# MrSwordFish/rvel-mcmc

Measured on AMD Instinct MI355X. Metric: walker-logL evals/sec (2-planet, 100 obs, 4096 walkers); ESS/sec, higher is better.
Workload: dtype f64

## Files before the change

include/rvmcmc.h:

```cpp
#ifndef RVMCMC_H
#define RVMCMC_H

#include <stddef.h>
#include <stdint.h>

#ifdef __cplusplus
extern "C" {
#endif

#define RVM_ABI_VERSION 12

#define RVM_STATUS_OK 0
#define RVM_STATUS_PRIOR 1
#define RVM_STATUS_ENCOUNTER 2
#define RVM_STATUS_NONFINITE 3
#define RVM_STATUS_UNRESOLVED 4
#define RVM_STATUS_SKIPPED 5

#define RVM_MAX_PLANETS 4
#define RVM_MAX_LEVELS 6
#define RVM_MAX_EPOCHS_PER_DIRECTION 1700
#define RVM_SMALA_MAX_PARAMS 20
#define RVM_RESOLVE_MAX_LIMIT 12

typedef struct {
    int32_t n_planets;
    double dt;
    int32_t n_levels;
    double npoints_norm;
    int32_t level_mult[RVM_MAX_LEVELS];
    double period_hint;
    int32_t inclined;
    double resolve_tol;
    int32_t resolve_max;
} rvm_config;

typedef struct rvm_plan rvm_plan;

int rvm_plan_create(const rvm_config* cfg, const double* t, const double* rv, const double* sigma, int32_t n_obs,
                    int32_t max_walkers, rvm_plan** out);
void rvm_plan_destroy(rvm_plan* plan);
int rvm_plan_info(const rvm_plan* plan, int32_t* steps_fwd, int32_t* steps_bwd, int32_t* epochs_fwd,
                  int32_t* epochs_bwd);
#define RVM_EXT_MAX_BYTES (4ull << 30)
int rvm_plan_extension(const rvm_plan* plan, int32_t* ext_mult);
int rvm_plan_set_verify_eccentricity(rvm_plan* plan, double e);

int rvm_plan_set_certain_reject(rvm_plan* plan, int32_t on);

int rvm_plan_faults(rvm_plan* plan, int32_t reset, int64_t* handoff_timeouts, int64_t* nonfinite,
                    int64_t* unresolved, int64_t* refined, int64_t* truncated, void* stream);
#define RVM_N_COUNTERS 7
int rvm_plan_counters(rvm_plan* plan, int32_t reset, int64_t* out, int32_t n, void* stream);
int rvm_plan_hedge_stats(rvm_plan* plan, int32_t reset, int64_t* hedged, int64_t* replayed, int64_t* missed,
                         void* stream);
int rvm_plan_hedge_marks(rvm_plan* plan, int32_t reset, int64_t* marked, int64_t* gave_up, void* stream);
int rvm_plan_time_kernels(rvm_plan* plan, int32_t max_launches);
int rvm_plan_kernel_times(rvm_plan* plan, float* logl_ms, float* refine_ms, int32_t max, int32_t* n_out);
int rvm_plan_set_handoff_timeout(rvm_plan* plan, double seconds);

int rvm_logl_batch(const rvm_plan* plan, int32_t n_walkers, const double* params, double hill_factor,
                   double* logl_out, int32_t* status_out, double* rv_out, void* stream);


int rvm_stretch_propose(int32_t n_params, int32_t n_s0, int64_t s0_begin, const double* x, int32_t n_s1,
                        const double* c, double a, uint64_t seed, uint64_t iteration, uint32_t half,
                        const double* draws, double* q_out, double* z_out, void* stream);
int rvm_stretch_accept(int32_t n_params, int32_t n_s0, int64_t s0_begin, double* x, double* lnp, const double* q,
                       const double* lnp_new, const double* z, uint64_t seed, uint64_t iteration, uint32_t half,
                       const double* draws, int32_t* accepted, void* stream);

#define RVM_MAX_PARAM_ROWS (7 * RVM_MAX_PLANETS)
typedef struct rvm_param_map {
    int32_t n_rows;
    int32_t src[RVM_MAX_PARAM_ROWS];
    double base[RVM_MAX_PARAM_ROWS];
} rvm_param_map;

int rvm_stretch_half_step(const rvm_plan* plan, const rvm_param_map* map, int32_t n_params, int32_t n_s0,
                          int64_t s0_begin, double* x, double* x_aos, double* lnp, int32_t n_s1, const double* c_aos,
                          double a, uint64_t seed, uint64_t iteration, uint32_t half, double hill_factor,
                          double* lnp_new_out, int32_t* status_out, int32_t* accepted, void* stream);

int rvm_stretch_iteration_begin(const rvm_plan* plan, const rvm_param_map* map, int32_t n_params, int32_t n_loc,
                                int64_t s0_begin, int64_t s1_begin, double* x0, double* lnp0, const double* x1,
                                const double* lnp1, int32_t n_half, const double* c0, const double* c1, double a,
                                uint64_t seed, uint64_t iteration, double hill_factor, double* lnp_spec,
                                int32_t* status_spec, int32_t* dec, int32_t* accepted0, void* stream);
int rvm_stretch_iteration_end(int32_t n_params, int32_t n_loc, int64_t s0_begin, int64_t s1_begin, const double* x0,
                              double* x0_aos, const int32_t* dec, const int32_t* dec_all, double* x1, double* x1_aos,
                              double* lnp1, int32_t n_half, const double* c0, const double* c1,
                              const double* lnp_spec, const int32_t* status_spec, double a, uint64_t seed,
                              uint64_t iteration, int32_t* accepted1, double* lnp_new_out, int32_t* status_new_out,
                              void* stream);

int rvm_pt_stretch_propose(int32_t n_params, int32_t n_temps, int32_t n_half, const double* x, const double* c,
                           double a, uint64_t seed, uint64_t iteration, uint32_t half, const double* draws,
                           double* q_out, double* z_out, void* stream);
int rvm_pt_stretch_accept(int32_t n_params, int32_t n_temps, int32_t n_half, const double* betas, double* x,
                          double* lnp, const double* q, const double* lnp_new, const double* z, uint64_t seed,
                          uint64_t iteration, uint32_t half, const double* draws, int32_t* accepted, void* stream);
int rvm_pt_swap(int32_t n_params, int32_t n_temps, int32_t n_half, const double* betas, double* x0, double* x1,
                double* lnp0, double* lnp1, uint64_t seed, uint64_t iteration, const double* draws,
                int32_t* swapped, void* stream);

int rvm_pt_ladder_update(int32_t n_temps, int32_t n_half, const int32_t* swapped, const double* lnp0,
                         const double* lnp1, double kappa, double* betas, int64_t* swap_totals_prev,
                         double* ratios_out, int64_t* n_refused, double* lnp_moments, void* workspace,
                         void* stream);

int rvm_mh_propose(int32_t n_params, int32_t n_chains, int64_t chain_begin, const double* x, const double* scales,
                   double step_size, uint64_t seed, uint64_t iteration, const double* draws, double* q_out,
                   void* stream);
int rvm_mh_accept(int32_t n_params, int32_t n_chains, int64_t chain_begin, double* x, double* lnp, const double* q,
                  const double* lnp_new, uint64_t seed, uint64_t iteration, const double* draws, int32_t* accepted,
                  void* stream);
int rvm_mh_step(const rvm_plan* plan, const rvm_param_map* map, int32_t n_params, int32_t n_chains,
                int64_t chain_begin, double* x, double* lnp, const double* scales, double step_size, uint64_t seed,
                uint64_t iteration, double hill_factor, double* lnp_new_out, int32_t* status_out, int32_t* accepted,
                void* stream);

int rvm_fd_params(int32_t n_params, int32_t n_chains, const double* x, double rel_step, const double* floor_,
                  double* out, void* stream);

typedef struct {
    double* lp;
    double* grad;
    double* mu;
    double* L;
    double* G;
    double* logdet;
    int32_t* ok;
} rvm_smala_cache;

int rvm_smala_derive(int32_t n_params, int32_t n_chains, int32_t n_obs, const double* x, double rel_step,
                     const double* floor_, const double* lp_stencil, const int32_t* status_stencil,
                     const double* rv_stencil, const double* inv_sigma2, double npoints_norm, double alpha,
                     double eps, const rvm_smala_cache* out, void* stream);
int rvm_smala_metric(int32_t n_params, int32_t n_chains, const double* x, const double* lp, const int32_t* status,
                     const double* grad, const double* hess, double alpha, double eps, const rvm_smala_cache* out,
                     void* stream);
int rvm_smala_propose(int32_t n_params, int32_t n_chains, int64_t chain_begin, const double* x,
                      const rvm_smala_cache* cur, double eps, uint64_t seed, uint64_t iteration,
                      const double* draws, double* x_prop, void* stream);
int rvm_smala_accept(int32_t n_params, int32_t n_chains, int64_t chain_begin, double* x, const rvm_smala_cache* cur,
                     const double* x_prop, const rvm_smala_cache* prop, double eps, uint64_t seed,
                     uint64_t iteration, const double* draws, int32_t* accepted, int32_t* failures, void* stream);

int rvm_smala_stencil_logl(const rvm_plan* plan, const rvm_param_map* map, int32_t n_params, int32_t n_chains,
                           const double* x, double rel_step, const double* floor_, double hill_factor,
                           double* logl_out, int32_t* status_out, double* rv_out, void* stream);
int rvm_smala_derive_accept(int32_t n_params, int32_t n_chains, int64_t chain_begin, int32_t n_obs, double* x,
                            const double* x_prop, double rel_step, const double* floor_, const double* lp_stencil,
                            const int32_t* status_stencil, const double* rv_stencil, const double* inv_sigma2,
                            double npoints_norm, double alpha, double eps, const rvm_smala_cache* cur,
                            const rvm_smala_cache* prop, uint64_t seed, uint64_t iteration, const double* draws,
                            int32_t* accepted, int32_t* failures, void* stream);
int rvm_smala_derive_sides(int32_t n_params, int32_t n_chains, int32_t n_obs, const double* x, double rel_step,
                           const double* floor_, const double* lp_stencil, const int32_t* status_stencil,
                           const double* rv_stencil, const double* inv_sigma2, double npoints_norm, double alpha,
                           double eps, const rvm_smala_cache* out, void* stream);
int rvm_smala_center_accept(int32_t n_params, int32_t n_chains, int64_t chain_begin, double* x, const double* x_prop,
                            const double* lp_center, const int32_t* status_center, const rvm_smala_cache* cur,
                            const rvm_smala_cache* prop, double eps, uint64_t seed, uint64_t iteration,
                            const double* draws, int32_t* accepted, int32_t* failures, void* stream);
int rvm_smala_metric_accept(int32_t n_params, int32_t n_chains, int64_t chain_begin, double* x, const double* x_prop,
                            const double* lp, const int32_t* status, const double* grad, const double* hess,
                            double alpha, double eps, const rvm_smala_cache* cur, const rvm_smala_cache* prop,
                            uint64_t seed, uint64_t iteration, const double* draws, int32_t* accepted,
                            int32_t* failures, void* stream);

size_t rvm_logl_derivs_workspace_bytes(int32_t n_chains, int32_t n_dirs);
int rvm_logl_derivs(const rvm_plan* plan, int32_t n_chains, const double* params, int32_t n_dirs,
                    const int32_t* dir_rows, double hill_factor, double* logl_out, double* grad_out, double* hess_out,
                    int32_t* status_out, void* workspace, void* stream);

int rvm_chain_record(int32_t n_params, int32_t n_cols, const double* src, int64_t src_ld, int64_t src_col0,
                     int64_t col_stride, double* dst, int64_t dst_ld, int64_t dst_col0, const double* lnp_src,
                     double* lnp_dst, void* stream);
int rvm_chain_moments(const double* chain, int32_t n_params, int32_t n_cols, int64_t t0, int64_t t1, double* mean_out,
                      double* m2_out, void* stream);
size_t rvm_chain_autocov_workspace_bytes(int32_t n_params, int32_t n_cols, int32_t n_lags);
int rvm_chain_autocov(const double* chain, const double* mean, int32_t n_params, int32_t n_cols, int64_t t0, int64_t t1,
                      int32_t lag0, int32_t n_lags, double* acov_out, void* workspace, void* stream);

const char* rvm_last_error(void);
int rvm_abi_version(void);

#ifdef __cplusplus
}
#endif

#endif
```

rvel-mcmc_amd/csrc/host_sanitize.cpp:

```cpp
#include <algorithm>
#include <cmath>
#include <cstdio>
#include <cstdlib>
#include <cstring>
#include <vector>

#include "rvm_plan_host.h"

static int fails = 0;
static void expect(bool ok, const char* what) {
    if (!ok) {
        std::fprintf(stderr, "FAIL %s\n", what);
        fails++;
    }
}

static double exact_weight(const int* m, int k0, int n, int k) {
    long long num = 1, den = 1;
    for (int j = k0; j < n; j++) {
        if (j == k) continue;
        num *= (long long)m[k] * m[k];
        den *= (long long)m[k] * m[k] - (long long)m[j] * m[j];
    }
    return (double)num / (double)den;
}

static bool close_rel(double a, double b, double rel) { return std::fabs(a - b) <= rel * std::fabs(b); }

static double ulp_of(double x) { return std::nextafter(std::fabs(x), INFINITY) - std::fabs(x); }

struct Range {
    size_t off, bytes;
    bool wide;
};
static void check_block(const std::vector<Range>& r, size_t block_bytes, const char* what) {
    size_t end = 0;
    for (const Range& x : r) {
        expect(x.off >= end, what);
        expect(!x.wide || x.off % 8 == 0, what);
        end = x.off + x.bytes;
    }
    expect(end <= block_bytes, what);
}

static const char* const kKnobNames[] = {
    "RVM_SKIP_VARIANTS", "RVM_LATE_SPO",   "RVM_NO_LEVEL_SPLIT", "RVM_REFINE_TEAMS", "RVM_EAGER_SPLIT",
    "RVM_NO_EXTENSION",  "RVM_REFINE_SPLIT", "RVM_TEAMS_HINT",   "RVM_EAGER",        "RVM_EAGER_PASSES",
    "RVM_HEDGE",         "RVM_HEDGE_GROUPS", "RVM_HEDGE_MARK",   "RVM_LS_F0"};

static rvm::PlanKnobs knobs_with(const char* name, const char* value) {
    setenv(name, value, 1);
    const rvm::PlanKnobs K = rvm::read_plan_knobs();
    unsetenv(name);
    return K;
}

static void check_plan_host(const rvm_config& cfg, const std::vector<double>& t, const std::vector<double>& rv,
                            const std::vector<double>& sg) {
    using namespace rvm;
    const int n_obs = (int)t.size();
    for (const char* name : kKnobNames) unsetenv(name);
    const PlanKnobs K = read_plan_knobs();
    expect(K.skip_variants == 1 && K.late_spo == 96.0 && !K.no_level_split && K.n_teams == RVM_TEAMS_DEFAULT &&
               K.eager_split == 1 && !K.no_extension && K.refine_split && K.teams_hint && K.eager &&
               K.eager_passes == 1 && K.hedge_groups == RVM_HEDGE_GROUPS_MAX && K.hedge_mark == 1,
           "knob defaults");
    expect(knobs_with("RVM_REFINE_TEAMS", "9").n_teams == RVM_TEAMS_MAX, "RVM_REFINE_TEAMS=9 clamps");
    expect(knobs_with("RVM_HEDGE", "0").hedge_groups == 0, "RVM_HEDGE=0");
    expect(knobs_with("RVM_HEDGE_GROUPS", "3").hedge_groups == 3, "RVM_HEDGE_GROUPS=3");
    expect(knobs_with("RVM_EAGER_PASSES", "2").eager_passes == 2, "RVM_EAGER_PASSES=2");
    expect(knobs_with("RVM_SKIP_VARIANTS", "0").skip_variants == 0, "RVM_SKIP_VARIANTS=0");

    int mult[RVM_MAX_LEVELS] = {}, max_mult = 0;
    expect(check_plan_config(&cfg, t.data(), rv.data(), sg.data(), n_obs, 4096, mult, &max_mult) == nullptr,
           "config ok");
    expect(mult[0] == 4 && mult[1] == 5 && mult[2] == 6 && mult[3] == 7 && max_mult == 7, "explicit ladder");
    {
        rvm_config h = cfg;
        h.n_levels = 3;
        std::memset(h.level_mult, 0, sizeof(h.level_mult));
        int hm[RVM_MAX_LEVELS] = {}, hmax = 0;
        expect(check_plan_config(&h, t.data(), rv.data(), sg.data(), n_obs, 64, hm, &hmax) == nullptr && hm[0] == 1 &&
                   hm[1] == 2 && hm[2] == 3 && hmax == 3,
               "harmonic ladder");
    }

    HostDir dir[2];
    expect(build_schedule(&cfg, mult, max_mult, t.data(), rv.data(), sg.data(), n_obs, dir) == nullptr, "schedule ok");
    std::vector<int> seen(n_obs, 0);
    int n_dup = 0;
    for (int d = 0; d < 2; d++) {
        const HostDir& D = dir[d];
        const size_t n = D.idx.size();
        expect(D.seg_n.size() == n && D.seg_len.size() == n && D.orv.size() == n && D.os2.size() == n,
               "schedule sizes");
        long long sum = 0, pre0 = 0, pre1 = 0;
        double tprev = 0.0;
        for (size_t i = 0; i < n; i++) {
            const int o = D.idx[i];
            expect(o >= 0 && o < n_obs && (d == 0) == (t[o] >= 0.0), "obs_idx direction");
            if (o >= 0 && o < n_obs) seen[o]++;
            const double at = std::fabs(t[o]), len = (d == 0 ? 1.0 : -1.0) * (at - tprev);
            expect(at >= tprev, "|t| non-decreasing");
            if (at == tprev) {
                n_dup += i > 0;
                expect(D.seg_n[i] == 0 && D.seg_len[i] == 0.0, "duplicate epoch: empty segment");
            } else {
                expect(D.seg_n[i] >= 1 && std::fabs(D.seg_len[i]) <= cfg.dt * (1.0 + 1e-9), "segment step <= dt");
                expect(std::fabs(D.seg_n[i] * D.seg_len[i] - len) <= 4.0 * ulp_of(len), "segment steps x step = length");
            }
            tprev = at;
            if ((int)i < D.split0) pre0 += D.seg_n[i];
            if ((int)i < D.split1) pre1 += D.seg_n[i];
            sum += D.seg_n[i];
        }
        expect(sum == D.total_steps, "sum(seg_n) = n_steps");
        expect(D.split0 >= 0 && D.split0 <= (int)n && D.split1 >= 0 && D.split1 <= (int)n, "split range");
        expect(pre0 == D.pre0 && pre1 == D.pre1, "pre = steps before the split");
    }
    expect(std::all_of(seen.begin(), seen.end(), [](int c) { return c == 1; }), "obs_idx is a permutation");
    expect(n_dup == 1, "one duplicate epoch");

    const size_t nf = dir[0].idx.size(), nb = dir[1].idx.size();
    rvm_config ad = cfg;
    ad.resolve_tol = 5e-7;
    ad.resolve_max = 6;
    DevPlan P{};
    fill_plan_scalars(&ad, mult, n_obs, nf, nb, 256, K, &P);
    expect(P.ext_mult == 0 && plan_wants_extension(P, K), "extension wanted, not yet applied");
    fill_plan_extension(&P);
    const int m5[5] = {4, 5, 6, 7, 8};
    for (int k = 0; k < 4; k++) expect(close_rel(P.lw[k], exact_weight(m5, 0, 4, k), 1e-14), "lw");
    for (int k = 1; k < 4; k++) expect(close_rel(P.lw3[k], exact_weight(m5, 1, 4, k), 1e-14), "lw3");
    for (int k = 0; k < 5; k++) expect(close_rel(P.lw5[k], exact_weight(m5, 0, 5, k), 1e-14), "lw5");
    expect(P.lw3[0] == 0.0 && P.lw[4] == 0.0 && P.lw[5] == 0.0 && P.lw5[5] == 0.0, "unused weights are zero");

    expect(P.fin_level == 3, "fin_level");
    expect(P.ext_mult == 8 && P.mult[4] == 8 && P.inv_ext == 0.125 && P.inv_mult[4] == 0.125, "ext_mult");
    expect(P.rmax == 6 && P.rtol_dir == 2.5e-7 && P.cut == 1 && P.n_teams == RVM_TEAMS_DEFAULT, "adaptive scalars");
    for (int k = 0; k < 4; k++) {
        const double nh = 2.0 * M_PI * cfg.dt / (mult[k] * cfg.period_hint), zn = 2.0 * nh * nh;
        expect(P.nt[k] == (zn <= 0.1 ? 6 : (zn <= 0.3 ? 7 : 8)) && P.spec[k] == (zn <= 0.04 ? 1 : 0), "nt / spec");
        expect(P.inv_mult[k] == 1.0 / mult[k], "inv_mult");
    }
    expect(P.ext_nt == P.nt[3] && P.ext_spec == P.spec[3] && P.nt[4] == P.nt[3] && P.spec[4] == P.spec[3],
           "ext nt / spec");
    expect(P.late_mult == (int)std::ceil(96 * 0.65 / 5.2 - 1e-9) && P.late_mult == 12, "late_mult");
    expect(P.lc_ring >= 2 && P.lc_ring <= RVM_LC_RING, "lc_ring range");
    expect((size_t)(cfg.n_levels + 1) * 32 * 8 * P.lc_ring <= RVM_LC_RING_BYTES, "lc_ring bytes");
    {
        DevPlan Q{};
        fill_plan_scalars(&cfg, mult, n_obs, nf, nb, 256, K, &Q);
        expect(Q.rmax == 0 && !plan_wants_extension(Q, K) && Q.ext_mult == 0, "no extension without resolve_tol");
        ad.resolve_max = 0;
        fill_plan_scalars(&ad, mult, n_obs, nf, nb, 256, K, &Q);
        expect(!plan_wants_extension(Q, K) && Q.ext_mult == 0, "no extension with resolve_max 0");
        expect(!plan_wants_extension(P, knobs_with("RVM_NO_EXTENSION", "1")), "RVM_NO_EXTENSION=1");
        fill_plan_scalars(&cfg, mult, n_obs, nf, nb, 256, knobs_with("RVM_LATE_SPO", "0"), &Q);
        expect(Q.late_mult == 0, "RVM_LATE_SPO=0");
    }

    for (int32_t mw : {1, 64, 6144}) {
        const size_t w = (size_t)mw, em = std::max(nf, nb);
        const DmemLayout D = dmem_layout(nf, nb, mw);
        check_block({{D.seg_h1[0], 8 * nf, true}, {D.obs_rv[0], 8 * nf, true}, {D.obs_s2[0], 8 * nf, true},
                     {D.seg_h1[1], 8 * nb, true}, {D.obs_rv[1], 8 * nb, true}, {D.obs_s2[1], 8 * nb, true},
                     {D.slots, 8 * w, true}, {D.counters, 8 * RVM_N_COUNTERS, true}, {D.seg_n[0], 4 * nf, false},
                     {D.obs_idx[0], 4 * nf, false}, {D.seg_n[1], 4 * nb, false}, {D.obs_idx[1], 4 * nb, false}},
                    D.bytes, "dmem layout");
        const LvLayout V = lv_layout(nf, nb, mw);
        expect(V.emax == (int32_t)em, "lv emax");
        check_block({{V.rv, 8 * 2 * em * w, true}, {V.enc, 4 * 2 * w, false}}, V.bytes, "lvmem layout");
        for (int teams : {1, 2, 4}) {
            const size_t nt = (size_t)std::max(teams, 2), xg = (w + 15) / 16 + 1;
            const XLayout X = x_layout(nf, nb, mw, teams);
            check_block({{X.lvx, 16 * em * w, true}, {X.rvp, 16 * em * w, true},
                         {X.rvp2, 16 * em * w * (teams - 1), true}},
                        X.bytes, "xmem layout");
            const RqLayout R = rq_layout(mw, teams);
            expect(R.xgroups == (int32_t)xg, "rq xgroups");
            check_block({{R.x, xg * nt * 256 * 8, true}, {R.xf, xg * nt * 2 * 8, true},
                         {R.t, xg * (nt - 1) * 1024 * 8, true}, {R.tf, xg * nt * 8, true}, {R.c, 16 * w, true},
                         {R.w, 12 * w, false}, {R.n, 16, false}, {R.gen, 8, true}, {R.mark, 4 * w, false},
                         {R.depth, 8 * (RVM_DEPTH_WINDOW + 1), true}},
                        R.bytes, "rqmem layout");
            expect(R.gen == R.n + 32 && R.mark == R.n + 64 && R.mark % 64 == R.n % 64, "rq_n | gen_dev | rq_mark");
        }
        const HLayout H = h_layout((int32_t)em, mw);
        const size_t hs = RVM_HEDGE_STRIDE;
        check_block({{H.hrv, 16 * em * hs, true}, {H.hsum, 48 * hs, true}, {H.hslot, 16 * hs, true},
                     {H.htab, 8 * w, true}, {H.hw, 8 * RVM_HW_WORDS, true}},
                    H.bytes, "hmem layout");
        const ELayout E = e_layout((int32_t)em, mw);
        check_block({{E.rve, 32 * em * w, true}, {E.esum, 96 * w, true},
                     {E.eflag, 8 * (RVM_EFLAG_WORDS * (size_t)((RVM_EAGER_MAX + 15) / 16) + 8), true}},
                    E.bytes, "emem layout");
    }
}

int main() {
    expect(rvm_abi_version() == RVM_ABI_VERSION, "abi version");
    rvm_config cfg{};
    cfg.n_planets = 2;
    cfg.dt = 0.65;
    cfg.n_levels = 4;
    cfg.npoints_norm = 100.0;
    const int mult[4] = {4, 5, 6, 7};
    std::memcpy(cfg.level_mult, mult, sizeof(mult));
    cfg.period_hint = 5.2;
    std::vector<double> t, rv, sg;
    for (int i = 0; i < 101; i++) {
        t.push_back(i % 2 ? -0.6 * i : 0.55 * (100 - i));
        rv.push_back(1e-4 * std::sin(i));
        sg.push_back(1.5e-4);
    }
    t[7] = t[9];
    rvm_plan* plan = nullptr;
    const int rc = rvm_plan_create(&cfg, t.data(), rv.data(), sg.data(), (int)t.size(), 4096, &plan);
    expect(rc == 0 || (rc < 0 && plan == nullptr), "plan_create valid input");
    if (rc == 0) rvm_plan_destroy(plan);
    check_plan_host(cfg, t, rv, sg);
    rvm_config bad = cfg;
    bad.n_levels = 0;
    expect(rvm_plan_create(&bad, t.data(), rv.data(), sg.data(), (int)t.size(), 64, &plan) < 0, "n_levels 0");
    bad = cfg;
    bad.level_mult[1] = 4;
    expect(rvm_plan_create(&bad, t.data(), rv.data(), sg.data(), (int)t.size(), 64, &plan) < 0, "dup multipliers");
    bad = cfg;
    bad.dt = -1.0;
    expect(rvm_plan_create(&bad, t.data(), rv.data(), sg.data(), (int)t.size(), 64, &plan) < 0, "negative dt");
    std::vector<double> tn = t;
    tn[3] = NAN;
    expect(rvm_plan_create(&cfg, tn.data(), rv.data(), sg.data(), (int)t.size(), 64, &plan) < 0, "nan epoch");
    expect(std::strlen(rvm_last_error()) > 0, "last_error");
    expect(rvm_logl_batch(nullptr, 1, nullptr, 1.0, nullptr, nullptr, nullptr, nullptr) < 0, "logl null plan");
    int64_t mk = -1, gu = -1;
    expect(rvm_plan_hedge_marks(nullptr, 0, &mk, &gu, nullptr) < 0 && mk == -1 && gu == -1, "hedge_marks null plan");
    rvm_param_map pm{};
    expect(rvm_stretch_half_step(nullptr, &pm, 10, 1, 0, nullptr, nullptr, nullptr, 1, nullptr, 2.0, 0, 0, 0, 1.0,
                                 nullptr, nullptr, nullptr, nullptr) < 0,
           "half_step null plan");
    expect(rvm_stretch_propose(0, 1, 0, nullptr, 1, nullptr, 2.0, 0, 0, 0, nullptr, nullptr, nullptr, nullptr) < 0,
           "propose bad");
    double d1 = 0.5;
    int32_t i1 = 0;
    expect(rvm_pt_stretch_propose(10, 0, 1, &d1, &d1, 2.0, 0, 0, 0, nullptr, &d1, &d1, nullptr) < 0, "pt n_temps 0");
    expect(rvm_pt_stretch_propose(10, 2, 1, &d1, &d1, 1.0, 0, 0, 0, nullptr, &d1, &d1, nullptr) < 0, "pt a = 1");
    expect(rvm_pt_stretch_propose(10, 1 << 16, 1 << 16, &d1, &d1, 2.0, 0, 0, 0, nullptr, &d1, &d1, nullptr) < 0,
           "pt int32 overflow");
    expect(rvm_pt_stretch_accept(10, 2, 1, nullptr, &d1, &d1, &d1, &d1, &d1, 0, 0, 0, nullptr, &i1, nullptr) < 0,
           "pt null betas");
    expect(rvm_pt_stretch_accept(10, 2, 1, &d1, &d1, &d1, &d1, &d1, &d1, 0, 0, 2, nullptr, &i1, nullptr) < 0,
           "pt half 2");
    expect(rvm_pt_swap(10, 2, 0, &d1, &d1, &d1, &d1, &d1, 0, 0, nullptr, &i1, nullptr) < 0, "pt n_half 0");
    expect(rvm_pt_swap(10, 1 << 15, 1 << 15, &d1, &d1, &d1, &d1, &d1, 0, 0, nullptr, &i1, nullptr) < 0,
           "pt swap int32 overflow");
    expect(rvm_pt_swap(10, 1, 4, nullptr, nullptr, nullptr, nullptr, nullptr, 0, 0, nullptr, nullptr, nullptr) == 0,
           "pt swap of one temperature");
    int64_t l1 = 0;
    expect(rvm_pt_ladder_update(3, 1, &i1, &d1, &d1, -1.0, &d1, &l1, &d1, &l1, nullptr, &d1, nullptr) < 0,
           "pt ladder kappa < 0");
    expect(rvm_pt_ladder_update(3, 1, &i1, &d1, &d1, 0.5, &d1, &l1, &d1, &l1, nullptr, nullptr, nullptr) < 0,
           "pt ladder null workspace");
    expect(rvm_pt_ladder_update(1 << 16, 1 << 15, &i1, &d1, &d1, 0.5, &d1, &l1, &d1, &l1, nullptr, &d1, nullptr) < 0,
           "pt ladder int32 overflow");
    expect(rvm_pt_ladder_update(1, 4, nullptr, nullptr, nullptr, 0.5, nullptr, nullptr, nullptr, nullptr, nullptr,
                                nullptr, nullptr) == 0,
           "pt ladder of one temperature");
    expect(rvm_chain_record(2, 4, &d1, 16, 0, INT64_MAX, &d1, 8, 0, nullptr, nullptr, nullptr) < 0,
           "chain record stride overflow");
    expect(rvm_chain_record(2, 4, &d1, 16, 0, 1, &d1, INT64_MAX, INT64_MAX - 1, nullptr, nullptr, nullptr) < 0,
           "chain record dst_col0 overflow");
    expect(rvm_chain_record(2, 4, &d1, 16, 0, 1, &d1, 8, 0, &d1, nullptr, nullptr) < 0, "chain record lone lnp_src");
    expect(rvm_chain_moments(&d1, 2, 4, 5, 5, &d1, &d1, nullptr) < 0, "chain moments empty range");
    expect(rvm_chain_autocov(&d1, &d1, 2, 4, 0, 10, INT32_MAX, 1 << 30, &d1, &d1, nullptr) < 0,
           "chain autocov lag overflow");
    expect(rvm_chain_autocov(&d1, &d1, 65534, 4, 0, INT64_MAX, 0, 1 << 30, &d1, &d1, nullptr) < 0,
           "chain autocov n_params * n_lags");
    expect(rvm_chain_autocov_workspace_bytes(10, 200, 17) == (size_t)8 * 10 * 32, "chain autocov workspace");
    expect(rvm_chain_autocov_workspace_bytes(1, 65535 * 256, 1 << 30) == (size_t)8 * ((size_t)1 << 30) * 65535,
           "chain autocov workspace, largest");
    expect(rvm_chain_autocov_workspace_bytes(65534, 4, 1 << 30) == 0, "chain autocov workspace, refused");
    expect(rvm_mh_accept(0, 1, 0, nullptr, nullptr, nullptr, nullptr, 0, 0, nullptr, nullptr, nullptr) < 0, "mh bad");
    expect(rvm_fd_params(10, 1, nullptr, 1e-6, nullptr, nullptr, nullptr) < 0, "fd bad");
    const int32_t rows[2] = {0, 0};
    expect(rvm_logl_derivs(nullptr, 1, nullptr, 2, rows, 1.0, nullptr, nullptr, nullptr, nullptr, nullptr, nullptr) < 0,
           "derivs null plan");
    expect(rvm_logl_derivs_workspace_bytes(256, 10) == (size_t)256 * 55 * 2 * 36, "derivs workspace");
    rvm_smala_cache c{};
    expect(rvm_smala_metric(10, 1, nullptr, nullptr, nullptr, nullptr, nullptr, 1.0, 0.5, &c, nullptr) < 0, "metric bad");
    std::printf("host sanitize driver: %d failures\n", fails);
    return fails;
}
```

rvel-mcmc_amd/csrc/rvm_internal.h:

```cpp
#pragma once
#include <stdint.h>

#include "../../include/rvmcmc.h"

namespace rvm {

constexpr int RVM_LS_RING = 64;
constexpr int RVM_LC_RING = 16;
constexpr int RVM_LC_RING_BYTES = 24 * 1024;
constexpr int RVM_LDS_PER_CU = 160 * 1024;
constexpr int RVM_INIT_DOUBLES = 8 * 64;
constexpr double RVM_EXT_ACCEPT = 1.0;
constexpr double RVM_CUT_EST_FACTOR = 100.0;
constexpr double RVM_FLOOR_BOUND = 4.0;
constexpr double RVM_CUT_ECC_FACTOR = 0.6712;
constexpr double RVM_CUT_GUARD_K = 10.0;
constexpr int RVM_CX_MIN_WALKERS = 32;
constexpr int RVM_EAGER_MAX = 512;
constexpr int RVM_EAGER_MIN = 32;
constexpr int RVM_EFLAG_WORDS = 8;
constexpr int RVM_TEAMS_MAX = 4;
constexpr int RVM_TEAMS_DEFAULT = 4;
constexpr int RVM_DEPTH_WINDOW = 8;
constexpr int RVM_HEDGE_GROUPS_MAX = 8;
constexpr int RVM_HEDGE_STRIDE = 512;
constexpr int RVM_HEDGE_CAND = RVM_HEDGE_STRIDE + 64;
constexpr int RVM_HEDGE_MAX_W = 12288;
constexpr int RVM_HW_STATS = 2 + 2 * RVM_HEDGE_GROUPS_MAX;
constexpr int RVM_HW_MARK = RVM_HW_STATS + 3 + 3;
constexpr int RVM_HW_WORDS = RVM_HW_MARK + 2 * RVM_HEDGE_GROUPS_MAX;

struct DirSched {
    int32_t n_epochs;
    int32_t n_steps;
    int32_t split0, pre0, split1, pre1;
    const int32_t* seg_n;
    const double* seg_h1;
    const double* obs_rv;
    const double* obs_s2;
    const int32_t* obs_idx;
};

struct DevPlan {
    int32_t n_planets;
    int32_t n_levels;
    int32_t mult[RVM_MAX_LEVELS];
    int32_t nt[RVM_MAX_LEVELS];
    int32_t spec[RVM_MAX_LEVELS];
    int32_t late_mult;
    int32_t lc_ring;
    double inv_mult[RVM_MAX_LEVELS];
    double lw[RVM_MAX_LEVELS];
    double lw3[RVM_MAX_LEVELS];
    double rtol_dir;
    int32_t rmax;
    int32_t fin_level;
    int32_t cut;
    int32_t ext_mult, ext_nt, ext_spec;
    double inv_ext;
    double lw5[RVM_MAX_LEVELS + 1];
    double* lvx;
    double* rvp;
    double e2_guard;
    double e2_cut;
    double cut_guard_k;
    int32_t lvx_emax, lvx_stride;
    int32_t* rq_n;
    int32_t* rq_w;
    double* rq_c;
    int32_t rq_cap;
    int32_t* rq_mark;
    int32_t skip_variants;
    unsigned long long* rq_x;
    unsigned long long* rq_xf;
    int32_t rq_xgroups;
    unsigned long long* rq_t;
    unsigned long long* rq_tf;
    double* rvp2;
    int32_t n_teams;
    unsigned long long* depth_w;
    double* rve;
    double* esum;
    unsigned long long* eflag;
    int32_t eager_max;
    int32_t eager_passes;
    int32_t eager_split;
    int32_t hedge_groups;
    int32_t hedge_mark;
    double* hrv;
    double* hsum;
    unsigned long long* hslot;
    unsigned long long* htab;
    unsigned long long* hw;
    unsigned long long* gen_dev;
    unsigned long long* counters;
    unsigned long long spin_ticks;
    double npoints;
    int32_t n_obs;
    int32_t inclined;
    int32_t n_cu;
    double* lv_rv;
    int32_t* lv_enc;
    int32_t lv_emax, lv_stride;
    DirSched fwd, bwd;
};

struct StretchArgs {
    const double* c;
    double* x;
    double* x_aos;
    double* lnp;
    int32_t* accepted;
    int64_t s0_begin;
    uint64_t seed, iteration;
    double a;
    int32_t n1, dim;
    uint32_t half;
    int32_t xstride;
    int32_t n_spec;
    const double* c0;
    const double* x1;
    int64_t s1_begin;
    int32_t* dec;
    const double* lnp1;
    const double* mh_scale;
    double mh_step;
    const double* fd_x;
    const double* fd_floor;
    double fd_rel;
    int32_t fd_n;
    int32_t src[RVM_MAX_PARAM_ROWS];
    double base[RVM_MAX_PARAM_ROWS];
};

struct IterEndArgs {
    int32_t dim, n, n_half;
    int64_t s0_begin, s1_begin;
    const double* x0;
    double* x0_aos;
    const int32_t* dec_local;
    const int32_t* dec_all;
    double* x1;
    double* x1_aos;
    double* lnp1;
    const double* c0;
    const double* c1;
    const double* lnp_spec;
    const int32_t* st_spec;
    double a;
    uint64_t seed, iteration;
    int32_t* accepted1;
    double* lnp_new_out;
    int32_t* status_new_out;
};

struct PtLadderArgs {
    int32_t T, Wh;
    const int32_t* swapped;
    const double* lnp0;
    const double* lnp1;
    double kappa;
    double* betas;
    int64_t* totals_prev;
    double* ratios;
    int64_t* n_refused;
    double* moments;
    int64_t* ws_totals;
    double* ws_moments;
};

struct SmalaCache {
    double* lp;
    double* grad;
    double* mu;
    double* L;
    double* G;
    double* logdet;
    int32_t* ok;
};

}
```

rvel-mcmc_amd/csrc/rvm_plan.hip:

```cpp
#include <algorithm>
#include <cmath>
#include <cstdlib>
#include <cstring>

#include "rvm_launch.h"
#include "rvm_plan.h"
#include "rvm_plan_host.h"

using rvm::fail;
using rvm::hip_fail;

namespace {

template <class T>
T* at(void* block, size_t offset) {
    return reinterpret_cast<T*>(reinterpret_cast<unsigned char*>(block) + offset);
}

template <class T>
const T* put(std::vector<unsigned char>& host, void* block, size_t offset, const std::vector<T>& v) {
    if (!v.empty()) std::memcpy(host.data() + offset, v.data(), v.size() * sizeof(T));
    return at<T>(block, offset);
}

bool alloc_filled(void** mem, size_t bytes, int fill) {
    if (hipMalloc(mem, bytes) == hipSuccess && hipMemset(*mem, fill, bytes) == hipSuccess &&
        hipDeviceSynchronize() == hipSuccess)
        return true;
    (void)hipGetLastError();
    if (*mem) (void)hipFree(*mem);
    *mem = nullptr;
    return false;
}

int upload_schedule(rvm_plan* plan, const rvm::HostDir dir[2], int32_t max_walkers) {
    const rvm::DmemLayout L = rvm::dmem_layout(dir[0].idx.size(), dir[1].idx.size(), max_walkers);
    hipError_t e = hipMalloc(&plan->dmem, L.bytes);
    if (e != hipSuccess) return hip_fail(e, "rvm_plan_create: hipMalloc");
    std::vector<unsigned char> host(L.bytes, 0);
    rvm::DirSched* S[2] = {&plan->dev.fwd, &plan->dev.bwd};
    for (int dd = 0; dd < 2; dd++) {
        const rvm::HostDir& D = dir[dd];
        S[dd]->n_epochs = (int32_t)D.idx.size();
        S[dd]->n_steps = plan->steps[dd] = (int32_t)D.total_steps;
        S[dd]->split0 = D.split0;
        S[dd]->pre0 = D.pre0;
        S[dd]->split1 = D.split1;
        S[dd]->pre1 = D.pre1;
        S[dd]->seg_h1 = put(host, plan->dmem, L.seg_h1[dd], D.seg_len);
        S[dd]->obs_rv = put(host, plan->dmem, L.obs_rv[dd], D.orv);
        S[dd]->obs_s2 = put(host, plan->dmem, L.obs_s2[dd], D.os2);
        S[dd]->seg_n = put(host, plan->dmem, L.seg_n[dd], D.seg_n);
        S[dd]->obs_idx = put(host, plan->dmem, L.obs_idx[dd], D.idx);
    }
    plan->slots = at<unsigned long long>(plan->dmem, L.slots);
    for (int32_t i = 0; i < max_walkers; i++)
        at<unsigned long long>(host.data(), L.slots)[i] = 0x7FF4DEADBEEF0001ULL;
    plan->dev.counters = at<unsigned long long>(plan->dmem, L.counters);
    plan->max_walkers = max_walkers;
    e = hipMemcpy(plan->dmem, host.data(), L.bytes, hipMemcpyHostToDevice);
    return e == hipSuccess ? 0 : hip_fail(e, "rvm_plan_create: hipMemcpy");
}

int device_cus() {
    int dev = 0, ncu = 0;
    if (hipGetDevice(&dev) != hipSuccess ||
        hipDeviceGetAttribute(&ncu, hipDeviceAttributeMultiprocessorCount, dev) != hipSuccess)
        ncu = 0;
    return ncu;
}

void alloc_level_split(rvm_plan* plan, size_t nf, size_t nb, const rvm::PlanKnobs& K) {
    rvm::DevPlan& P = plan->dev;
    if (!rvm::plan_wants_level_split(P, plan->max_walkers, K)) return;
    const rvm::LvLayout L = rvm::lv_layout(nf, nb, plan->max_walkers);
    if (!alloc_filled(&plan->lvmem, L.bytes, 0xFF)) return;
    P.lv_rv = at<double>(plan->lvmem, L.rv);
    P.lv_enc = at<int32_t>(plan->lvmem, L.enc);
    P.lv_emax = L.emax;
    P.lv_stride = plan->max_walkers;
    plan->lv_bytes = L.bytes;
}

void alloc_extension(rvm_plan* plan, size_t nf, size_t nb, const rvm::PlanKnobs& K) {
    rvm::DevPlan& P = plan->dev;
    if (!rvm::plan_wants_extension(P, K)) return;
    const rvm::XLayout L = rvm::x_layout(nf, nb, plan->max_walkers, K.n_teams);
    if (L.bytes > RVM_EXT_MAX_BYTES) return;
    if (hipMalloc(&plan->xmem, L.bytes) != hipSuccess) {
        plan->xmem = nullptr;
        (void)hipGetLastError();
        return;
    }
    rvm::fill_plan_extension(&P);
    P.lvx = at<double>(plan->xmem, L.lvx);
    P.rvp = at<double>(plan->xmem, L.rvp);
    P.rvp2 = K.n_teams >= 2 ? at<double>(plan->xmem, L.rvp2) : nullptr;
    P.lvx_emax = L.emax;
    P.lvx_stride = plan->max_walkers;
}

int alloc_work_lists(rvm_plan* plan, const rvm::PlanKnobs& K) {
    rvm::DevPlan& P = plan->dev;
    if (P.rmax <= 0) return 0;
    const rvm::RqLayout L = rvm::rq_layout(plan->max_walkers, K.n_teams);
    if (hipMalloc(&plan->rqmem, L.bytes) != hipSuccess || hipMemset(plan->rqmem, 0, L.bytes) != hipSuccess ||
        hipDeviceSynchronize() != hipSuccess) {
        (void)hipGetLastError();
        return fail(-3, "rvm_plan_create: hipMalloc of the refinement work lists failed");
    }
    P.rq_x = K.refine_split ? at<unsigned long long>(plan->rqmem, L.x) : nullptr;
    P.rq_xf = at<unsigned long long>(plan->rqmem, L.xf);
    P.rq_t = K.n_teams >= 2 ? at<unsigned long long>(plan->rqmem, L.t) : nullptr;
    P.rq_tf = at<unsigned long long>(plan->rqmem, L.tf);
    P.rq_c = at<double>(plan->rqmem, L.c);
    P.rq_w = at<int32_t>(plan->rqmem, L.w);
    P.rq_n = at<int32_t>(plan->rqmem, L.n);
    P.gen_dev = at<unsigned long long>(plan->rqmem, L.gen);
    P.rq_mark = at<int32_t>(plan->rqmem, L.mark);
    P.depth_w = K.teams_hint ? at<unsigned long long>(plan->rqmem, L.depth) : nullptr;
    P.rq_cap = plan->max_walkers;
    P.rq_xgroups = L.xgroups;
    const unsigned long long gen1 = 1;
    if (hipMemcpy(P.gen_dev, &gen1, sizeof(gen1), hipMemcpyHostToDevice) != hipSuccess) {
        (void)hipGetLastError();
        return fail(-3, "rvm_plan_create: initialising the launch generation failed");
    }
    return 0;
}

void side_drop(rvm_plan* plan) {
    (void)hipGetLastError();
    if (plan->ev_fork) (void)hipEventDestroy(plan->ev_fork);
    if (plan->ev_join) (void)hipEventDestroy(plan->ev_join);
    if (plan->side) (void)hipStreamDestroy(plan->side);
    plan->side = nullptr;
    plan->ev_fork = plan->ev_join = nullptr;
    plan->dev.hedge_groups = 0;
}

bool side_create(rvm_plan* plan) {
    if (hipStreamCreateWithFlags(&plan->side, hipStreamNonBlocking) == hipSuccess &&
        hipEventCreateWithFlags(&plan->ev_fork, hipEventDisableTiming) == hipSuccess &&
        hipEventCreateWithFlags(&plan->ev_join, hipEventDisableTiming) == hipSuccess)
        return true;
    side_drop(plan);
    return false;
}

void setup_side_features(rvm_plan* plan, const rvm::PlanKnobs& K) {
    rvm::DevPlan& P = plan->dev;
    const int32_t mw = plan->max_walkers;
    const bool refines = P.rmax >= 2 && P.rvp != nullptr && P.gen_dev != nullptr && P.n_levels <= 4 &&
                         mw >= rvm::RVM_EAGER_MIN;
    if (K.hedge_groups > 0 && refines && P.n_cu >= 4) {
        const rvm::HLayout L = rvm::h_layout(P.lvx_emax, mw);
        if (alloc_filled(&plan->hmem, L.bytes, 0)) {
            P.hrv = at<double>(plan->hmem, L.hrv);
            P.hsum = at<double>(plan->hmem, L.hsum);
            P.hslot = at<unsigned long long>(plan->hmem, L.hslot);
            P.htab = at<unsigned long long>(plan->hmem, L.htab);
            P.hw = at<unsigned long long>(plan->hmem, L.hw);
            P.hedge_groups = K.hedge_groups;
            P.hedge_mark = K.hedge_mark;
        }
    }
    if (!(refines && K.eager)) {
        if (P.hedge_groups > 0) (void)side_create(plan);
        return;
    }
    const rvm::ELayout L = rvm::e_layout(P.lvx_emax, P.lvx_stride);
    if (alloc_filled(&plan->emem, L.bytes, 0) && side_create(plan)) {
        P.rve = at<double>(plan->emem, L.rve);
        P.esum = at<double>(plan->emem, L.esum);
        P.eflag = at<unsigned long long>(plan->emem, L.eflag);
        P.eager_max = std::min<int>(mw, rvm::RVM_EAGER_MAX);
        P.eager_passes = K.eager_passes;
    } else {
        side_drop(plan);
        if (plan->emem) (void)hipFree(plan->emem);
        plan->emem = nullptr;
    }
}

int prepare_kernels(const rvm::DevPlan& P) {
    const hipError_t pe = rvm::prepare_logl(P);
    if (pe != hipSuccess)
        return fail(-1, pe == hipErrorInvalidConfiguration
                            ? "rvm_plan_create: the epoch schedule does not fit the likelihood kernel's LDS "
                              "(too many epochs in one direction)"
                            : "rvm_plan_create: n_planets has no kernel instantiation");
    if (rvm::prepare_refine(P) != hipSuccess)
        return fail(-1, "rvm_plan_create: the epoch schedule does not fit the refinement kernel's LDS "
                        "(too many epochs in one direction for the adaptive resolution)");
    return 0;
}

int read_hw_words(rvm_plan* plan, const char* who, int first, int n, int32_t reset, void* stream,
                  unsigned long long* h) {
    if (!plan) return fail(-1, std::string(who) + ": null plan");
    std::memset(h, 0, n * sizeof(*h));
    if (plan->dev.hw == nullptr) return 0;
    hipStream_t st = (hipStream_t)stream;
    unsigned long long* d = plan->dev.hw + first;
    hipError_t e = hipMemcpyAsync(h, d, n * sizeof(*h), hipMemcpyDeviceToHost, st);
    if (e == hipSuccess && reset) e = hipMemsetAsync(d, 0, n * sizeof(*h), st);
    if (e == hipSuccess) e = hipStreamSynchronize(st);
    return e == hipSuccess ? 0 : hip_fail(e, who);
}

}

extern "C" {

int rvm_plan_create(const rvm_config* cfg, const double* t, const double* rv, const double* sigma, int32_t n_obs,
                    int32_t max_walkers, rvm_plan** out) {
    if (!cfg || !t || !rv || !sigma || !out) return fail(-1, "rvm_plan_create: null argument");
    int mult[RVM_MAX_LEVELS], max_mult = 1;
    if (const char* m = rvm::check_plan_config(cfg, t, rv, sigma, n_obs, max_walkers, mult, &max_mult))
        return fail(-1, m);
    rvm::HostDir dir[2];
    if (const char* m = rvm::build_schedule(cfg, mult, max_mult, t, rv, sigma, n_obs, dir)) return fail(-1, m);
    const size_t nf = dir[0].idx.size(), nb = dir[1].idx.size();
    const rvm::PlanKnobs K = rvm::read_plan_knobs();
    rvm_plan* plan = new rvm_plan();
    int rc = upload_schedule(plan, dir, max_walkers);
    if (rc == 0) {
        rvm::fill_plan_scalars(cfg, mult, n_obs, nf, nb, device_cus(), K, &plan->dev);
        alloc_level_split(plan, nf, nb, K);
        alloc_extension(plan, nf, nb, K);
        rc = alloc_work_lists(plan, K);
    }
    if (rc == 0) {
        setup_side_features(plan, K);
        rc = prepare_kernels(plan->dev);
    }
    if (rc != 0) {
        rvm_plan_destroy(plan);
        return rc;
    }
    *out = plan;
    return 0;
}

void rvm_plan_destroy(rvm_plan* plan) {
    if (!plan) return;
    if (plan->side) (void)hipStreamSynchronize(plan->side);
    if (plan->ev_fork) (void)hipEventDestroy(plan->ev_fork);
    if (plan->ev_join) (void)hipEventDestroy(plan->ev_join);
    if (plan->side) (void)hipStreamDestroy(plan->side);
    if (plan->emem) (void)hipFree(plan->emem);
    if (plan->hmem) (void)hipFree(plan->hmem);
    for (hipEvent_t ev : plan->tev) (void)hipEventDestroy(ev);
    if (plan->rqmem) (void)hipFree(plan->rqmem);
    if (plan->lvmem) (void)hipFree(plan->lvmem);
    if (plan->xmem) (void)hipFree(plan->xmem);
    if (plan->dmem) (void)hipFree(plan->dmem);
    delete plan;
}

int rvm_plan_set_certain_reject(rvm_plan* plan, int32_t on) {
    if (!plan) return fail(-1, "rvm_plan_set_certain_reject: null plan");
    plan->dev.cut = on ? 1 : 0;
    return 0;
}

int rvm_plan_set_verify_eccentricity(rvm_plan* plan, double e) {
    if (!plan) return fail(-1, "rvm_plan_set_verify_eccentricity: null plan");
    if (std::isnan(e) || e >= 1.0) return fail(-1, "rvm_plan_set_verify_eccentricity: e must be < 1 (<= 0: off)");
    plan->dev.e2_guard = e > 0.0 ? e * e : INFINITY;
    {
        const char* cf = getenv("RVM_CUT_FACTOR");
        const double ec = 1.0 - (1.0 - e) * (cf ? atof(cf) : rvm::RVM_CUT_ECC_FACTOR);
        const char* cg = getenv("RVM_CUT_GUARD");
        plan->dev.e2_cut = e > 0.0 && !(cg && atoi(cg) == 0) ? ec * ec : INFINITY;
        const char* ck = getenv("RVM_CUT_GUARD_K");
        plan->dev.cut_guard_k = ck ? atof(ck) : rvm::RVM_CUT_GUARD_K;
    }
    return 0;
}

int rvm_plan_extension(const rvm_plan* plan, int32_t* ext_mult) {
    if (!plan) return fail(-1, "rvm_plan_extension: null plan");
    if (ext_mult) *ext_mult = plan->dev.ext_mult;
    return 0;
}

int rvm_plan_counters(rvm_plan* plan, int32_t reset, int64_t* out, int32_t n, void* stream) {
    if (!plan) return fail(-1, "rvm_plan_counters: null plan");
    if (n < 0 || (n > 0 && !out)) return fail(-1, "rvm_plan_counters: bad output array");
    hipStream_t st = (hipStream_t)stream;
    unsigned long long h[RVM_N_COUNTERS] = {};
    hipError_t e = hipMemcpyAsync(h, plan->dev.counters, sizeof(h), hipMemcpyDeviceToHost, st);
    if (e == hipSuccess) e = hipStreamSynchronize(st);
    if (e != hipSuccess) return hip_fail(e, "rvm_plan_counters");
    for (int i = 0; i < n; i++) out[i] = i < RVM_N_COUNTERS ? (int64_t)h[i] : 0;
    if (reset) {
        if (plan->lvmem) e = hipMemsetAsync(plan->lvmem, 0xFF, plan->lv_bytes, st);
        if (e == hipSuccess) e = hipMemsetAsync(plan->dev.counters, 0, sizeof(h), st);
        if (e == hipSuccess) e = hipStreamSynchronize(st);
        if (e != hipSuccess) return hip_fail(e, "rvm_plan_counters: reset");
    }
    return 0;
}

int rvm_plan_hedge_stats(rvm_plan* plan, int32_t reset, int64_t* hedged, int64_t* replayed, int64_t* missed,
                         void* stream) {
    unsigned long long h[3];
    const int rc = read_hw_words(plan, "rvm_plan_hedge_stats", rvm::RVM_HW_STATS, 3, reset, stream, h);
    if (rc != 0) return rc;
    if (hedged) *hedged = (int64_t)h[0];
    if (replayed) *replayed = (int64_t)h[1];
    if (missed) *missed = (int64_t)h[2];
    return 0;
}

int rvm_plan_hedge_marks(rvm_plan* plan, int32_t reset, int64_t* marked, int64_t* gave_up, void* stream) {
    unsigned long long h[2];
    const int rc = read_hw_words(plan, "rvm_plan_hedge_marks", rvm::RVM_HW_STATS + 3, 2, reset, stream, h);
    if (rc != 0) return rc;
    if (marked) *marked = (int64_t)h[0];
    if (gave_up) *gave_up = (int64_t)h[1];
    return 0;
}

int rvm_plan_faults(rvm_plan* plan, int32_t reset, int64_t* handoff_timeouts, int64_t* nonfinite,
                    int64_t* unresolved, int64_t* refined, int64_t* truncated, void* stream) {
    if (!plan) return fail(-1, "rvm_plan_faults: null plan");
    int64_t c[RVM_N_COUNTERS] = {};
    const int rc = rvm_plan_counters(plan, reset, c, RVM_N_COUNTERS, stream);
    if (rc != 0) return rc;
    if (handoff_timeouts) *handoff_timeouts = c[0];
    if (nonfinite) *nonfinite = c[1];
    if (unresolved) *unresolved = c[2];
    if (refined) *refined = c[3];
    if (truncated) *truncated = c[4];
    return 0;
}

int rvm_plan_time_kernels(rvm_plan* plan, int32_t max_launches) {
    if (!plan) return fail(-1, "rvm_plan_time_kernels: null plan");
    if (max_launches < 0 || max_launches > 4096) return fail(-1, "rvm_plan_time_kernels: max_launches out of range");
    while ((int32_t)plan->tev.size() < 3 * max_launches) {
        hipEvent_t ev;
        const hipError_t e = hipEventCreate(&ev);
        if (e != hipSuccess) return hip_fail(e, "rvm_plan_time_kernels: hipEventCreate");
        plan->tev.push_back(ev);
    }
    plan->tcap = max_launches;
    plan->tn = 0;
    return 0;
}

int rvm_plan_kernel_times(rvm_plan* plan, float* logl_ms, float* refine_ms, int32_t max, int32_t* n_out) {
    if (!plan || max < 0) return fail(-1, "rvm_plan_kernel_times: bad arguments");
    const int n = std::min(plan->tn, max);
    for (int i = 0; i < n; i++) {
        hipError_t e = hipEventSynchronize(plan->tev[3 * i + 2]);
        float a = 0.0f, b = 0.0f;
        if (e == hipSuccess) e = hipEventElapsedTime(&a, plan->tev[3 * i], plan->tev[3 * i + 1]);
        if (e == hipSuccess) e = hipEventElapsedTime(&b, plan->tev[3 * i + 1], plan->tev[3 * i + 2]);
        if (e != hipSuccess) return hip_fail(e, "rvm_plan_kernel_times");
        if (logl_ms) logl_ms[i] = a;
        if (refine_ms) refine_ms[i] = b;
    }
    if (n_out) *n_out = n;
    plan->tn = 0;
    plan->tcap = 0;
    return 0;
}

int rvm_plan_set_handoff_timeout(rvm_plan* plan, double seconds) {
    if (!plan) return fail(-1, "rvm_plan_set_handoff_timeout: null plan");
    if (!(seconds > 0.0) || !(seconds < 1e9)) return fail(-1, "rvm_plan_set_handoff_timeout: seconds out of range");
    const double ticks = seconds * 1e8;
    plan->dev.spin_ticks = ticks < 1.0 ? 1ull : (unsigned long long)ticks;
    return 0;
}

int rvm_plan_info(const rvm_plan* plan, int32_t* sf, int32_t* sb, int32_t* ef, int32_t* eb) {
    if (!plan) return fail(-1, "rvm_plan_info: null plan");
    if (sf) *sf = plan->steps[0];
    if (sb) *sb = plan->steps[1];
    if (ef) *ef = plan->dev.fwd.n_epochs;
    if (eb) *eb = plan->dev.bwd.n_epochs;
    return 0;
}

}
```

rvel-mcmc_amd/csrc/rvm_plan_host.cpp:

```cpp
#include "rvm_plan_host.h"

#include <algorithm>
#include <cmath>
#include <cstdlib>

#ifndef RVM_EAGER_DEFAULT
#define RVM_EAGER_DEFAULT true
#endif
#ifndef RVM_EAGER_PASSES_DEFAULT
#define RVM_EAGER_PASSES_DEFAULT 1
#endif

namespace rvm {

static bool starts(const char* s, char c) { return s && s[0] == c; }

PlanKnobs read_plan_knobs() {
    PlanKnobs K;
    K.skip_variants = starts(getenv("RVM_SKIP_VARIANTS"), '0') ? 0 : 1;
    const char* ls = getenv("RVM_LATE_SPO");
    K.late_spo = ls ? atof(ls) : 96.0;
    K.no_level_split = false;
#ifdef RVM_PROFILE
    K.no_level_split = starts(getenv("RVM_NO_LEVEL_SPLIT"), '1');
#endif
    K.n_teams = RVM_TEAMS_DEFAULT;
    if (const char* tp = getenv("RVM_REFINE_TEAMS")) K.n_teams = std::max(1, std::min(atoi(tp), RVM_TEAMS_MAX));
    K.eager_split = starts(getenv("RVM_EAGER_SPLIT"), '0') ? 0 : 1;
    K.no_extension = starts(getenv("RVM_NO_EXTENSION"), '1');
    K.refine_split = !starts(getenv("RVM_REFINE_SPLIT"), '0');
    K.teams_hint = !starts(getenv("RVM_TEAMS_HINT"), '0');
    const char* eg = getenv("RVM_EAGER");
    K.eager = eg ? eg[0] == '1' : RVM_EAGER_DEFAULT;
    const char* ep = getenv("RVM_EAGER_PASSES");
    K.eager_passes = starts(ep, '1') ? 1 : (starts(ep, '2') ? 2 : RVM_EAGER_PASSES_DEFAULT);
    K.hedge_groups = starts(getenv("RVM_HEDGE"), '0') ? 0 : RVM_HEDGE_GROUPS_MAX;
    if (const char* hn = getenv("RVM_HEDGE_GROUPS"))
        K.hedge_groups = std::min(K.hedge_groups, std::max(0, std::min(atoi(hn), (int)RVM_HEDGE_GROUPS_MAX)));
    K.hedge_mark = starts(getenv("RVM_HEDGE_MARK"), '0') ? 0 : 1;
    return K;
}

const char* check_plan_config(const rvm_config* cfg, const double* t, const double* rv, const double* sigma,
                              int32_t n_obs, int32_t max_walkers, int mult[RVM_MAX_LEVELS], int* max_mult) {
    if (cfg->n_planets < 1 || cfg->n_planets > RVM_MAX_PLANETS) return "rvm_plan_create: n_planets out of range";
    if (cfg->n_levels < 1 || cfg->n_levels > RVM_MAX_LEVELS) return "rvm_plan_create: n_levels out of range";
    if (!(cfg->dt > 0.0) || !std::isfinite(cfg->dt)) return "rvm_plan_create: dt must be > 0";
    if (n_obs < 0 || max_walkers < 1) return "rvm_plan_create: bad sizes";
    if (!(cfg->npoints_norm != 0.0)) return "rvm_plan_create: npoints_norm must be nonzero";
    bool harmonic = true;
    for (int k = 0; k < cfg->n_levels; k++) harmonic = harmonic && cfg->level_mult[k] == 0;
    *max_mult = 1;
    for (int k = 0; k < cfg->n_levels; k++) {
        mult[k] = harmonic ? k + 1 : cfg->level_mult[k];
        if (mult[k] < 1 || mult[k] > 64) return "rvm_plan_create: level_mult out of range (1..64)";
        for (int j = 0; j < k; j++)
            if (mult[j] == mult[k]) return "rvm_plan_create: level_mult entries must be distinct";
        *max_mult = std::max(*max_mult, mult[k]);
    }
    if (!(cfg->period_hint >= 0.0) || !std::isfinite(cfg->period_hint))
        return "rvm_plan_create: period_hint must be >= 0";
    if (std::isnan(cfg->resolve_tol) || cfg->resolve_max < 0 || cfg->resolve_max > RVM_RESOLVE_MAX_LIMIT)
        return "rvm_plan_create: resolve_tol must be a number and resolve_max in 0..12";
    for (int i = 0; i < n_obs; i++)
        if (!std::isfinite(t[i]) || !std::isfinite(rv[i]) || !std::isfinite(sigma[i]))
            return "rvm_plan_create: non-finite observation";
    return nullptr;
}

static void split_point(const HostDir& D, double frac, int32_t* split, int32_t* pre) {
    const double target = frac * (double)D.total_steps;
    long long cum = 0, best_cum = 0;
    int best = 0;
    double best_d = target;
    for (size_t i = 0; i < D.seg_n.size(); i++) {
        cum += D.seg_n[i];
        const double dist = std::fabs((double)cum - target);
        if (dist < best_d) {
            best_d = dist;
            best = (int)i + 1;
            best_cum = cum;
        }
    }
    *split = best;
    *pre = (int32_t)best_cum;
}

const char* build_schedule(const rvm_config* cfg, const int* mult, int max_mult, const double* t, const double* rv,
                           const double* sigma, int32_t n_obs, HostDir dir[2]) {
    const int rmax = cfg->resolve_tol > 0.0 ? cfg->resolve_max : 0;
    double f0 = 0.5;
    if (cfg->n_levels == 4) f0 = (double)(mult[3] + mult[0] - mult[2]) / (2.0 * mult[0]) + 0.11;
#ifdef RVM_PROFILE
    if (const char* ef = getenv("RVM_LS_F0")) f0 = atof(ef);
#endif
    f0 = std::min(1.0, std::max(0.0, f0));
    for (int dd = 0; dd < 2; dd++) {
        HostDir& D = dir[dd];
        for (int i = 0; i < n_obs; i++)
            if ((dd == 0) == (t[i] >= 0.0)) D.idx.push_back(i);
        std::stable_sort(D.idx.begin(), D.idx.end(), [&](int a, int b) { return std::fabs(t[a]) < std::fabs(t[b]); });
        const double sign = dd == 0 ? 1.0 : -1.0;
        double tprev = 0.0;
        for (int i : D.idx) {
            const double at = std::fabs(t[i]);
            const double len = at - tprev;
            tprev = at;
            int n = len > 0.0 ? (int)std::ceil(len / cfg->dt - 1e-9) : 0;
            if (len > 0.0 && n < 1) n = 1;
            D.seg_n.push_back(n);
            D.seg_len.push_back(n > 0 ? sign * len / n : 0.0);
            D.orv.push_back(rv[i]);
            D.os2.push_back(sigma[i] * sigma[i]);
            D.total_steps += n;
        }
        if ((D.total_steps * (long long)max_mult) << rmax > (1LL << 30))
            return "rvm_plan_create: dt too small for the epoch span";
        if (D.idx.size() > (size_t)RVM_MAX_EPOCHS_PER_DIRECTION)
            return "rvm_plan_create: too many epochs in one direction (the schedule is staged in LDS)";
        split_point(D, f0, &D.split0, &D.pre0);
        split_point(D, 0.5, &D.split1, &D.pre1);
    }
    return nullptr;
}

void lagrange_at_zero(const int* m, int k0, int n, double* w) {
    for (int k = k0; k < n; k++) {
        const double xk = 1.0 / ((double)m[k] * m[k]);
        double wk = 1.0;
        for (int j = k0; j < n; j++) {
            if (j == k) continue;
            const double xj = 1.0 / ((double)m[j] * m[j]);
            wk *= xj / (xj - xk);
        }
        w[k] = wk;
    }
}

void fill_plan_scalars(const rvm_config* cfg, const int* mult, int32_t n_obs, size_t nf, size_t nb, int n_cu,
                       const PlanKnobs& K, DevPlan* Pp) {
    DevPlan& P = *Pp;
    const int nl = cfg->n_levels;
    P.n_planets = cfg->n_planets;
    P.n_levels = nl;
    P.npoints = cfg->npoints_norm;
    P.n_obs = n_obs;
    P.inclined = cfg->inclined ? 1 : 0;
    P.n_cu = n_cu;
    for (int k = 0; k < RVM_MAX_LEVELS; k++) {
        P.mult[k] = k < nl ? mult[k] : 1;
        P.inv_mult[k] = 1.0 / P.mult[k];
        P.lw[k] = P.lw3[k] = 0.0;
        P.nt[k] = 8;
        P.spec[k] = 0;
        if (k < nl && cfg->period_hint > 0.0) {
            const double nh = 2.0 * M_PI * cfg->dt / (mult[k] * cfg->period_hint);
            const double zn = 2.0 * nh * nh;
            P.nt[k] = zn <= 0.1 ? 6 : (zn <= 0.3 ? 7 : 8);
            P.spec[k] = zn <= 0.04 ? 1 : 0;
        }
    }
    lagrange_at_zero(mult, 0, nl, P.lw);
    lagrange_at_zero(mult, 1, nl, P.lw3);
    P.rtol_dir = cfg->resolve_tol > 0.0 && nl >= 2 ? 0.5 * cfg->resolve_tol : INFINITY;
    P.fin_level = 0;
    for (int k = 1; k < nl; k++)
        if (mult[k] > mult[P.fin_level]) P.fin_level = k;
    P.rmax = P.rtol_dir < INFINITY ? cfg->resolve_max : 0;
    P.cut = 1;
    P.spin_ticks = 200000000ull;
    const int emax = (int)std::max<size_t>(std::max(nf, nb), 1);
    const int fit = (int)(RVM_LC_RING_BYTES / ((size_t)(nl + 1) * walkers_per_group(cfg->n_planets) * sizeof(double)));
    P.lc_ring = std::max(2, std::min(std::min(RVM_LC_RING, emax), fit));
    P.skip_variants = K.skip_variants;
    P.late_mult = 0;
    if (K.late_spo > 0.0 && cfg->period_hint > 0.0)
        P.late_mult = std::max(1, (int32_t)std::ceil(K.late_spo * cfg->dt / cfg->period_hint - 1e-9));
    P.n_teams = P.rmax > 0 ? std::max(K.n_teams, 2) : K.n_teams;
    P.eager_split = K.eager_split;
    P.e2_guard = P.e2_cut = INFINITY;
    P.cut_guard_k = 0.0;
    P.ext_mult = 0;
    P.ext_nt = 8;
    P.ext_spec = 0;
    P.inv_ext = 1.0;
    for (int k = 0; k <= RVM_MAX_LEVELS; k++) P.lw5[k] = 0.0;
}

bool plan_wants_extension(const DevPlan& P, const PlanKnobs& K) {
    return P.rmax > 0 && P.n_levels >= 2 && P.n_levels < RVM_MAX_LEVELS && !K.no_extension;
}

void fill_plan_extension(DevPlan* Pp) {
    DevPlan& P = *Pp;
    const int nl = P.n_levels, fin = P.fin_level;
    int m5[RVM_MAX_LEVELS + 1];
    for (int k = 0; k < nl; k++) m5[k] = P.mult[k];
    m5[nl] = P.mult[fin] + 1;
    lagrange_at_zero(m5, 0, nl + 1, P.lw5);
    P.ext_mult = m5[nl];
    P.ext_nt = P.nt[fin];
    P.ext_spec = P.spec[fin];
    P.inv_ext = 1.0 / m5[nl];
    P.mult[nl] = P.ext_mult;
    P.nt[nl] = P.ext_nt;
    P.spec[nl] = P.ext_spec;
    P.inv_mult[nl] = P.inv_ext;
}

bool plan_wants_level_split(const DevPlan& P, int32_t max_walkers, const PlanKnobs& K) {
    const int wpb = walkers_per_group(P.n_planets);
    const int64_t groups = ((int64_t)max_walkers + wpb - 1) / wpb;
    bool inc = P.n_levels == 4 && !K.no_level_split;
    for (int k = 1; inc && k < 4; k++) inc = P.mult[k] > P.mult[k - 1];
    return inc && P.n_cu > 0 && 2 * groups > P.n_cu;
}

static size_t take(size_t& end, size_t bytes) {
    end += bytes;
    return end - bytes;
}
static size_t epochs_max(size_t nf, size_t nb) { return std::max<size_t>(std::max(nf, nb), 1); }

DmemLayout dmem_layout(size_t nf, size_t nb, int32_t max_walkers) {
    DmemLayout L{};
    const size_t n[2] = {nf, nb};
    for (int d = 0; d < 2; d++) {
        L.seg_h1[d] = take(L.bytes, n[d] * sizeof(double));
        L.obs_rv[d] = take(L.bytes, n[d] * sizeof(double));
        L.obs_s2[d] = take(L.bytes, n[d] * sizeof(double));
    }
    L.slots = take(L.bytes, (size_t)max_walkers * sizeof(unsigned long long));
    L.counters = take(L.bytes, RVM_N_COUNTERS * sizeof(unsigned long long));
    for (int d = 0; d < 2; d++) {
        L.seg_n[d] = take(L.bytes, n[d] * sizeof(int32_t));
        L.obs_idx[d] = take(L.bytes, n[d] * sizeof(int32_t));
    }
    L.bytes += 64;
    return L;
}

LvLayout lv_layout(size_t nf, size_t nb, int32_t max_walkers) {
    LvLayout L{};
    L.emax = (int32_t)epochs_max(nf, nb);
    L.rv = take(L.bytes, (size_t)(2 * (int64_t)L.emax * max_walkers) * sizeof(double));
    L.enc = take(L.bytes, (size_t)(2 * (int64_t)max_walkers) * sizeof(int32_t));
    return L;
}

XLayout x_layout(size_t nf, size_t nb, int32_t max_walkers, int n_teams) {
    XLayout L{};
    L.emax = (int32_t)epochs_max(nf, nb);
    const size_t bl = 2 * (size_t)L.emax * (size_t)max_walkers * sizeof(double);
    L.lvx = take(L.bytes, bl);
    L.rvp = take(L.bytes, bl);
    L.rvp2 = take(L.bytes, ((size_t)n_teams - 1) * bl);
    return L;
}

RqLayout rq_layout(int32_t max_walkers, int n_teams) {
    RqLayout L{};
    const size_t xg = (size_t)(((int64_t)max_walkers + 15) / 16 + 1), nt = (size_t)std::max(n_teams, 2);
    const size_t u64 = sizeof(unsigned long long);
    L.xgroups = (int32_t)xg;
    L.x = take(L.bytes, xg * nt * 2 * 2 * 64 * u64);
    L.xf = take(L.bytes, xg * nt * 2 * u64);
    L.t = take(L.bytes, xg * (nt - 1) * 16 * 64 * u64);
    L.tf = take(L.bytes, xg * nt * u64);
    L.c = take(L.bytes, 2 * (size_t)max_walkers * sizeof(double));
    L.w = take(L.bytes, (3 * (size_t)max_walkers * sizeof(int32_t) + 7) & ~(size_t)7);
    L.n = take(L.bytes, 64);
    L.gen = L.n + 32;
    L.mark = take(L.bytes, ((size_t)max_walkers * sizeof(int32_t) + 63) & ~(size_t)63);
    L.depth = take(L.bytes, (RVM_DEPTH_WINDOW + 1) * u64);
    return L;
}

HLayout h_layout(int32_t lvx_emax, int32_t max_walkers) {
    HLayout L{};
    const size_t hs = RVM_HEDGE_STRIDE, w = sizeof(double);
    L.hrv = take(L.bytes, 2 * (size_t)lvx_emax * hs * w);
    L.hsum = take(L.bytes, 6 * hs * w);
    L.hslot = take(L.bytes, 2 * hs * w);
    L.htab = take(L.bytes, (size_t)max_walkers * w);
    L.hw = take(L.bytes, RVM_HW_WORDS * w);
    return L;
}

ELayout e_layout(int32_t lvx_emax, int32_t lvx_stride) {
    ELayout L{};
    const size_t plane = (size_t)lvx_emax * lvx_stride;
    L.rve = take(L.bytes, 4 * plane * sizeof(double));
    L.esum = take(L.bytes, 12 * (size_t)lvx_stride * sizeof(double));
    L.eflag = take(L.bytes, (RVM_EFLAG_WORDS * (size_t)((RVM_EAGER_MAX + 15) / 16) + 8) * sizeof(double));
    return L;
}

}
```

rvel-mcmc_amd/csrc/rvm_plan_host.h:

```cpp
#pragma once
#include <cstddef>
#include <vector>

#include "rvm_internal.h"

namespace rvm {

struct PlanKnobs {
    int32_t skip_variants;
    double late_spo;
    bool no_level_split;
    int32_t n_teams;
    int32_t eager_split;
    bool no_extension;
    bool refine_split;
    bool teams_hint;
    bool eager;
    int32_t eager_passes;
    int32_t hedge_groups;
    int32_t hedge_mark;
};
PlanKnobs read_plan_knobs();

const char* check_plan_config(const rvm_config* cfg, const double* t, const double* rv, const double* sigma,
                              int32_t n_obs, int32_t max_walkers, int mult[RVM_MAX_LEVELS], int* max_mult);

struct HostDir {
    std::vector<int32_t> idx, seg_n;
    std::vector<double> seg_len, orv, os2;
    long long total_steps = 0;
    int32_t split0 = 0, pre0 = 0, split1 = 0, pre1 = 0;
};
const char* build_schedule(const rvm_config* cfg, const int* mult, int max_mult, const double* t, const double* rv,
                           const double* sigma, int32_t n_obs, HostDir dir[2]);

void lagrange_at_zero(const int* m, int k0, int n, double* w);

inline int walkers_per_group(int n_planets) { return n_planets == 1 ? 64 : (n_planets == 2 ? 32 : 16); }

void fill_plan_scalars(const rvm_config* cfg, const int* mult, int32_t n_obs, size_t nf, size_t nb, int n_cu,
                       const PlanKnobs& K, DevPlan* P);
bool plan_wants_extension(const DevPlan& P, const PlanKnobs& K);
void fill_plan_extension(DevPlan* P);
bool plan_wants_level_split(const DevPlan& P, int32_t max_walkers, const PlanKnobs& K);

struct DmemLayout {
    size_t seg_h1[2], obs_rv[2], obs_s2[2], slots, counters, seg_n[2], obs_idx[2], bytes;
};
DmemLayout dmem_layout(size_t nf, size_t nb, int32_t max_walkers);
struct LvLayout {
    size_t rv, enc, bytes;
    int32_t emax;
};
LvLayout lv_layout(size_t nf, size_t nb, int32_t max_walkers);
struct XLayout {
    size_t lvx, rvp, rvp2, bytes;
    int32_t emax;
};
XLayout x_layout(size_t nf, size_t nb, int32_t max_walkers, int n_teams);
struct RqLayout {
    size_t x, xf, t, tf, c, w, n, gen, mark, depth, bytes;
    int32_t xgroups;
};
RqLayout rq_layout(int32_t max_walkers, int n_teams);
struct HLayout {
    size_t hrv, hsum, hslot, htab, hw, bytes;
};
HLayout h_layout(int32_t lvx_emax, int32_t max_walkers);
struct ELayout {
    size_t rve, esum, eflag, bytes;
};
ELayout e_layout(int32_t lvx_emax, int32_t lvx_stride);

}
```

rvel-mcmc_amd/csrc/rvm_refine_impl.h:

```cpp
#pragma once
#include <hip/hip_runtime.h>
#include <math.h>

#pragma clang fp contract(on)

#include "rvm_walker.h"

#ifndef RVM_REFINE_GUESS
#define RVM_REFINE_GUESS 0
#endif
#ifndef RVM_REFINE_RELAXED_COUNT
#define RVM_REFINE_RELAXED_COUNT 0
#endif

namespace rvm {

#ifdef RVM_PROFILE
#define RVM_RPROF_SLOTS 20
#define RVM_RPROF_MAX_WAVES 4096
static __device__ unsigned long long rvm_rprof[RVM_RPROF_MAX_WAVES * RVM_RPROF_SLOTS];
#define RPROF_T(v) const unsigned long long v = __builtin_readcyclecounter()
#define RPROF_RT(v) const unsigned long long v = __builtin_amdgcn_s_memrealtime()
#else
#define RPROF_T(v)
#define RPROF_RT(v)
#endif

__device__ __forceinline__ bool claim_item(gu64* w, unsigned long long gen, unsigned long long code) {
    unsigned long long v = __hip_atomic_load(w, __ATOMIC_RELAXED, __HIP_MEMORY_SCOPE_AGENT);
    for (;;) {
        if ((v >> 8) == gen) return false;
        unsigned long long expect = v;
        if (__hip_atomic_compare_exchange_strong(w, &expect, (gen << 8) | code, __ATOMIC_RELAXED, __ATOMIC_RELAXED,
                                                 __HIP_MEMORY_SCOPE_AGENT))
            return true;
        v = expect;
    }
}

__device__ __forceinline__ void hedge_mark_unneeded(const int32_t* rq_w, const int rq_cap,
                                                    const unsigned long long* htab, unsigned long long* hw_,
                                                    const int n0, const int n1, const int n2,
                                                    const unsigned long long gen, const int hedge, const int wpb) {
    const int lane = threadIdx.x & 63;
    unsigned need = 0;
    for (int l2 = 0; l2 < 3; l2++) {
        int n = l2 == 0 ? n0 : (l2 == 1 ? n1 : n2);
        n = n < rq_cap ? n : rq_cap;
        for (int i = lane; i < n; i += 64) {
            const int wl = rq_w[(size_t)l2 * rq_cap + i];
            if (wl < 0 || wl >= rq_cap) continue;
            const unsigned long long tb = __hip_atomic_load((gu64*)htab + wl, __ATOMIC_RELAXED, __HIP_MEMORY_SCOPE_AGENT);
            const int hg = (int)(tb & 0xFFFF) / wpb;
            if ((tb >> 16) != gen || hg >= RVM_HEDGE_GROUPS_MAX) continue;
            if (l2 != 2) need |= 1u << (2 * hg);
            if (l2 != 1) need |= 1u << (2 * hg + 1);
        }
    }
    for (int d = 32; d >= 1; d >>= 1) need |= (unsigned)__shfl_xor((int)need, d, 64);
    gu64* hw = (gu64*)hw_;
    const bool mark = lane < hedge && lane < 2 * RVM_HEDGE_GROUPS_MAX && !((need >> lane) & 1u);
    if (mark) __hip_atomic_store(hw + RVM_HW_MARK + lane, (gen << 8) | 1ull, __ATOMIC_RELAXED, __HIP_MEMORY_SCOPE_AGENT);
    const unsigned long long nm = __builtin_popcountll(ballot(mark));
    if (lane == 0 && nm)
        __hip_atomic_fetch_add(hw + RVM_HW_STATS + 3, nm, __ATOMIC_RELAXED, __HIP_MEMORY_SCOPE_AGENT);
}

__device__ __forceinline__ unsigned long long pass_ticks(const DevPlan& P, int rf) {
    const unsigned long long t = P.spin_ticks << (rf < RVM_RESOLVE_MAX_LIMIT ? rf : RVM_RESOLVE_MAX_LIMIT);
    constexpr unsigned long long cap = 6000000000ull;
    return t < cap ? t : (P.spin_ticks > cap ? P.spin_ticks : cap);
}

struct DirState {
    int open;
    double chi, lb, pest, best, bchi;
};

constexpr int RVM_REFINE_HM = 5;
template <int NP, bool D3, int NW>
__global__ __launch_bounds__((NW == RVM_REFINE_HM ? 4 : NW) * 64) void refine_kernel(
    const DevPlan P, const int W, const double* __restrict__ params, const double hill_factor,
    double* __restrict__ rv_out, double* __restrict__ logl_out, int32_t* __restrict__ status_out, const StretchArgs sa,
    const int eager, const int hedge) {
    constexpr bool HM = NW == RVM_REFINE_HM;
    constexpr int L = LanesPerWalker<NP>::value;
    constexpr int WPB = 64 / L;
    constexpr int PR = D3 ? 7 : 5;
    constexpr int R = PR * NP;
    const int wv = threadIdx.x >> 6;
    const int lane = threadIdx.x & 63;
    const int slot = lane / L;
    const int pl_idx = lane % L;
    const int nl = P.n_levels;
    RPROF_T(pt_entry);
    RPROF_RT(prt_entry);
#ifdef RVM_PROFILE
    unsigned long long p_seg = 0, p_epo = 0, p_steps = 0, p_wait = 0, p_pass = 0;
    int p_lvl = -1;
#endif

    __shared__ int s_n[3];
    __shared__ unsigned long long s_gen;
    __shared__ int s_depth;
    if (threadIdx.x == 0) {
        for (int i = 0; i < 3; i++) s_n[i] = __hip_atomic_load(P.rq_n + i, __ATOMIC_RELAXED, __HIP_MEMORY_SCOPE_AGENT);
        const unsigned long long g0 = __hip_atomic_load(P.gen_dev, __ATOMIC_RELAXED, __HIP_MEMORY_SCOPE_AGENT);
        s_gen = g0;
        int d = P.depth_w != nullptr ? 0 : RVM_TEAMS_MAX;
        if (P.depth_w != nullptr) {
            unsigned long long v[RVM_DEPTH_WINDOW];
#pragma unroll
            for (int i = 0; i < RVM_DEPTH_WINDOW; i++)
                v[i] = __hip_atomic_load(P.depth_w + (g0 + 1 + i) % (RVM_DEPTH_WINDOW + 1), __ATOMIC_RELAXED,
                                         __HIP_MEMORY_SCOPE_AGENT);
#pragma unroll
            for (int i = 0; i < RVM_DEPTH_WINDOW; i++)
                if ((v[i] >> 8) < g0 && (v[i] >> 8) + RVM_DEPTH_WINDOW >= g0 && (int)(v[i] & 0xFF) > d)
                    d = (int)(v[i] & 0xFF);
        }
        s_depth = d;
#if RVM_REFINE_RELAXED_COUNT
        asm volatile("s_waitcnt vmcnt(0)" ::: "memory");
        const int done = __hip_atomic_fetch_add(P.rq_n + 3, 1, __ATOMIC_RELAXED, __HIP_MEMORY_SCOPE_AGENT);
#else
        const int done = __hip_atomic_fetch_add(P.rq_n + 3, 1, __ATOMIC_ACQ_REL, __HIP_MEMORY_SCOPE_AGENT);
#endif
        if (done == (int)gridDim.x - 1) {
            for (int i = 0; i < 4; i++) __hip_atomic_store(P.rq_n + i, 0, __ATOMIC_RELAXED, __HIP_MEMORY_SCOPE_AGENT);
            if (!eager && !hedge) __hip_atomic_store(P.gen_dev, g0 + 1, __ATOMIC_RELAXED, __HIP_MEMORY_SCOPE_AGENT);
        }
    }
    __syncthreads();
    RPROF_T(pt_lists);
    const unsigned long long gen = s_gen;
    const int nq[3] = {s_n[0], s_n[1], s_n[2]};
    const int depth_hint = s_depth;
    const int gq0 = (nq[0] + WPB - 1) / WPB, gq1 = (nq[1] + WPB - 1) / WPB, gq2 = (nq[2] + WPB - 1) / WPB;
    const int ng = gq0 + gq1 + gq2;
    const int ntask_split = 2 * gq0 + gq1 + gq2;
    const int gfit = hedge && P.n_cu - hedge < (int)gridDim.x ? P.n_cu - hedge : (int)gridDim.x;
    auto leave = [&]() {
        if (hedge && threadIdx.x == 0) {
            gu64* hw = (gu64*)P.hw;
            if (__hip_atomic_fetch_add(hw + 1, 1ull, __ATOMIC_RELAXED, __HIP_MEMORY_SCOPE_AGENT) + 1 == gridDim.x) {
                __hip_atomic_store(hw + 1, 0ull, __ATOMIC_RELAXED, __HIP_MEMORY_SCOPE_AGENT);
                __hip_atomic_store(hw, (gen << 8) | 1ull, __ATOMIC_RELAXED, __HIP_MEMORY_SCOPE_AGENT);
            }
        }
    };
    const bool split = !eager && P.rq_x != nullptr && gq0 <= P.rq_xgroups && ((int)gridDim.x & 1) == 0 &&
                       ntask_split <= gfit;
    int nteam = 0;
    if (split && P.rq_t != nullptr && P.rvp != nullptr && P.rvp2 != nullptr && rv_out == nullptr &&
        ng <= P.rq_xgroups) {
        nteam = P.n_teams < P.rmax ? P.n_teams : P.rmax;
        if (nteam > (depth_hint > 2 ? depth_hint : 2)) nteam = depth_hint > 2 ? depth_hint : 2;
        while (nteam >= 2 && nteam * ntask_split > gfit) nteam--;
    }
    const bool team = nteam >= 2;
    const int ntask_team = nteam * ntask_split;
    const int ngw = (W + WPB - 1) / WPB;
    const bool esplit = eager && P.eager_split && P.rq_x != nullptr && ngw <= P.rq_xgroups &&
                        ((int)gridDim.x & 1) == 0 && 2 * ngw <= (int)gridDim.x;
    const int ntask = eager ? (esplit ? 2 * ngw : ngw) : (team ? ntask_team : (split ? ntask_split : ng));
    if ((int)blockIdx.x >= ntask) {
        if constexpr (HM) {
            if (hedge && blockIdx.x == gridDim.x - 1 && wv == 0)
                hedge_mark_unneeded(P.rq_w, P.rq_cap, P.htab, P.hw, nq[0], nq[1], nq[2], gen, hedge, WPB);
        }
        leave();
        return;
    }

    extern __shared__ double s_sched[];
    __shared__ double s_rv[2][2][RVM_MAX_LEVELS][64];
    __shared__ int s_enc[2][RVM_MAX_LEVELS][64];
    __shared__ double s_init[8][64];
    __shared__ double s_chi[2][64], s_lb[2][64];
    __shared__ double s_pest[2][64], s_best[2][64], s_bchi[2][64];
    __shared__ int s_open[2][64];
    __shared__ int s_live[64];
    __shared__ int s_stw[64];
    __shared__ double s_lpw[64];
    __shared__ double s_acc[3][64];
    __shared__ int s_dmode[64];
    __shared__ unsigned long long s_mask[2];
    __shared__ int s_xfault;
    __shared__ double s_tc2[2][64], s_te2[2][64];
    __shared__ int s_ter[2][64];
    __shared__ int s_cancel[2];
    __shared__ int s_eitems[64], s_eli[64], s_eany;
    __shared__ int s_emask;
    __shared__ int s_hix[2][64];
    __shared__ int s_skip[64];
    const int emax = P.fwd.n_epochs > P.bwd.n_epochs ? P.fwd.n_epochs : P.bwd.n_epochs;
    for (int dd = 0; dd < 2; dd++) {
        const DirSched& SD = dd ? P.bwd : P.fwd;
        double* b = s_sched + (size_t)dd * 4 * emax;
        const int ED = SD.n_epochs;
        int* bn = reinterpret_cast<int*>(b + 3 * ED);
        for (int i = threadIdx.x; i < ED; i += blockDim.x) {
            b[i] = SD.seg_h1[i];
            b[ED + i] = SD.obs_rv[i];
            b[2 * ED + i] = SD.obs_s2[i];
            bn[i] = SD.seg_n[i];
            bn[ED + i] = SD.obs_idx[i];
        }
    }
    RPROF_T(pt_sched);
    const bool stretch = sa.c != nullptr;
    const bool mh = sa.mh_scale != nullptr;
    const bool mapped = stretch || mh || sa.fd_x != nullptr;

    for (int t = blockIdx.x; t < ntask; t += gridDim.x) {
        int g = t, own = -1, tm = 0;
        if (team) {
            if (t < 2 * nteam * gq0) {
                g = t / (2 * nteam);
                const int r = t - g * 2 * nteam;
                own = r & 1;
                tm = r >> 1;
            } else {
                const int u = t - 2 * nteam * gq0;
                g = gq0 + u / nteam;
                tm = u - (u / nteam) * nteam;
            }
        } else if (esplit) {
            g = t >> 1;
            own = t & 1;
        } else if (split) {
            if (t < 2 * gq0) {
                g = t >> 1;
                own = t & 1;
            } else {
                g = t - gq0;
            }
        }
        int li = g < gq0 ? 0 : (g < gq0 + gq1 ? 1 : 2);
        const int base = (li == 0 ? g : (li == 1 ? g - gq0 : g - gq0 - gq1)) * WPB;
        int cnt = nq[li] - base < WPB ? nq[li] - base : WPB;
        const int* items = P.rq_w + (size_t)li * P.rq_cap + base;
        gu64* ef = eager ? (gu64*)(P.eflag + (size_t)g * RVM_EFLAG_WORDS) : nullptr;
        if (eager) {
            const int w0 = g * WPB;
            __syncthreads();
            if (threadIdx.x < 64) {
                s_eitems[threadIdx.x] = w0 + (int)threadIdx.x < W ? w0 + (int)threadIdx.x : w0;
                s_eli[threadIdx.x] = -1;
            }
            if (threadIdx.x == 0) s_eany = 0;
            __syncthreads();
            for (int l2 = 0; l2 < 3; l2++)
                for (int i = threadIdx.x; i < nq[l2]; i += blockDim.x) {
                    const int wl = P.rq_w[(size_t)l2 * P.rq_cap + i];
                    if (wl >= w0 && wl < w0 + WPB) {
                        s_eli[wl - w0] = l2;
                        s_eany = 1;
                    }
                }
            __syncthreads();
            if (!s_eany) {
                if (threadIdx.x == 0)
                    __hip_atomic_store(ef, (gen << 8) | 1ull, __ATOMIC_RELAXED, __HIP_MEMORY_SCOPE_AGENT);
                continue;
            }
            items = s_eitems;
            cnt = WPB;
        }
        const int wo = items[slot < cnt ? slot : 0];
        int kind = 0, wk = wo, jst = 0, jp = 0;
        double zst = 0.0, zp = 0.0;
        if (stretch) stretch_slot(sa, wo, kind, wk, zst, jst, zp, jp);
#ifdef RVM_PROFILE
        asm volatile("s_waitcnt vmcnt(0) lgkmcnt(0)" ::: "memory");
#endif
        RPROF_T(pt_slot);
        double rowv[R];
#pragma unroll
        for (int r = 0; r < R; r++) rowv[r] = walker_param(mapped, params, W, wk, sa, r, zst, jst, kind, zp, jp);
#ifdef RVM_PROFILE
        asm volatile("s_waitcnt vmcnt(0) lgkmcnt(0)" ::: "memory");
#endif
        RPROF_T(pt_rows);
        Lane<NP> s;
        int status = RVM_STATUS_OK;
        double e2w;
        walker_setup<NP, D3, L>(rowv, pl_idx, hill_factor, s, status, e2w);
        RPROF_T(pt_setup);
        __syncthreads();
        if (wv == 0) {
            s_init[0][lane] = s.rx;
            s_init[1][lane] = s.ry;
            s_init[2][lane] = s.vx;
            s_init[3][lane] = s.vy;
            s_init[4][lane] = s.rz;
            s_init[5][lane] = s.vz;
            s_init[6][lane] = s.r;
            s_init[7][lane] = s.ir;
            if (lane < WPB) {
                const int lli = eager ? s_eli[lane] : li;
                int skip = 0;
                if (P.skip_variants && stretch && sa.n_spec > 0 && sa.dec != nullptr && lane < cnt && lli >= 0) {
                    int k2 = 0, wk2 = 0, j2 = 0, jp2 = 0;
                    double z2 = 0.0, zp2 = 0.0;
                    stretch_slot(sa, items[lane], k2, wk2, z2, j2, zp2, jp2);
                    const long long jl = (long long)j2 - sa.s0_begin;
                    if (k2 != 0 && jl >= 0 && jl < sa.n_spec && P.rq_mark[jl] != (int32_t)gen)
                        skip = (k2 == 2) != (sa.dec[jl] == 1);
                }
                s_skip[lane] = skip;
                const bool v = lane < cnt && lli >= 0 && !skip;
                const int wl = items[lane < cnt ? lane : 0];
                const bool of = v && lli != 2, ob = v && lli != 1;
                s_open[0][lane] = of ? 1 : 0;
                s_open[1][lane] = ob ? 1 : 0;
                s_chi[0][lane] = of ? 0.0 : P.rq_c[wl];
                s_chi[1][lane] = ob ? 0.0 : P.rq_c[(size_t)P.rq_cap + wl];
                s_lb[0][lane] = s_chi[0][lane];
                s_lb[1][lane] = s_chi[1][lane];
                for (int d2i = 0; d2i < 2; d2i++) {
// ... 243 lines not shown
                                                                                 nullptr, (gen << 8) | 2ull, late);
                        else
                            segment_gated<D3, NP, L, RVM_REFINE_GUESS>(s, kq, r_len[e] * sc, ns, nt_r, late);
                    }
                    RPROF_T(pt_s1);
#ifdef RVM_PROFILE
                    p_seg += pt_s1 - pt_s0;
                    p_steps += (unsigned long long)ns;
#endif
                    if (work && here) {
                        const double v0 = star_vx<NP, L>(s);
                        if (pl_idx == 0) s_rv[dd_u][e & 1][k_u][slot] = v0;
                    }
                    if (bfirst && wv == 0 && lane == 0)
                        s_cancel[e & 1] = __hip_atomic_load(tdone, __ATOMIC_RELAXED, __HIP_MEMORY_SCOPE_AGENT) ==
                                          ((gen << 8) | 2ull);
                    __syncthreads();
                    if (bfirst && s_cancel[e & 1]) {
                        cancelled = true;
                        break;
                    }
                    if (cmb && here) {
                        double rvx = 0.0, rv3 = 0.0;
                        for (int q = 0; q < nl; q++) rvx += P.lw[q] * s_rv[dd_u][e & 1][q][lane];
                        for (int q = 1; q < nl; q++) rv3 += P.lw3[q] * s_rv[dd_u][e & 1][q][lane];
                        const double r = rvx - r_rv[e];
                        c2 += (r * r) / r_s2[e];
                        e2 += fabs((rvx - rv3) * (r + (rv3 - r_rv[e]))) / r_s2[e];
                        if (hasp) {
                            d2 += fabs((rvx - pv) * (r + (pv - r_rv[e]))) / r_s2[e];
                            if (team && tm < nteam - 1)
                                __hip_atomic_store((gu64*)(pp + (size_t)e * P.lvx_stride),
                                                   (unsigned long long)__double_as_longlong(rvx), __ATOMIC_RELAXED,
                                                   __HIP_MEMORY_SCOPE_AGENT);
                            else
                                pp[(size_t)e * P.lvx_stride] = rvx;
                        }
                        if (rv_out != nullptr) rv_out[(size_t)r_idx[e] * W + wme] = rvx;
                    }
#ifdef RVM_PROFILE
                    p_epo += __builtin_readcyclecounter() - pt_s1;
#endif
                }
#ifdef RVM_PROFILE
                if (work) {
                    p_pass++;
                    p_lvl = k;
                }
#endif
                if (cancelled) break;
                if (work && pl_idx == 0) s_enc[dd_u][k_u][slot] = (int)(((s.encm >> lane) & kick_enc_bits<NP>()) != 0);
                __syncthreads();
                if (bfirst) {
                    if (work && k == 0 && lane < WPB) {
                        int er = 0;
                        for (int q = 0; q < nl; q++) er |= s_enc[dd_u][q][lane];
                        s_tc2[dd_u][lane] = c2;
                        s_te2[dd_u][lane] = e2;
                        s_ter[dd_u][lane] = er;
                    }
                    continue;
                }
                if (work && k == 0 && lane < WPB) {
                    if ((need >> lane) & 1) {
                        int er = 0;
                        for (int q = 0; q < nl; q++) er |= s_enc[dd_u][q][lane];
                        pass_result(dd_u, rf, c2, e2, d2, er);
                    }
                    if (lane == 0 && need)
                        __hip_atomic_fetch_add(P.counters + 3, (unsigned long long)__builtin_popcountll(need),
                                               __ATOMIC_RELAXED, __HIP_MEMORY_SCOPE_AGENT);
                }
            }
            if (cancelled) break;
            rf_last = rf;
            RPROF_T(pt_w0);
            __syncthreads();
            if (emask != 0 && wv == 0) {
                const bool mine0 = (emask & 1) && lane < WPB && ((mk0 >> lane) & 1);
                const bool mine1 = (emask & 2) && lane < WPB && ((mk1 >> lane) & 1);
                gu64* f0 = hrep ? nullptr : ef + 2 + 2 * (rf - 1);
                const unsigned long long done = (gen << 8) | 2ull;
                SpinClock clk;
                clk.restart();
                bool ok = true;
                for (; !hrep;) {
                    const bool rdy = (!mine0 || __hip_atomic_load(f0, __ATOMIC_RELAXED, __HIP_MEMORY_SCOPE_AGENT) == done) &&
                                     (!mine1 || __hip_atomic_load(f0 + 1, __ATOMIC_RELAXED, __HIP_MEMORY_SCOPE_AGENT) == done);
                    if (ballot(!rdy) == 0) break;
                    if (clk.expired(pass_ticks(P, rf))) {
                        ok = false;
                        break;
                    }
                    __builtin_amdgcn_s_sleep(2);
                }
                __builtin_amdgcn_fence(__ATOMIC_ACQUIRE, "agent");
                if (!ok) {
                    if (lane == 0) {
                        s_xfault = 1;
                        __hip_atomic_fetch_add(P.counters, 1ull, __ATOMIC_RELAXED, __HIP_MEMORY_SCOPE_AGENT);
                    }
                } else {
                    for (int d3 = 0; d3 < 2; d3++) {
                        if (!(d3 ? mine1 : mine0)) continue;
                        const DirSched& SB = d3 ? P.bwd : P.fwd;
                        const int Eb = SB.n_epochs;
                        const double* b_dir = s_sched + (size_t)d3 * 4 * emax;
                        const double* b_rv = b_dir + Eb;
                        const double* b_s2 = b_dir + 2 * Eb;
                        const size_t plane = (size_t)P.lvx_emax * P.lvx_stride;
                        const size_t cst = hrep ? (size_t)RVM_HEDGE_STRIDE : (size_t)P.lvx_stride;
                        gu64* cur = hrep ? (gu64*)(P.hrv + (size_t)d3 * P.lvx_emax * RVM_HEDGE_STRIDE + s_hix[d3][lane])
                                         : (gu64*)(P.rve + ((size_t)(rf - 1) * 2 + d3) * plane + wme);
                        double* prv = P.rvp + (size_t)d3 * plane + wme;
                        double d2 = 0.0;
                        constexpr int RCH = 16;
                        for (int e0 = 0; e0 < Eb; e0 += RCH) {
                            double rvc[RCH], pvc[RCH];
#pragma unroll
                            for (int j = 0; j < RCH; j++) {
                                const int e = e0 + j < Eb ? e0 + j : Eb - 1;
                                rvc[j] = __longlong_as_double((long long)__hip_atomic_load(
                                    cur + (size_t)e * cst, __ATOMIC_RELAXED, __HIP_MEMORY_SCOPE_AGENT));
                                pvc[j] = prv[(size_t)e * P.lvx_stride];
                            }
#pragma unroll
                            for (int j = 0; j < RCH; j++) {
                                const int e = e0 + j;
                                if (e < Eb) {
                                    const double rvx = rvc[j], pv = pvc[j];
                                    const double r = rvx - b_rv[e];
                                    d2 += fabs((rvx - pv) * (r + (pv - b_rv[e]))) / b_s2[e];
                                    prv[(size_t)e * P.lvx_stride] = rvx;
                                }
                            }
                        }
                        gu64* es = hrep ? (gu64*)(P.hsum + (size_t)d3 * 3 * RVM_HEDGE_STRIDE + s_hix[d3][lane])
                                        : (gu64*)(P.esum + ((size_t)(rf - 1) * 2 + d3) * 3 * P.lvx_stride + wme);
                        auto ld = [&](size_t o) {
                            return __longlong_as_double((long long)__hip_atomic_load(es + o, __ATOMIC_RELAXED,
                                                                                     __HIP_MEMORY_SCOPE_AGENT));
                        };
                        pass_result(d3, rf, ld(0), ld(cst), d2, (int)ld(2 * cst));
                    }
                }
                if (lane == 0) {
                    const unsigned long long nd = ((emask & 1) ? __builtin_popcountll(mk0) : 0) +
                                                  ((emask & 2) ? __builtin_popcountll(mk1) : 0);
                    __hip_atomic_fetch_add(P.counters + 3, nd, __ATOMIC_RELAXED, __HIP_MEMORY_SCOPE_AGENT);
                }
            }
            if (bfirst) {
                if (wv == 0) {
                    SpinClock clk;
                    clk.restart();
                    unsigned long long f = 0;
                    bool ok = true;
                    while (((f = __hip_atomic_load(tpflag, __ATOMIC_RELAXED, __HIP_MEMORY_SCOPE_AGENT)) >> 8) != gen) {
                        if (__hip_atomic_load(tdone, __ATOMIC_RELAXED, __HIP_MEMORY_SCOPE_AGENT) == ((gen << 8) | 2ull)) {
                            f = (gen << 8) | 2ull;
                            break;
                        }
                        if (clk.expired(pass_ticks(P, tm))) {
                            ok = false;
                            break;
                        }
                        __builtin_amdgcn_s_sleep(2);
                    }
                    ok = __builtin_amdgcn_readfirstlane((int)ok) != 0;
                    f = __builtin_amdgcn_readfirstlane(f);
                    __builtin_amdgcn_fence(__ATOMIC_ACQUIRE, "agent");
                    if (!ok) {
                        if (lane == 0) {
                            s_xfault = 1;
                            __hip_atomic_fetch_add(P.counters, 1ull, __ATOMIC_RELAXED, __HIP_MEMORY_SCOPE_AGENT);
                        }
                    } else if ((f & 0xFF) == 2) {
                        if (lane == 0) s_cancel[0] = 1;
                    } else if (lane < WPB) {
                        unsigned long long row_v[15];
#pragma unroll
                        for (int rw = 0; rw < 15; rw++)
                            row_v[rw] = __hip_atomic_load(tprev + rw * 64 + lane, __ATOMIC_RELAXED, __HIP_MEMORY_SCOPE_AGENT);
                        auto ld = [&](int row) { return row_v[row]; };
                        s_live[lane] = (int)ld(0);
                        s_stw[lane] = (int)ld(1);
                        s_lpw[lane] = __longlong_as_double((long long)ld(2));
                        for (int d3 = 0; d3 < 2; d3++) {
                            s_open[d3][lane] = (int)ld(3 + 6 * d3);
                            s_chi[d3][lane] = __longlong_as_double((long long)ld(4 + 6 * d3));
                            s_lb[d3][lane] = __longlong_as_double((long long)ld(5 + 6 * d3));
                            s_pest[d3][lane] = __longlong_as_double((long long)ld(6 + 6 * d3));
                            s_best[d3][lane] = __longlong_as_double((long long)ld(7 + 6 * d3));
                            s_bchi[d3][lane] = __longlong_as_double((long long)ld(8 + 6 * d3));
                        }
                    }
                }
                __syncthreads();
                if (s_cancel[0]) {
                    cancelled = true;
                    break;
                }
                const double* rprev = tm == 1 ? P.rvp : P.rvp2 + (size_t)(tm - 2) * plane2;
                const double* rown = P.rvp2 + (size_t)(tm - 1) * plane2;
                for (int d3 = 0; d3 < 2; d3++) {
                    const bool mine = own < 0 ? (((d3 == 0 ? mk0 : mk1) != 0)) : d3 == own;
                    if (!mine || wv != 0 || lane >= WPB) continue;
                    const bool open_here = s_xfault == 0 && s_live[lane] != 0 && s_open[d3][lane] == 1;
                    const uint64_t needb = ballot(open_here);
                    if (open_here) {
                        const DirSched& SB = d3 ? P.bwd : P.fwd;
                        const int Eb = SB.n_epochs;
                        const double* b_dir = s_sched + (size_t)d3 * 4 * emax;
                        const double* b_rv = b_dir + Eb;
                        const double* b_s2 = b_dir + 2 * Eb;
                        const size_t off = (size_t)d3 * P.lvx_emax * P.lvx_stride + wme;
                        double d2b = 0.0;
                        constexpr int RCH = 16;
                        for (int e0 = 0; e0 < Eb; e0 += RCH) {
                            double pvc[RCH], rvc[RCH];
#pragma unroll
                            for (int j = 0; j < RCH; j++) {
                                const int e = e0 + j < Eb ? e0 + j : Eb - 1;
                                pvc[j] = __longlong_as_double((long long)__hip_atomic_load(
                                    (gu64*)(rprev + off + (size_t)e * P.lvx_stride), __ATOMIC_RELAXED,
                                    __HIP_MEMORY_SCOPE_AGENT));
                                rvc[j] = rown[off + (size_t)e * P.lvx_stride];
                            }
#pragma unroll
                            for (int j = 0; j < RCH; j++) {
                                const int e = e0 + j;
                                if (e < Eb) {
                                    const double pv = pvc[j], rvx = rvc[j];
                                    const double r = rvx - b_rv[e];
                                    d2b += fabs((rvx - pv) * (r + (pv - b_rv[e]))) / b_s2[e];
                                }
                            }
                        }
                        pass_result(d3, 1 + tm, s_tc2[d3][lane], s_te2[d3][lane], d2b, s_ter[d3][lane]);
                    }
                    if (lane == 0 && needb)
                        __hip_atomic_fetch_add(P.counters + 3, (unsigned long long)__builtin_popcountll(needb),
                                               __ATOMIC_RELAXED, __HIP_MEMORY_SCOPE_AGENT);
                }
                __syncthreads();
            }
            if (own >= 0 && wv == 0) {
                const size_t xb = ((size_t)(g * P.n_teams + tm) * 2) * 2 * 64;
                gu64* mine = (gu64*)(P.rq_x + xb + ((size_t)own * 2 + (rf & 1)) * 64);
                gu64* theirs = (gu64*)(P.rq_x + xb + ((size_t)(own ^ 1) * 2 + (rf & 1)) * 64);
                if (lane < WPB) {
                    const int o = s_open[own][lane];
                    const unsigned long long b =
                        o >= 2 ? slot_status(o == 2 ? RVM_STATUS_ENCOUNTER : RVM_STATUS_NONFINITE)
                               : (unsigned long long)__double_as_longlong(o == 1 ? -s_lb[own][lane] : s_chi[own][lane]);
                    __hip_atomic_store(mine + lane, b, __ATOMIC_RELAXED, __HIP_MEMORY_SCOPE_AGENT);
                }
                asm volatile("s_waitcnt vmcnt(0)" ::: "memory");
                const unsigned long long tag = (gen << 8) | (unsigned long long)rf;
                if (lane == 0)
                    __hip_atomic_store((gu64*)(P.rq_xf + ((size_t)g * P.n_teams + tm) * 2 + own), tag, __ATOMIC_RELAXED,
                                       __HIP_MEMORY_SCOPE_AGENT);
                gu64* tf = (gu64*)(P.rq_xf + ((size_t)g * P.n_teams + tm) * 2 + (own ^ 1));
                SpinClock clk;
                clk.restart();
                bool ok = true;
                while (__hip_atomic_load(tf, __ATOMIC_RELAXED, __HIP_MEMORY_SCOPE_AGENT) != tag) {
                    if (clk.expired(pass_ticks(P, rf))) {
                        ok = false;
                        break;
                    }
                    __builtin_amdgcn_s_sleep(2);
                }
                ok = __builtin_amdgcn_readfirstlane((int)ok) != 0;
                __builtin_amdgcn_fence(__ATOMIC_ACQUIRE, "agent");
                if (!ok) {
                    if (lane == 0) {
                        s_xfault = 1;
                        __hip_atomic_fetch_add(P.counters, 1ull, __ATOMIC_RELAXED, __HIP_MEMORY_SCOPE_AGENT);
                    }
                } else if (lane < WPB) {
                    const unsigned long long b = __hip_atomic_load(theirs + lane, __ATOMIC_RELAXED, __HIP_MEMORY_SCOPE_AGENT);
                    const int od = own ^ 1;
                    if (slot_is_status(b)) {
                        s_open[od][lane] = (b & 0xFF) == RVM_STATUS_NONFINITE ? 3 : 2;
                    } else {
                        const double v = __longlong_as_double((long long)b);
                        s_open[od][lane] = signbit(v) ? 1 : 0;
                        s_chi[od][lane] = fabs(v);
                        s_lb[od][lane] = fabs(v);
                    }
                }
            }
#ifdef RVM_PROFILE
            p_wait += __builtin_readcyclecounter() - pt_w0;
#endif
            if (wv == 0) {
                bool live = lane < WPB && s_live[lane] != 0;
                if (live) {
                    int stw, ncut;
                    double lp;
                    if (decide(dir_load(0), dir_load(1), rf, stw, lp, ncut)) {
                        if (ncut && own <= 0)
                            __hip_atomic_fetch_add(P.counters + 4, (unsigned long long)ncut, __ATOMIC_RELAXED,
                                                   __HIP_MEMORY_SCOPE_AGENT);
                        live = false;
                        s_live[lane] = 0;
                        s_stw[lane] = stw;
                        s_lpw[lane] = stw == RVM_STATUS_OK ? lp : -INFINITY;
                    }
                }
                uint64_t m0 = ballot(live && s_open[0][lane] == 1);
                uint64_t m1 = ballot(live && s_open[1][lane] == 1);
                if (hedge && team && tm == 0 && rf == 1 && own <= 0 && P.rmax >= 2 && (m0 | m1) != 0) {
                    const bool o0 = live && s_open[0][lane] == 1, o1 = live && s_open[1][lane] == 1;
                    const int hi[2] = {hedge_index(0, o0), hedge_index(1, o1)};
                    bool took = false;
                    if (ballot((o0 && hi[0] < 0) || (o1 && hi[1] < 0)) == 0) {
                        DirState q[2] = {dir_load(0), dir_load(1)};
                        bool fl[2] = {false, false};
                        for (int d3 = 0; d3 < 2; d3++) {
                            if (!(d3 ? o1 : o0)) continue;
                            const int Eb = (d3 ? P.bwd : P.fwd).n_epochs;
                            const double* b_dir = s_sched + (size_t)d3 * 4 * emax;
                            const double* b_rv = b_dir + Eb;
                            const double* b_s2 = b_dir + 2 * Eb;
                            const gu64* cur = (const gu64*)(P.hrv + (size_t)d3 * P.lvx_emax * RVM_HEDGE_STRIDE + hi[d3]);
                            const gu64* prv = (const gu64*)(P.rvp + (size_t)d3 * P.lvx_emax * P.lvx_stride + wme);
                            double d2 = 0.0;
                            constexpr int RCH = 16;
                            for (int e0 = 0; e0 < Eb; e0 += RCH) {
                                double rvc[RCH], pvc[RCH];
#pragma unroll
                                for (int j = 0; j < RCH; j++) {
                                    const int e = e0 + j < Eb ? e0 + j : Eb - 1;
                                    rvc[j] = __longlong_as_double((long long)__hip_atomic_load(
                                        cur + (size_t)e * RVM_HEDGE_STRIDE, __ATOMIC_RELAXED, __HIP_MEMORY_SCOPE_AGENT));
                                    pvc[j] = __longlong_as_double((long long)__hip_atomic_load(
                                        prv + (size_t)e * P.lvx_stride, __ATOMIC_RELAXED, __HIP_MEMORY_SCOPE_AGENT));
                                }
#pragma unroll
                                for (int j = 0; j < RCH; j++) {
                                    const int e = e0 + j;
                                    if (e < Eb) {
                                        const double rvx = rvc[j], pv = pvc[j];
                                        const double r = rvx - b_rv[e];
                                        d2 += fabs((rvx - pv) * (r + (pv - b_rv[e]))) / b_s2[e];
                                    }
                                }
                            }
                            const gu64* es = (const gu64*)(P.hsum + (size_t)d3 * 3 * RVM_HEDGE_STRIDE + hi[d3]);
                            auto ld = [&](size_t o) {
                                return __longlong_as_double((long long)__hip_atomic_load(es + o, __ATOMIC_RELAXED,
                                                                                         __HIP_MEMORY_SCOPE_AGENT));
                            };
                            fl[d3] = pass_eval(q[d3], 2, ld(0), ld(RVM_HEDGE_STRIDE), d2, (int)ld(2 * RVM_HEDGE_STRIDE));
                        }
                        int stw = RVM_STATUS_OK, ncut = 0;
                        double lp = 0.0;
                        const bool dn = live ? decide(q[0], q[1], 2, stw, lp, ncut) : true;
                        if (ballot(live && !dn) == 0) {
                            took = true;
                            if (live) {
                                if (o0) dir_store(0, q[0], fl[0]);
                                if (o1) dir_store(1, q[1], fl[1]);
                                if (ncut)
                                    __hip_atomic_fetch_add(P.counters + 4, (unsigned long long)ncut, __ATOMIC_RELAXED,
                                                           __HIP_MEMORY_SCOPE_AGENT);
                                live = false;
                                s_live[lane] = 0;
                                s_stw[lane] = stw;
                                s_lpw[lane] = stw == RVM_STATUS_OK ? lp : -INFINITY;
                            }
                            rf_last = 2;
                        }
                    }
                    if (lane == 0) {
                        const unsigned long long nd = __builtin_popcountll(m0) + __builtin_popcountll(m1);
                        if (took) __hip_atomic_fetch_add(P.counters + 3, nd, __ATOMIC_RELAXED, __HIP_MEMORY_SCOPE_AGENT);
                        __hip_atomic_fetch_add((gu64*)P.hw + RVM_HW_STATS + (took ? 1 : 2), nd, __ATOMIC_RELAXED,
                                               __HIP_MEMORY_SCOPE_AGENT);
                    }
                    if (took) m0 = m1 = 0;
                }
                if (lane == 0) {
                    s_mask[0] = m0;
                    s_mask[1] = m1;
                }
                if (team && tm < nteam - 1 && own <= 0) {
                    if (lane < WPB) {
                        auto st = [&](int row, unsigned long long v) {
                            __hip_atomic_store(tpub + row * 64 + lane, v, __ATOMIC_RELAXED, __HIP_MEMORY_SCOPE_AGENT);
                        };
                        auto bits = [](double v) { return (unsigned long long)__double_as_longlong(v); };
                        st(0, (unsigned long long)s_live[lane]);
                        st(1, (unsigned long long)(unsigned)s_stw[lane]);
                        st(2, bits(s_lpw[lane]));
                        for (int d3 = 0; d3 < 2; d3++) {
                            st(3 + 6 * d3, (unsigned long long)(unsigned)s_open[d3][lane]);
                            st(4 + 6 * d3, bits(s_chi[d3][lane]));
                            st(5 + 6 * d3, bits(s_lb[d3][lane]));
                            st(6 + 6 * d3, bits(s_pest[d3][lane]));
                            st(7 + 6 * d3, bits(s_best[d3][lane]));
                            st(8 + 6 * d3, bits(s_bchi[d3][lane]));
                        }
                    }
                    asm volatile("s_waitcnt vmcnt(0)" ::: "memory");
                    if (lane == 0) {
                        __hip_atomic_store(tflag, (gen << 8) | ((m0 | m1) == 0 ? 2ull : 1ull), __ATOMIC_RELAXED,
                                           __HIP_MEMORY_SCOPE_AGENT);
                        if ((m0 | m1) == 0)
                            __hip_atomic_store(tdone, (gen << 8) | 2ull, __ATOMIC_RELAXED, __HIP_MEMORY_SCOPE_AGENT);
                    }
                }
            }
            __syncthreads();
            if (team && tm < nteam - 1) {
                finisher = own <= 0 && (s_mask[0] | s_mask[1]) == 0;
                break;
            }
        }
        RPROF_T(pt_loop1);
        RPROF_RT(prt_loop1);
        if (team && tm == nteam - 1) finisher = own <= 0 && !cancelled;
        if (team && cancelled && tm < nteam - 1 && own <= 0 && threadIdx.x == 0)
            __hip_atomic_store(tflag, (gen << 8) | 2ull, __ATOMIC_RELAXED, __HIP_MEMORY_SCOPE_AGENT);
        if (finisher && threadIdx.x == 0 && P.depth_w != nullptr && rf_last > 0)
            __hip_atomic_fetch_max(P.depth_w + gen % (RVM_DEPTH_WINDOW + 1), (gen << 8) | (unsigned long long)rf_last,
                                   __ATOMIC_RELAXED,
                                   __HIP_MEMORY_SCOPE_AGENT);
        if (finisher && wv == 0 && lane < WPB && lane < cnt && s_skip[lane]) {
            logl_out[wme] = -INFINITY;
            status_out[wme] = RVM_STATUS_SKIPPED;
            __hip_atomic_fetch_add(P.counters + 6, 1ull, __ATOMIC_RELAXED, __HIP_MEMORY_SCOPE_AGENT);
        } else if (finisher && wv == 0 && lane < WPB && lane < cnt && (!eager || s_eli[lane] >= 0)) {
            int k2 = 0, wk2 = wme, j2 = 0, jp2 = 0;
            double z2 = 0.0, zp2 = 0.0;
            if (stretch) stretch_slot(sa, wme, k2, wk2, z2, j2, zp2, jp2);
            auto row = [&](int r) { return walker_param(mapped, params, W, wk2, sa, r, z2, j2, k2, zp2, jp2); };
            const double u3 = stretch ? stretch_u3(sa.seed, (uint64_t)(sa.s0_begin + wme), sa.iteration, sa.half)
                                      : (mh ? mh_u(sa.seed, (uint64_t)(sa.s0_begin + wme), sa.iteration) : 0.0);
            const double lnp0 = (stretch && k2 == 0) || mh ? sa.lnp[wme] : 0.0;
            walker_out<R>(P, sa, wme, s_stw[lane], s_lpw[lane], logl_out, status_out, row, z2, u3, lnp0);
        }
        if (eager && threadIdx.x == 0)
            __hip_atomic_store(ef, (gen << 8) | 1ull, __ATOMIC_RELAXED, __HIP_MEMORY_SCOPE_AGENT);
#ifdef RVM_PROFILE
        if (t == (int)blockIdx.x && lane == 0 && (size_t)blockIdx.x * 8 + wv < RVM_RPROF_MAX_WAVES / 2) {
            unsigned long long* o = rvm_rprof + ((size_t)blockIdx.x * 8 + wv) * RVM_RPROF_SLOTS;
            o[0] = prt_entry;
            o[1] = prt_loop0;
            o[2] = prt_loop1;
            o[3] = __builtin_amdgcn_s_memrealtime();
            o[4] = p_seg;
            o[5] = p_epo;
            o[6] = p_steps;
            o[7] = pt_loop0 - pt_entry;
            o[8] = pt_loop1 - pt_loop0;
            o[9] = (unsigned long long)t | ((unsigned long long)tm << 16) | ((unsigned long long)(own + 1) << 20) |
                   ((unsigned long long)(p_lvl + 1) << 24) | ((unsigned long long)(eager ? 1 : 0) << 28);
            o[10] = p_pass;
            o[11] = (unsigned long long)(unsigned)__builtin_amdgcn_s_getreg((31 << 11) | 4);
            o[12] = p_wait;
            o[13] = pt_lists - pt_entry;
            o[14] = pt_sched - pt_entry;
            o[15] = pt_setup - pt_entry;
            o[16] = pt_slot - pt_entry;
            o[17] = pt_rows - pt_entry;
        }
#endif
    }
    leave();
}

template <int NP, bool D3>
__global__ __launch_bounds__(256) void eager_kernel(const DevPlan P, const int W, const double* __restrict__ params,
                                                    const double hill_factor) {
    constexpr int L = LanesPerWalker<NP>::value;
    constexpr int WPB = 64 / L;
    constexpr int PR = D3 ? 7 : 5;
    constexpr int R = PR * NP;
    const int wv = threadIdx.x >> 6;
    const int lane = threadIdx.x & 63;
    const int slot = lane / L;
    const int pl_idx = lane % L;
    const int nl = P.n_levels;
    const int np2 = P.eager_passes == 2;
    const int g = blockIdx.x >> (1 + np2), dd = (blockIdx.x >> np2) & 1, rf = 1 + (np2 & blockIdx.x);
    const DirSched& SR = dd ? P.bwd : P.fwd;
    const int Er = SR.n_epochs;
    __shared__ double s_rv[2][RVM_MAX_LEVELS][64];
    __shared__ int s_enc[RVM_MAX_LEVELS][64];
    __shared__ int s_cancel[2];
    __shared__ unsigned long long s_gen;
    gu64* ef = (gu64*)(P.eflag + (size_t)g * RVM_EFLAG_WORDS);
    if (threadIdx.x == 0) s_gen = __hip_atomic_load(P.gen_dev, __ATOMIC_RELAXED, __HIP_MEMORY_SCOPE_AGENT);
    __syncthreads();
    const unsigned long long gen = s_gen;
    const unsigned long long ctag = (gen << 8) | 1ull;
    auto cancelled_now = [&]() {
        return __hip_atomic_load(ef, __ATOMIC_RELAXED, __HIP_MEMORY_SCOPE_AGENT) == ctag ||
               __hip_atomic_load(ef + 6 + dd, __ATOMIC_RELAXED, __HIP_MEMORY_SCOPE_AGENT) == ctag;
    };
    gu64* item = ef + 2 + 2 * (rf - 1) + dd;
    if (threadIdx.x == 0) s_cancel[0] = cancelled_now() || !claim_item(item, gen, 1ull);
    __syncthreads();
    if (s_cancel[0]) return;
    const int w0 = g * WPB;
    const int wo = w0 + slot < W ? w0 + slot : w0;
    double rowv[R];
#pragma unroll
    for (int r = 0; r < R; r++) rowv[r] = params[(size_t)r * W + wo];
    Lane<NP> s;
    int status = RVM_STATUS_OK;
    double e2w;
    walker_setup<NP, D3, L>(rowv, pl_idx, hill_factor, s, status, e2w);
    int k = wv < nl ? wv : -1;
    k = __builtin_amdgcn_readfirstlane(k);
    const int k_u = k < 0 ? 0 : k;
    const bool work = k >= 0;
    KickPrep<NP> kq{};
    if (work && Er > 0) kq = kick_prep<NP, L, D3>(s, 1.875);
    const int m_r = P.mult[k_u] << rf;
    const int nt_r = P.nt[k_u];
    const bool late = P.late_mult > 0 && m_r >= P.late_mult;
    const double sc = ldexp(P.inv_mult[k_u], -rf);
    const bool cmb = work && k == 0 && lane < WPB && w0 + lane < W;
    const size_t plane = (size_t)P.lvx_emax * P.lvx_stride;
    gu64* rvo = (gu64*)(P.rve + ((size_t)(rf - 1) * 2 + dd) * plane + (cmb ? w0 + lane : 0));
    double c2 = 0.0, e2 = 0.0;
    bool cancelled = false;
    for (int e = 0; e < Er; e++) {
        const int ns = __builtin_amdgcn_readfirstlane(work ? SR.seg_n[e] * m_r : 0);
        if (ns > 0) segment_gated<D3, NP, L, RVM_REFINE_GUESS>(s, kq, SR.seg_h1[e] * sc, ns, nt_r, late);
        if (work) {
            const double v0 = star_vx<NP, L>(s);
            if (pl_idx == 0) s_rv[e & 1][k_u][slot] = v0;
        }
        if (wv == 0 && lane == 0) s_cancel[e & 1] = cancelled_now();
        __syncthreads();
        if (s_cancel[e & 1]) {
            cancelled = true;
            break;
        }
        if (cmb) {
            double rvx = 0.0, rv3 = 0.0;
            for (int q = 0; q < nl; q++) rvx += P.lw[q] * s_rv[e & 1][q][lane];
            for (int q = 1; q < nl; q++) rv3 += P.lw3[q] * s_rv[e & 1][q][lane];
            const double ob = SR.obs_rv[e], s2 = SR.obs_s2[e];
            const double r = rvx - ob;
            c2 += (r * r) / s2;
            e2 += fabs((rvx - rv3) * (r + (rv3 - ob))) / s2;
            __hip_atomic_store(rvo + (size_t)e * P.lvx_stride, (unsigned long long)__double_as_longlong(rvx),
                               __ATOMIC_RELAXED, __HIP_MEMORY_SCOPE_AGENT);
        }
    }
    if (cancelled) return;
    if (work && pl_idx == 0) s_enc[k_u][slot] = (int)(((s.encm >> lane) & kick_enc_bits<NP>()) != 0);
    __syncthreads();
    if (wv == 0) {
        if (cmb) {
            int er = 0;
            for (int q = 0; q < nl; q++) er |= s_enc[q][lane];
            gu64* es = (gu64*)(P.esum + ((size_t)(rf - 1) * 2 + dd) * 3 * P.lvx_stride + w0 + lane);
            auto bits = [](double v) { return (unsigned long long)__double_as_longlong(v); };
            __hip_atomic_store(es, bits(c2), __ATOMIC_RELAXED, __HIP_MEMORY_SCOPE_AGENT);
            __hip_atomic_store(es + P.lvx_stride, bits(e2), __ATOMIC_RELAXED, __HIP_MEMORY_SCOPE_AGENT);
            __hip_atomic_store(es + 2 * (size_t)P.lvx_stride, bits((double)er), __ATOMIC_RELAXED,
                               __HIP_MEMORY_SCOPE_AGENT);
        }
        asm volatile("s_waitcnt vmcnt(0)" ::: "memory");
        if (lane == 0) __hip_atomic_store(item, (gen << 8) | 2ull, __ATOMIC_RELAXED, __HIP_MEMORY_SCOPE_AGENT);
    }
}

template <int NPV, bool D3V>
static hipError_t launch_eager_t(const DevPlan& P, int W, const double* params, double hill_factor, hipStream_t st) {
    constexpr int wpb = 64 / LanesPerWalker<NPV>::value;
    const int groups = (W + wpb - 1) / wpb;
    eager_kernel<NPV, D3V><<<dim3(2 * P.eager_passes * groups), dim3(256), 0, st>>>(P, W, params, hill_factor);
    return hipGetLastError();
}

template <int NP, bool D3>
__global__ __launch_bounds__(256) void hedge_kernel(const DevPlan P, const int W, const double hill_factor,
                                                    const StretchArgs sa, const int ngrp, const int skip) {
    constexpr int L = LanesPerWalker<NP>::value;
    constexpr int WPB = 64 / L;
    constexpr int PR = D3 ? 7 : 5;
    constexpr int R = PR * NP;
    const int tid = threadIdx.x;
    const int wv = threadIdx.x >> 6;
    const int lane = threadIdx.x & 63;
    const int slot = lane / L;
    const int pl_idx = lane % L;
    const int nl = P.n_levels;
    const int g = blockIdx.x >> 1, dd = blockIdx.x & 1;
    const DirSched& SR = dd ? P.bwd : P.fwd;
    const int Er = SR.n_epochs;
    extern __shared__ unsigned long long s_key[];
    __shared__ double s_rv[2][RVM_MAX_LEVELS][64];
    __shared__ int s_enc[RVM_MAX_LEVELS][64];
    __shared__ int s_cnt[2][256];
    __shared__ unsigned long long s_ck[RVM_HEDGE_CAND];
    __shared__ int s_ci[RVM_HEDGE_CAND];
    __shared__ int s_sel[64];
    __shared__ int s_cancel[2];
    __shared__ unsigned long long s_gen, s_pref;
    __shared__ int s_need;
#ifdef RVM_PROFILE
    const unsigned long long prt_entry = __builtin_amdgcn_s_memrealtime();
#endif
    gu64* hw = (gu64*)P.hw;
    if (tid == 0) s_gen = __hip_atomic_load(P.gen_dev, __ATOMIC_RELAXED, __HIP_MEMORY_SCOPE_AGENT);
    __syncthreads();
    const unsigned long long gen = s_gen;
    const unsigned long long ctag = (gen << 8) | 1ull;
    __shared__ int s_marked;
    auto stopped = [&]() {
        const bool mk = __hip_atomic_load(hw + RVM_HW_MARK + blockIdx.x, __ATOMIC_RELAXED, __HIP_MEMORY_SCOPE_AGENT) == ctag;
        if (mk) s_marked = 1;
        return mk || __hip_atomic_load(hw, __ATOMIC_RELAXED, __HIP_MEMORY_SCOPE_AGENT) == ctag;
    };
    if (tid == 0) {
        s_marked = 0;
        s_cancel[0] = stopped();
    }
    __syncthreads();
    auto count_marked = [&]() {
        if (tid == 0 && s_marked)
            __hip_atomic_fetch_add(hw + RVM_HW_STATS + 4, 1ull, __ATOMIC_RELAXED, __HIP_MEMORY_SCOPE_AGENT);
    };
    if (s_cancel[0]) {
        count_marked();
        return;
    }
    const unsigned long long kbad = ~0ull;
    for (int i = tid; i < RVM_HEDGE_CAND; i += 256) {
        s_ck[i] = kbad;
        s_ci[i] = 0;
    }
    for (int i = tid; i < W; i += 256) {
        int kind = 0, wk = i, jst = 0, jp = 0;
        double zst = 0.0, zp = 0.0;
        stretch_slot(sa, i, kind, wk, zst, jst, zp, jp);
        double sc = INFINITY;
        bool ok = true;
#pragma unroll
        for (int p = 0; p < NP; p++) {
            const double m = walker_param(true, nullptr, W, wk, sa, PR * p + 0, zst, jst, kind, zp, jp);
            const double a = walker_param(true, nullptr, W, wk, sa, PR * p + 1, zst, jst, kind, zp, jp);
            const double h = walker_param(true, nullptr, W, wk, sa, PR * p + 2, zst, jst, kind, zp, jp);
            const double k = walker_param(true, nullptr, W, wk, sa, PR * p + 3, zst, jst, kind, zp, jp);
            const double e = sqrt(h * h + k * k);
            ok = ok && a > 0.02 && m > 5e-6 && e < 1.0;
            sc = fmin(sc, a * (1.0 - e) / cbrt(1.0 + m));
        }
        ok = ok && isfinite(sc) && sc > 0.0;
        s_key[i] = ok ? (unsigned long long)__double_as_longlong(sc) : kbad;
    }
    auto scan256 = [&](int* c) {
        const int c0 = c[4 * lane], c1 = c[4 * lane + 1], c2 = c[4 * lane + 2], c3 = c[4 * lane + 3];
        int inc = c0 + c1 + c2 + c3;
        for (int d = 1; d < 64; d <<= 1) {
            const int v = __shfl_up(inc, d, 64);
            if (lane >= d) inc += v;
        }
        const int ex = inc - (c0 + c1 + c2 + c3);
        c[4 * lane] = ex;
        c[4 * lane + 1] = ex + c0;
        c[4 * lane + 2] = ex + c0 + c1;
        c[4 * lane + 3] = ex + c0 + c1 + c2;
    };
    const int want = skip + ngrp * WPB;
    const int kq = want < W ? want : W;
    if (tid == 0) {
        s_pref = 0;
        s_need = kq;
    }
    for (int rd = 7; rd >= 0; rd--) {
        const int sh = 8 * rd;
        s_cnt[0][tid] = 0;
        __syncthreads();
        const unsigned long long pref = s_pref;
        const unsigned long long hi = rd == 7 ? 0ull : (~0ull << (sh + 8));
        for (int i = tid; i < W; i += 256) {
            const unsigned long long key = s_key[i];
            if ((key & hi) == pref) atomicAdd(&s_cnt[0][(int)((key >> sh) & 255)], 1);
        }
        __syncthreads();
        if (wv == 0) {
            const int need = s_need;
            const int c0 = s_cnt[0][4 * lane], c1 = s_cnt[0][4 * lane + 1], c2 = s_cnt[0][4 * lane + 2],
                      c3 = s_cnt[0][4 * lane + 3];
            int inc = c0 + c1 + c2 + c3;
            for (int d = 1; d < 64; d <<= 1) {
                const int v = __shfl_up(inc, d, 64);
                if (lane >= d) inc += v;
            }
            int ex = inc - (c0 + c1 + c2 + c3);
            if (ex < need && need <= inc) {
                int b = 0;
                if (need > ex + c0) {
                    ex += c0;
                    b = 1;
                    if (need > ex + c1) {
                        ex += c1;
                        b = 2;
                        if (need > ex + c2) {
                            ex += c2;
                            b = 3;
                        }
                    }
                }
                s_pref = pref | ((unsigned long long)(4 * lane + b) << sh);
                s_need = need - ex;
            }
        }
        __syncthreads();
    }
    const unsigned long long kth = s_pref;
    const int ntie = kth == kbad ? 0 : s_need;
    const int nless = kq - s_need;
    const int nsel = nless + ntie;
    const int per = (W + 255) / 256;
    const int i0 = tid * per < W ? tid * per : W, i1 = i0 + per < W ? i0 + per : W;
    {
        int a = 0, b = 0;
        for (int i = i0; i < i1; i++) {
            const unsigned long long key = s_key[i];
            a += key < kth ? 1 : 0;
            b += key == kth ? 1 : 0;
        }
        s_cnt[0][tid] = a;
        s_cnt[1][tid] = b;
    }
    __syncthreads();
    if (wv == 0) {
        scan256(s_cnt[0]);
        scan256(s_cnt[1]);
    }
    __syncthreads();
    {
        int a = s_cnt[0][tid], b = s_cnt[1][tid];
        for (int i = i0; i < i1; i++) {
            const unsigned long long key = s_key[i];
            int pos = -1;
            if (key < kth) {
                pos = a++;
            } else if (key == kth) {
                if (b < ntie) pos = nless + b;
                b++;
            }
            if (pos >= 0 && pos < RVM_HEDGE_CAND) {
                s_ck[pos] = key;
                s_ci[pos] = i;
            }
        }
    }
    __syncthreads();
    const int r0 = skip + g * WPB;
    const int cnt = nsel - r0 < WPB ? nsel - r0 : WPB;
    if (cnt <= 0) return;
    for (int c = tid; c < nsel; c += 256) {
        const unsigned long long key = s_ck[c];
        int rk = 0;
        for (int o = 0; o < nsel; o++) rk += (s_ck[o] < key || (s_ck[o] == key && o < c)) ? 1 : 0;
        if (rk >= r0 && rk < r0 + WPB) s_sel[rk - r0] = s_ci[c];
    }
    __syncthreads();
    if (wv == 0 && lane < cnt) {
        const int hx = g * WPB + lane;
        __hip_atomic_store((gu64*)P.htab + s_sel[lane], (gen << 16) | (unsigned long long)hx, __ATOMIC_RELAXED,
                           __HIP_MEMORY_SCOPE_AGENT);
        __hip_atomic_store((gu64*)P.hslot + (size_t)dd * RVM_HEDGE_STRIDE + hx,
                           (gen << 16) | (unsigned long long)s_sel[lane], __ATOMIC_RELAXED, __HIP_MEMORY_SCOPE_AGENT);
    }
    if (tid == 0 && dd == 0)
        __hip_atomic_fetch_add(hw + RVM_HW_STATS, (unsigned long long)cnt, __ATOMIC_RELAXED, __HIP_MEMORY_SCOPE_AGENT);
    const int wo = s_sel[slot < cnt ? slot : 0];
    int kind = 0, wk = wo, jst = 0, jp = 0;
    double zst = 0.0, zp = 0.0;
    stretch_slot(sa, wo, kind, wk, zst, jst, zp, jp);
    double rowv[R];
#pragma unroll
    for (int r = 0; r < R; r++) rowv[r] = walker_param(true, nullptr, W, wk, sa, r, zst, jst, kind, zp, jp);
    Lane<NP> s;
    int status = RVM_STATUS_OK;
    double e2w;
    walker_setup<NP, D3, L>(rowv, pl_idx, hill_factor, s, status, e2w);
    int k = wv < nl ? wv : -1;
    k = __builtin_amdgcn_readfirstlane(k);
    const int k_u = k < 0 ? 0 : k;
    const bool work = k >= 0;
    KickPrep<NP> kq0{};
    if (work && Er > 0) kq0 = kick_prep<NP, L, D3>(s, 1.875);
    constexpr int rf = 2;
    const int m_r = P.mult[k_u] << rf;
    const int nt_r = P.nt[k_u];
    const bool late = P.late_mult > 0 && m_r >= P.late_mult;
    const double sc = ldexp(P.inv_mult[k_u], -rf);
    const bool cmb = work && k == 0 && lane < cnt;
    const int hx = g * WPB + (cmb ? lane : 0);
    gu64* rvo = (gu64*)(P.hrv + (size_t)dd * P.lvx_emax * RVM_HEDGE_STRIDE + hx);
    double c2 = 0.0, e2 = 0.0;
    bool cancelled = false;
#ifdef RVM_PROFILE
    const unsigned long long prt_loop0 = __builtin_amdgcn_s_memrealtime();
#endif
    for (int e = 0; e < Er; e++) {
        const int ns = __builtin_amdgcn_readfirstlane(work ? SR.seg_n[e] * m_r : 0);
        if (ns > 0)
            (void)segment_gated_c<D3, NP, L, RVM_REFINE_GUESS>(s, kq0, SR.seg_h1[e] * sc, ns, nt_r, hw, nullptr, ctag, late);
        if (work) {
            const double v0 = star_vx<NP, L>(s);
            if (pl_idx == 0) s_rv[e & 1][k_u][slot] = v0;
        }
        if (wv == 0 && lane == 0) s_cancel[e & 1] = stopped();
        __syncthreads();
        if (s_cancel[e & 1]) {
            cancelled = true;
            break;
        }
        if (cmb) {
            double rvx = 0.0, rv3 = 0.0;
            for (int q = 0; q < nl; q++) rvx += P.lw[q] * s_rv[e & 1][q][lane];
            for (int q = 1; q < nl; q++) rv3 += P.lw3[q] * s_rv[e & 1][q][lane];
            const double ob = SR.obs_rv[e], s2 = SR.obs_s2[e];
            const double r = rvx - ob;
            c2 += (r * r) / s2;
            e2 += fabs((rvx - rv3) * (r + (rv3 - ob))) / s2;
            __hip_atomic_store(rvo + (size_t)e * RVM_HEDGE_STRIDE, (unsigned long long)__double_as_longlong(rvx),
                               __ATOMIC_RELAXED, __HIP_MEMORY_SCOPE_AGENT);
        }
    }
#ifdef RVM_PROFILE
    if (lane == 0 && RVM_RPROF_MAX_WAVES / 2 + (size_t)blockIdx.x * 8 + wv < RVM_RPROF_MAX_WAVES) {
        unsigned long long* o = rvm_rprof + (RVM_RPROF_MAX_WAVES / 2 + (size_t)blockIdx.x * 8 + wv) * RVM_RPROF_SLOTS;
        o[0] = prt_entry;
        o[1] = prt_loop0;
        o[2] = __builtin_amdgcn_s_memrealtime();
        o[3] = o[2];
        o[9] = (unsigned long long)blockIdx.x | (1ull << 29) | ((unsigned long long)(cancelled ? 1 : 0) << 30);
        o[10] = cancelled ? 0 : 1;
        o[11] = (unsigned long long)(unsigned)__builtin_amdgcn_s_getreg((31 << 11) | 4);
    }
#endif
    if (cancelled) {
        count_marked();
        return;
    }
    if (work && pl_idx == 0) s_enc[k_u][slot] = (int)(((s.encm >> lane) & kick_enc_bits<NP>()) != 0);
    __syncthreads();
    if (wv == 0) {
        if (__builtin_amdgcn_readfirstlane((int)stopped())) {
            count_marked();
            return;
        }
        if (cmb) {
            int er = 0;
            for (int q = 0; q < nl; q++) er |= s_enc[q][lane];
            gu64* es = (gu64*)(P.hsum + (size_t)dd * 3 * RVM_HEDGE_STRIDE + hx);
            auto bits = [](double v) { return (unsigned long long)__double_as_longlong(v); };
            __hip_atomic_store(es, bits(c2), __ATOMIC_RELAXED, __HIP_MEMORY_SCOPE_AGENT);
            __hip_atomic_store(es + RVM_HEDGE_STRIDE, bits(e2), __ATOMIC_RELAXED, __HIP_MEMORY_SCOPE_AGENT);
            __hip_atomic_store(es + 2 * RVM_HEDGE_STRIDE, bits((double)er), __ATOMIC_RELAXED, __HIP_MEMORY_SCOPE_AGENT);
        }
        asm volatile("s_waitcnt vmcnt(0)" ::: "memory");
        if (lane == 0)
            __hip_atomic_store(hw + 2 + 2 * g + dd, (gen << 8) | 2ull, __ATOMIC_RELAXED, __HIP_MEMORY_SCOPE_AGENT);
    }
}

template <int NPV, bool D3V>
static size_t hedge_budget() {
    static size_t budget[64] = {};
    static bool known[64] = {};
    int dev = 0;
    if (hipGetDevice(&dev) != hipSuccess || dev < 0 || dev >= 64) {
        (void)hipGetLastError();
        return 0;
    }
    if (!known[dev]) {
        const void* f = reinterpret_cast<const void*>(&hedge_kernel<NPV, D3V>);
        hipFuncAttributes fa{};
        size_t b = 0;
        if (hipFuncGetAttributes(&fa, f) == hipSuccess && fa.sharedSizeBytes < (size_t)RVM_LDS_PER_CU) {
            const size_t lim = (size_t)RVM_LDS_PER_CU - fa.sharedSizeBytes;
            if (hipFuncSetAttribute(f, hipFuncAttributeMaxDynamicSharedMemorySize, (int)lim) == hipSuccess) b = lim;
        }
        (void)hipGetLastError();
        budget[dev] = b;
        known[dev] = true;
    }
    return budget[dev];
}

template <int NPV, bool D3V>
static int hedge_groups_t(const DevPlan& P, int W, int logl_blocks) {
    constexpr int wpb = 64 / LanesPerWalker<NPV>::value;
    if (P.hedge_groups <= 0 || P.hw == nullptr || P.rvp == nullptr || P.rmax < 2 || P.n_levels > 4 || W < 1 ||
        W > RVM_HEDGE_MAX_W || W > P.rq_cap || (size_t)W * sizeof(unsigned long long) > hedge_budget<NPV, D3V>())
        return 0;
    const int idle = P.n_cu - logl_blocks;
    int n = std::min(P.hedge_groups, idle / 2);
    n = std::min(n, (W + wpb - 1) / wpb);
    return n > 0 ? n : 0;
}

template <int NPV, bool D3V>
static hipError_t launch_hedge_t(const DevPlan& P, int W, double hill_factor, const StretchArgs& sa, int ngrp,
                                 hipStream_t st) {
    constexpr int wpb = 64 / LanesPerWalker<NPV>::value;
    const int skip = W >= 2 * (ngrp + 1) * wpb ? wpb : 0;
    hedge_kernel<NPV, D3V><<<dim3(2 * ngrp), dim3(256), hedge_budget<NPV, D3V>(), st>>>(P, W, hill_factor, sa, ngrp, skip);
    return hipGetLastError();
}

template <int NPV, bool D3V, int NW>
static size_t refine_budget() {
    static size_t budget[64] = {};
    int dev = 0;
    if (hipGetDevice(&dev) != hipSuccess || dev < 0 || dev >= 64) {
        (void)hipGetLastError();
        return 32 * 1024;
    }
    if (budget[dev] == 0) {
        const void* f = reinterpret_cast<const void*>(&refine_kernel<NPV, D3V, NW>);
        hipFuncAttributes fa{};
        size_t b = 32 * 1024;
        if (hipFuncGetAttributes(&fa, f) == hipSuccess && fa.sharedSizeBytes < (size_t)RVM_LDS_PER_CU) {
            const size_t lim = (size_t)RVM_LDS_PER_CU - fa.sharedSizeBytes;
            if (hipFuncSetAttribute(f, hipFuncAttributeMaxDynamicSharedMemorySize, (int)lim) == hipSuccess) b = lim;
        }
        (void)hipGetLastError();
        budget[dev] = b;
    }
    return budget[dev];
}

template <int NPV, bool D3V>
static hipError_t launch_refine_t(const DevPlan& P, int W, const double* params, double hill_factor, double* logl,
                                  int32_t* status, double* rv_out, const StretchArgs& sa, int eager, int hedge,
                                  hipStream_t stream) {
    constexpr int wpb = 64 / LanesPerWalker<NPV>::value;
    const int emax = P.fwd.n_epochs > P.bwd.n_epochs ? P.fwd.n_epochs : P.bwd.n_epochs;
    const size_t smem = (size_t)emax * 8 * sizeof(double);
    static const bool w4_env = [] {
        const char* e = getenv("RVM_REFINE_W4");
        return !(e && e[0] == '0');
    }();
    const bool w4 = P.n_levels <= 4 && w4_env;
    if (smem > (w4 ? refine_budget<NPV, D3V, 4>() : refine_budget<NPV, D3V, 8>())) return hipErrorInvalidConfiguration;
    const int groups = (W + wpb - 1) / wpb + 2;
    int nb = std::max(2, std::min(P.n_cu > 0 ? P.n_cu : 256, 2 * groups));
    nb &= ~1;
    if (w4 && hedge && P.hedge_mark && smem <= refine_budget<NPV, D3V, RVM_REFINE_HM>())
        refine_kernel<NPV, D3V, RVM_REFINE_HM><<<dim3(nb), dim3(256), smem, stream>>>(P, W, params, hill_factor, rv_out,
                                                                                      logl, status, sa, eager, hedge);
    else if (w4)
        refine_kernel<NPV, D3V, 4><<<dim3(nb), dim3(256), smem, stream>>>(P, W, params, hill_factor, rv_out, logl, status,
                                                                          sa, eager, hedge);
    else
        refine_kernel<NPV, D3V, 8><<<dim3(nb), dim3(512), smem, stream>>>(P, W, params, hill_factor, rv_out, logl, status,
                                                                          sa, eager, hedge);
    return hipGetLastError();
}

template <int NPV, bool D3V>
static hipError_t prepare_refine_t(const DevPlan& P) {
    const int emax = P.fwd.n_epochs > P.bwd.n_epochs ? P.fwd.n_epochs : P.bwd.n_epochs;
    const size_t smem = (size_t)emax * 8 * sizeof(double);
    const size_t b = std::min(refine_budget<NPV, D3V, 4>(), refine_budget<NPV, D3V, 8>());
    if (P.hedge_groups > 0) (void)hedge_budget<NPV, D3V>();
    if (P.hedge_groups > 0 && P.hedge_mark) (void)refine_budget<NPV, D3V, RVM_REFINE_HM>();
    return smem <= b ? hipSuccess : hipErrorInvalidConfiguration;
}

#define RVM_REFINE_NP_API(N)                                                                                     \
    hipError_t launch_refine_np##N(const DevPlan& P, int W, const double* params, double hill_factor, double* logl, \
                                   int32_t* status, double* rv_out, const StretchArgs& sa, int eager, int hedge, \
                                   hipStream_t stream);                                                          \
    int hedge_groups_np##N(const DevPlan& P, int W, int logl_blocks);                                           \
    hipError_t launch_hedge_np##N(const DevPlan& P, int W, double hill_factor, const StretchArgs& sa, int ngrp, \
                                  hipStream_t stream);                                                           \
    hipError_t launch_eager_np##N(const DevPlan& P, int W, const double* params, double hill_factor,            \
                                  hipStream_t stream);                                                           \
    hipError_t prepare_refine_np##N(const DevPlan& P);
RVM_REFINE_NP_API(1)
RVM_REFINE_NP_API(2)
RVM_REFINE_NP_API(3)
RVM_REFINE_NP_API(4)
#undef RVM_REFINE_NP_API

}
```

rvel-mcmc_amd/rvmcmc/_lib.py:

```python
from __future__ import annotations

import ctypes as C
import os

_HERE = os.path.dirname(os.path.abspath(__file__))
LIB_PATH = os.environ.get("RVM_LIB_PATH") or os.path.join(_HERE, "librvmcmc.so")

RVM_STATUS_OK = 0
RVM_STATUS_PRIOR = 1
RVM_STATUS_ENCOUNTER = 2
RVM_STATUS_NONFINITE = 3
RVM_STATUS_UNRESOLVED = 4
RVM_STATUS_SKIPPED = 5
RVM_MAX_PLANETS = 4
RVM_MAX_LEVELS = 6
RVM_N_COUNTERS = 7
ABI_VERSION = 12


class RvmConfig(C.Structure):
    _fields_ = [
        ("n_planets", C.c_int32),
        ("dt", C.c_double),
        ("n_levels", C.c_int32),
        ("npoints_norm", C.c_double),
        ("level_mult", C.c_int32 * RVM_MAX_LEVELS),
        ("period_hint", C.c_double),
        ("inclined", C.c_int32),
        ("resolve_tol", C.c_double),
        ("resolve_max", C.c_int32),
    ]


RVM_SMALA_MAX_PARAMS = 20
RVM_MAX_PARAM_ROWS = 7 * RVM_MAX_PLANETS


class ParamMapC(C.Structure):
    _fields_ = [
        ("n_rows", C.c_int32),
        ("src", C.c_int32 * RVM_MAX_PARAM_ROWS),
        ("base", C.c_double * RVM_MAX_PARAM_ROWS),
    ]


class SmalaCache(C.Structure):
    _fields_ = [(k, C.c_void_p) for k in ("lp", "grad", "mu", "L", "G", "logdet", "ok")]


class RvmError(RuntimeError):
    pass


_dp = C.c_void_p
SIGNATURES = {
    "rvm_abi_version": (C.c_int, []),
    "rvm_smala_derive": (C.c_int, [C.c_int32, C.c_int32, C.c_int32, _dp, C.c_double, _dp, _dp, _dp, _dp, _dp,
                                   C.c_double, C.c_double, C.c_double, C.POINTER(SmalaCache), _dp]),
    "rvm_smala_metric": (C.c_int, [C.c_int32, C.c_int32, _dp, _dp, _dp, _dp, _dp, C.c_double, C.c_double,
                                   C.POINTER(SmalaCache), _dp]),
    "rvm_smala_propose": (C.c_int, [C.c_int32, C.c_int32, C.c_int64, _dp, C.POINTER(SmalaCache), C.c_double,
                                    C.c_uint64, C.c_uint64, _dp, _dp, _dp]),
    "rvm_smala_accept": (C.c_int, [C.c_int32, C.c_int32, C.c_int64, _dp, C.POINTER(SmalaCache), _dp,
                                   C.POINTER(SmalaCache), C.c_double, C.c_uint64, C.c_uint64, _dp, _dp, _dp, _dp]),
    "rvm_smala_stencil_logl": (C.c_int, [C.c_void_p, C.POINTER(ParamMapC), C.c_int32, C.c_int32, _dp, C.c_double,
                                         _dp, C.c_double, _dp, _dp, _dp, _dp]),
    "rvm_smala_derive_accept": (C.c_int, [C.c_int32, C.c_int32, C.c_int64, C.c_int32, _dp, _dp, C.c_double, _dp, _dp,
                                          _dp, _dp, _dp, C.c_double, C.c_double, C.c_double, C.POINTER(SmalaCache),
                                          C.POINTER(SmalaCache), C.c_uint64, C.c_uint64, _dp, _dp, _dp, _dp]),
    "rvm_smala_derive_sides": (C.c_int, [C.c_int32, C.c_int32, C.c_int32, _dp, C.c_double, _dp, _dp, _dp, _dp, _dp,
                                         C.c_double, C.c_double, C.c_double, C.POINTER(SmalaCache), _dp]),
    "rvm_smala_center_accept": (C.c_int, [C.c_int32, C.c_int32, C.c_int64, _dp, _dp, _dp, _dp, C.POINTER(SmalaCache),
                                          C.POINTER(SmalaCache), C.c_double, C.c_uint64, C.c_uint64, _dp, _dp, _dp,
                                          _dp]),
    "rvm_smala_metric_accept": (C.c_int, [C.c_int32, C.c_int32, C.c_int64, _dp, _dp, _dp, _dp, _dp, _dp, C.c_double,
                                          C.c_double, C.POINTER(SmalaCache), C.POINTER(SmalaCache), C.c_uint64,
                                          C.c_uint64, _dp, _dp, _dp, _dp]),
    "rvm_last_error": (C.c_char_p, []),
    "rvm_plan_create": (C.c_int, [C.POINTER(RvmConfig), C.POINTER(C.c_double), C.POINTER(C.c_double),
                                  C.POINTER(C.c_double), C.c_int32, C.c_int32, C.POINTER(C.c_void_p)]),
    "rvm_plan_destroy": (None, [C.c_void_p]),
    "rvm_plan_faults": (C.c_int, [C.c_void_p, C.c_int32, C.POINTER(C.c_int64), C.POINTER(C.c_int64),
                                  C.POINTER(C.c_int64), C.POINTER(C.c_int64), C.POINTER(C.c_int64), _dp]),
    "rvm_plan_set_handoff_timeout": (C.c_int, [C.c_void_p, C.c_double]),
    "rvm_plan_time_kernels": (C.c_int, [C.c_void_p, C.c_int32]),
    "rvm_plan_kernel_times": (C.c_int, [C.c_void_p, C.POINTER(C.c_float), C.POINTER(C.c_float), C.c_int32,
                                        C.POINTER(C.c_int32)]),
    "rvm_plan_extension": (C.c_int, [C.c_void_p, C.POINTER(C.c_int32)]),
    "rvm_plan_set_verify_eccentricity": (C.c_int, [C.c_void_p, C.c_double]),
    "rvm_plan_set_certain_reject": (C.c_int, [C.c_void_p, C.c_int32]),
    "rvm_plan_counters": (C.c_int, [C.c_void_p, C.c_int32, C.POINTER(C.c_int64), C.c_int32, C.c_void_p]),
    "rvm_plan_hedge_stats": (C.c_int, [C.c_void_p, C.c_int32, C.POINTER(C.c_int64), C.POINTER(C.c_int64),
                                       C.POINTER(C.c_int64), C.c_void_p]),
    "rvm_plan_hedge_marks": (C.c_int, [C.c_void_p, C.c_int32, C.POINTER(C.c_int64), C.POINTER(C.c_int64), C.c_void_p]),
    "rvm_plan_info": (C.c_int, [C.c_void_p, C.POINTER(C.c_int32), C.POINTER(C.c_int32), C.POINTER(C.c_int32),
                                C.POINTER(C.c_int32)]),
    "rvm_logl_batch": (C.c_int, [C.c_void_p, C.c_int32, _dp, C.c_double, _dp, _dp, _dp, _dp]),
    "rvm_stretch_propose": (C.c_int, [C.c_int32, C.c_int32, C.c_int64, _dp, C.c_int32, _dp, C.c_double, C.c_uint64,
                                      C.c_uint64, C.c_uint32, _dp, _dp, _dp, _dp]),
    "rvm_stretch_accept": (C.c_int, [C.c_int32, C.c_int32, C.c_int64, _dp, _dp, _dp, _dp, _dp, C.c_uint64, C.c_uint64,
                                     C.c_uint32, _dp, _dp, _dp]),
    "rvm_pt_stretch_propose": (C.c_int, [C.c_int32, C.c_int32, C.c_int32, _dp, _dp, C.c_double, C.c_uint64,
                                         C.c_uint64, C.c_uint32, _dp, _dp, _dp, _dp]),
    "rvm_pt_stretch_accept": (C.c_int, [C.c_int32, C.c_int32, C.c_int32, _dp, _dp, _dp, _dp, _dp, _dp, C.c_uint64,
                                        C.c_uint64, C.c_uint32, _dp, _dp, _dp]),
    "rvm_pt_swap": (C.c_int, [C.c_int32, C.c_int32, C.c_int32, _dp, _dp, _dp, _dp, _dp, C.c_uint64, C.c_uint64, _dp,
                              _dp, _dp]),
    "rvm_pt_ladder_update": (C.c_int, [C.c_int32, C.c_int32, _dp, _dp, _dp, C.c_double, _dp, _dp, _dp, _dp, _dp, _dp,
                                       _dp]),
    "rvm_stretch_half_step": (C.c_int, [C.c_void_p, C.POINTER(ParamMapC), C.c_int32, C.c_int32, C.c_int64, _dp, _dp,
                                        _dp, C.c_int32, _dp, C.c_double, C.c_uint64, C.c_uint64, C.c_uint32,
                                        C.c_double, _dp, _dp, _dp, _dp]),
    "rvm_stretch_iteration_begin": (C.c_int, [C.c_void_p, C.POINTER(ParamMapC), C.c_int32, C.c_int32, C.c_int64,
                                              C.c_int64, _dp, _dp, _dp, _dp, C.c_int32, _dp, _dp, C.c_double, C.c_uint64,
                                              C.c_uint64, C.c_double, _dp, _dp, _dp, _dp, _dp]),
    "rvm_stretch_iteration_end": (C.c_int, [C.c_int32, C.c_int32, C.c_int64, C.c_int64, _dp, _dp, _dp, _dp, _dp,
                                            _dp, _dp, C.c_int32, _dp, _dp, _dp, _dp, C.c_double, C.c_uint64,
                                            C.c_uint64, _dp, _dp, _dp, _dp]),
    "rvm_mh_propose": (C.c_int, [C.c_int32, C.c_int32, C.c_int64, _dp, _dp, C.c_double, C.c_uint64, C.c_uint64, _dp,
                                 _dp, _dp]),
    "rvm_mh_accept": (C.c_int, [C.c_int32, C.c_int32, C.c_int64, _dp, _dp, _dp, _dp, C.c_uint64, C.c_uint64, _dp, _dp,
                                _dp]),
    "rvm_mh_step": (C.c_int, [C.c_void_p, C.POINTER(ParamMapC), C.c_int32, C.c_int32, C.c_int64, _dp, _dp, _dp,
                              C.c_double, C.c_uint64, C.c_uint64, C.c_double, _dp, _dp, _dp, _dp]),
    "rvm_chain_record": (C.c_int, [C.c_int32, C.c_int32, _dp, C.c_int64, C.c_int64, C.c_int64, _dp, C.c_int64,
                                   C.c_int64, _dp, _dp, _dp]),
    "rvm_chain_moments": (C.c_int, [_dp, C.c_int32, C.c_int32, C.c_int64, C.c_int64, _dp, _dp, _dp]),
    "rvm_chain_autocov_workspace_bytes": (C.c_size_t, [C.c_int32, C.c_int32, C.c_int32]),
    "rvm_chain_autocov": (C.c_int, [_dp, _dp, C.c_int32, C.c_int32, C.c_int64, C.c_int64, C.c_int32, C.c_int32, _dp,
                                    _dp, _dp]),
    "rvm_fd_params": (C.c_int, [C.c_int32, C.c_int32, _dp, C.c_double, _dp, _dp, _dp]),
    "rvm_logl_derivs_workspace_bytes": (C.c_size_t, [C.c_int32, C.c_int32]),
    "rvm_logl_derivs": (C.c_int, [C.c_void_p, C.c_int32, _dp, C.c_int32, C.POINTER(C.c_int32), C.c_double, _dp, _dp,
                                  _dp, _dp, _dp, _dp]),
}

_lib = None


def load():
    global _lib
    if _lib is not None:
        return _lib
    if not os.path.exists(LIB_PATH):
        raise RvmError(
            f"librvmcmc.so not found at {LIB_PATH}: build it with `make -C rvel-mcmc_amd` "
            "(or __graft_entry__.build()); there is no CPU fallback")
    try:
        lib = C.CDLL(LIB_PATH)
    except OSError as e:
        raise RvmError(f"failed to load {LIB_PATH}: {e}") from e
    for name, (res, args) in SIGNATURES.items():
        fn = getattr(lib, name)
        fn.restype = res
        fn.argtypes = args
    if lib.rvm_abi_version() != ABI_VERSION:
        raise RvmError("librvmcmc.so ABI version mismatch")
    _lib = lib
    return lib


def check(rc: int, what: str):
    if rc != 0:
        msg = load().rvm_last_error()
        raise RvmError(f"{what} failed ({rc}): {msg.decode() if msg else ''}")


def stream_handle(stream=None) -> int:
    import torch

    s = stream if stream is not None else torch.cuda.current_stream()
    return int(s.cuda_stream)
```

rvel-mcmc_amd/rvmcmc/engine.py:

```python
from __future__ import annotations

import ctypes as C
import math
from dataclasses import dataclass
from typing import Optional

import numpy as np

from . import _lib

KERNEL_KEYS = ("m", "a", "h", "k", "l")
KERNEL_KEYS_INCLINED = KERNEL_KEYS + ("ix", "iy")
SUPPORTED_KEYS = set(KERNEL_KEYS_INCLINED)


def level_multipliers(levels) -> tuple:
    if isinstance(levels, (int, np.integer)):
        mult = tuple(range(1, int(levels) + 1))
    else:
        mult = tuple(int(m) for m in levels)
    if not 1 <= len(mult) <= _lib.RVM_MAX_LEVELS:
        raise ValueError(f"1..{_lib.RVM_MAX_LEVELS} Richardson levels supported, got {len(mult)}")
    if len(set(mult)) != len(mult) or min(mult) < 1 or max(mult) > 64:
        raise ValueError("level multipliers must be distinct integers in 1..64")
    return mult


DT_GRID = 16
ECC_GRID = 64


@dataclass(frozen=True)
class IntegratorConfig:

    steps_per_orbit: float = 8.0
    levels: tuple = (4, 5, 6, 7)
    dt: Optional[float] = None
    resolve_tol: float = 5e-7
    resolve_max: int = 12
    verify_speedup: float = 1.1
    certain_reject: bool = True

    @property
    def mult(self) -> tuple:
        return level_multipliers(self.levels)

    @property
    def n_levels(self) -> int:
        return len(self.mult)

    def step_for(self, planets) -> float:
        if self.dt is not None:
            return float(self.dt)
        raw = min_period(planets) / float(self.steps_per_orbit)
        return 2.0 ** (round(math.log2(raw) * DT_GRID) / DT_GRID)

    def resolve(self, planets=None) -> tuple:
        return float(self.resolve_tol), int(self.resolve_max), self.ecc_guard(planets), bool(self.certain_reject)

    def ecc_guard(self, planets) -> float:
        if not planets or not (self.verify_speedup > 0.0) or not (self.resolve_tol > 0.0):
            return 0.0
        e_ref = max(float(np.hypot(p.get("h", 0.0), p.get("k", 0.0))) for p in planets)
        e_ref = round(e_ref * ECC_GRID) / ECC_GRID
        if not e_ref < 1.0:
            return 0.0
        return float(1.0 - (self.verify_speedup * (1.0 - e_ref) ** -1.5) ** (-2.0 / 3.0))

    def plan_args(self, planets):
        dt = self.step_for(planets)
        hint = dt * float(self.steps_per_orbit) if self.dt is None else min_period(planets)
        return dt, self.mult, hint


def is_inclined(planets) -> bool:
    return any(("ix" in p) or ("iy" in p) for p in planets)


DEFAULT_CONFIG = IntegratorConfig()


def min_period(planets) -> float:
    best = math.inf
    for p in planets:
        a = float(p["a"])
        m = float(p.get("m", 0.0))
        if a > 0:
            best = min(best, 2.0 * math.pi * math.sqrt(a ** 3 / (1.0 + max(m, 0.0))))
    if not math.isfinite(best):
        raise ValueError("cannot derive an integrator step: no planet with a > 0")
    return best


def _torch():
    import torch

    return torch


def default_device():
    torch = _torch()
    if not torch.cuda.is_available():
        raise _lib.RvmError("no HIP device visible: the likelihood runs only on the GPU (no CPU fallback)")
    return torch.device("cuda", torch.cuda.current_device())


class LoglPlan:

    def __init__(self, t, rv, sigma, npoints, n_planets, dt, levels=4, max_walkers=4096, device=None,
                 period_hint=0.0, inclined=False, resolve=(0.0, 0)):
        torch = _torch()
        self.lib = _lib.load()
        self.device = torch.device(device) if device is not None else default_device()
        t = np.ascontiguousarray(np.asarray(t, dtype=np.float64))
        rv = np.ascontiguousarray(np.asarray(rv, dtype=np.float64))
        sigma = np.ascontiguousarray(np.asarray(sigma, dtype=np.float64))
        if not (len(t) == len(rv) == len(sigma)):
            raise ValueError("t, rv and sigma must have the same length")
        self.n_obs = len(t)
        self.n_planets = int(n_planets)
        self.dt = float(dt)
        self.mult = level_multipliers(levels)
        self.n_levels = len(self.mult)
        self.period_hint = float(period_hint)
        self.inclined = bool(inclined)
        self.rows = (7 if self.inclined else 5) * self.n_planets
        self.npoints = float(npoints)
        self.max_walkers = int(max_walkers)
        self.resolve_tol, self.resolve_max = float(resolve[0]), int(resolve[1])
        self.ecc_guard = float(resolve[2]) if len(resolve) > 2 else 0.0
        self.certain_reject = bool(resolve[3]) if len(resolve) > 3 else True
        lm = (C.c_int32 * _lib.RVM_MAX_LEVELS)(*self.mult)
        cfg = _lib.RvmConfig(self.n_planets, self.dt, self.n_levels, self.npoints, lm, self.period_hint,
                             int(self.inclined), self.resolve_tol, self.resolve_max)
        handle = C.c_void_p()
        dp = C.POINTER(C.c_double)
        with torch.cuda.device(self.device):
            rc = self.lib.rvm_plan_create(C.byref(cfg), t.ctypes.data_as(dp), rv.ctypes.data_as(dp),
                                          sigma.ctypes.data_as(dp), self.n_obs, self.max_walkers, C.byref(handle))
        _lib.check(rc, "rvm_plan_create")
        self._h = handle
        ext = C.c_int32()
        _lib.check(self.lib.rvm_plan_extension(self._h, C.byref(ext)), "rvm_plan_extension")
        self.ext_mult = ext.value
        if self.ecc_guard > 0.0:
            _lib.check(self.lib.rvm_plan_set_verify_eccentricity(self._h, self.ecc_guard),
                       "rvm_plan_set_verify_eccentricity")
        if not self.certain_reject:
            _lib.check(self.lib.rvm_plan_set_certain_reject(self._h, 0), "rvm_plan_set_certain_reject")

    def faults(self, reset=False, stream=None) -> dict:
        vals = (C.c_int64 * _lib.RVM_N_COUNTERS)()
        _lib.check(self.lib.rvm_plan_counters(self._h, int(bool(reset)), vals, _lib.RVM_N_COUNTERS,
                                              _lib.stream_handle(stream)), "rvm_plan_counters")
        f = dict(handoff_timeouts=vals[0], nonfinite=vals[1], unresolved=vals[2], refined=vals[3],
                 truncated=vals[4], floor_settled=vals[5], skipped=vals[6])
        if reset:
            tot = self.__dict__.setdefault("totals", dict.fromkeys(f, 0))
            for k, v in f.items():
                tot[k] += v
        return f

    def hedge_stats(self, reset=False, stream=None) -> dict:
        h, r, m = C.c_int64(), C.c_int64(), C.c_int64()
        _lib.check(self.lib.rvm_plan_hedge_stats(self._h, int(bool(reset)), C.byref(h), C.byref(r), C.byref(m),
                                                 _lib.stream_handle(stream)), "rvm_plan_hedge_stats")
        return dict(hedged=h.value, replayed=r.value, missed=m.value)

    def hedge_marks(self, reset=False, stream=None) -> dict:
        m, g = C.c_int64(), C.c_int64()
        _lib.check(self.lib.rvm_plan_hedge_marks(self._h, int(bool(reset)), C.byref(m), C.byref(g),
                                                 _lib.stream_handle(stream)), "rvm_plan_hedge_marks")
        return dict(marked=m.value, gave_up=g.value)

    def check_faults(self, what="plan", stream=None, group=None) -> dict:
        f = self.faults(reset=True, stream=stream)
        bad = [f["handoff_timeouts"], f["nonfinite"], f["unresolved"] if self.resolve_max > 0 else 0]
        if group is not None:
            torch = _torch()
            dist = torch.distributed
            dev = self.device if dist.get_backend(group) == "nccl" else torch.device("cpu")
            t = torch.tensor(bad, dtype=torch.int64, device=dev)
            dist.all_reduce(t, group=group)
            bad = [int(v) for v in t.cpu()]
        if any(bad):
            raise _lib.RvmError(f"{what}: {bad[0]} level-split hand-off timeout(s), {bad[1]} non-finite "
                                f"log-likelihood(s), {bad[2]} walker(s) not resolved to the plan's tolerance after "
                                f"{self.resolve_max} halvings on the GPU (rvm_plan_faults"
                                f"{', summed over the ranks' if group is not None else ''})")
        return f

    def time_kernels(self, max_launches):
        _lib.check(self.lib.rvm_plan_time_kernels(self._h, int(max_launches)), "rvm_plan_time_kernels")

    def kernel_times(self, max_launches=4096):
        a = (C.c_float * max_launches)()
        b = (C.c_float * max_launches)()
        n = C.c_int32()
        _lib.check(self.lib.rvm_plan_kernel_times(self._h, a, b, int(max_launches), C.byref(n)), "rvm_plan_kernel_times")
        return np.array(a[:n.value], dtype=np.float64), np.array(b[:n.value], dtype=np.float64)

    def set_handoff_timeout(self, seconds):
        _lib.check(self.lib.rvm_plan_set_handoff_timeout(self._h, float(seconds)), "rvm_plan_set_handoff_timeout")

    def info(self):
        vals = [C.c_int32() for _ in range(4)]
        _lib.check(self.lib.rvm_plan_info(self._h, *[C.byref(v) for v in vals]), "rvm_plan_info")
        return dict(steps_fwd=vals[0].value, steps_bwd=vals[1].value, epochs_fwd=vals[2].value,
                    epochs_bwd=vals[3].value)

    def logl(self, params, hill_factor=1.0, want_rv=False, out=None, status=None, rv_out=None, stream=None):
        torch = _torch()
        if params.dtype != torch.float64 or params.device != self.device or params.dim() != 2:
            raise ValueError("params must be a 2-D float64 tensor on the plan's device")
        if params.shape[0] != self.rows:
            raise ValueError(f"params must have {self.rows} rows (m,a,h,k,l{',ix,iy' if self.inclined else ''} "
                             f"per planet)")
        params = params.contiguous()
        W = params.shape[1]
        if W > self.max_walkers:
            raise ValueError(f"{W} walkers exceed the plan's max_walkers={self.max_walkers}")
        if out is None:
            out = torch.empty(W, dtype=torch.float64, device=self.device)
        if status is None:
            status = torch.empty(W, dtype=torch.int32, device=self.device)
        rvp = 0
        if want_rv:
            if rv_out is None:
                rv_out = torch.empty((self.n_obs, W), dtype=torch.float64, device=self.device)
            rvp = rv_out.data_ptr()
        with torch.cuda.device(self.device):
            rc = self.lib.rvm_logl_batch(self._h, W, params.data_ptr(), float(hill_factor), out.data_ptr(),
                                         status.data_ptr(), rvp, _lib.stream_handle(stream))
        _lib.check(rc, "rvm_logl_batch")
        return out, status, (rv_out if want_rv else None)

    def derivs(self, params, dir_rows, hill_factor=1.0, stream=None):
        torch = _torch()
        if params.dtype != torch.float64 or params.device != self.device or params.dim() != 2:
            raise ValueError("params must be a 2-D float64 tensor on the plan's device")
        if params.shape[0] != self.rows:
            raise ValueError(f"params must have {self.rows} rows")
        params = params.contiguous()
        C_ = params.shape[1]
        rows = np.ascontiguousarray(np.asarray(dir_rows, dtype=np.int32))
        P = len(rows)
        f64 = dict(dtype=torch.float64, device=self.device)
        lp = torch.empty(C_, **f64)
        grad = torch.empty((P, C_), **f64)
        hess = torch.empty((P, P, C_), **f64)
        st = torch.empty(C_, dtype=torch.int32, device=self.device)
        nb = int(self.lib.rvm_logl_derivs_workspace_bytes(C_, P))
        ws = torch.empty(max(nb, 8), dtype=torch.uint8, device=self.device)
        with torch.cuda.device(self.device):
            rc = self.lib.rvm_logl_derivs(self._h, C_, params.data_ptr(), P, rows.ctypes.data_as(C.POINTER(C.c_int32)),
                                          float(hill_factor), lp.data_ptr(), grad.data_ptr(), hess.data_ptr(),
                                          st.data_ptr(), ws.data_ptr(), _lib.stream_handle(stream))
        _lib.check(rc, "rvm_logl_derivs")
        return lp, grad, hess, st

    def stretch_half_step(self, pmap, X0, lnp0, c_aos, s0_begin, a, seed, iteration, half, hill_factor=1.0,
                          lnp_new=None, status=None, accepted=None, X0_aos=None, stream=None):
        torch = _torch()
        for t in (X0, lnp0, c_aos) + ((X0_aos,) if X0_aos is not None else ()):
            if t.dtype != torch.float64 or t.device != self.device or not t.is_contiguous():
                raise ValueError("X0, lnp0, c_aos, X0_aos must be contiguous float64 tensors on the plan's device")
        dim, n0 = X0.shape
        if c_aos.dim() != 2 or c_aos.shape[1] != dim or lnp0.shape != (n0,):
            raise ValueError("shape mismatch between X0 [dim][n0], lnp0 [n0] and c_aos [n1][dim]")
        if X0_aos is not None and X0_aos.shape != (n0, dim):
            raise ValueError("X0_aos must be [n0][dim]")
        if n0 > self.max_walkers:
            raise ValueError(f"{n0} walkers exceed the plan's max_walkers={self.max_walkers}")
        with torch.cuda.device(self.device):
            rc = self.lib.rvm_stretch_half_step(
                self._h, C.byref(pmap.c_map()), dim, n0, int(s0_begin), X0.data_ptr(),
                X0_aos.data_ptr() if X0_aos is not None else 0, lnp0.data_ptr(), c_aos.shape[0], c_aos.data_ptr(),
                float(a), int(seed), int(iteration), int(half), float(hill_factor),
                lnp_new.data_ptr() if lnp_new is not None else 0, status.data_ptr() if status is not None else 0,
                accepted.data_ptr() if accepted is not None else 0, _lib.stream_handle(stream))
        _lib.check(rc, "rvm_stretch_half_step")

    def stretch_iteration_begin(self, pmap, X0, lnp0, X1, c0_aos, c1_aos, s0_begin, s1_begin, a, seed, iteration,
                                lnp_spec, status_spec, dec, hill_factor=1.0, accepted0=None, stream=None, lnp1=None):
        torch = _torch()
        for t in (X0, lnp0, X1, c0_aos, c1_aos, lnp_spec):
            if t.dtype != torch.float64 or t.device != self.device or not t.is_contiguous():
                raise ValueError("X0, lnp0, X1, c0_aos, c1_aos, lnp_spec must be contiguous float64 tensors on the "
                                 "plan's device")
        dim, n = X0.shape
        n_half = c0_aos.shape[0]
        if X1.shape != (dim, n) or lnp0.shape != (n,) or c0_aos.shape != (n_half, dim) or c1_aos.shape != (n_half, dim):
            raise ValueError("shape mismatch between X0/X1 [dim][n], lnp0 [n] and c0_aos/c1_aos [n_half][dim]")
        if lnp_spec.shape != (3 * n,) or status_spec.shape != (3 * n,) or dec.shape != (n,):
            raise ValueError("lnp_spec / status_spec must be [3 n], dec [n]")
        if lnp1 is not None and (lnp1.dtype != torch.float64 or lnp1.device != self.device or lnp1.shape != (n,)
                                 or not lnp1.is_contiguous()):
            raise ValueError("lnp1 must be a contiguous float64 [n] tensor on the plan's device")
        if status_spec.dtype != torch.int32 or dec.dtype != torch.int32:
            raise ValueError("status_spec and dec must be int32")
        if 3 * n > self.max_walkers:
            raise ValueError(f"3 x {n} walker slots exceed the plan's max_walkers={self.max_walkers}")
        with torch.cuda.device(self.device):
            rc = self.lib.rvm_stretch_iteration_begin(
                self._h, C.byref(pmap.c_map()), dim, n, int(s0_begin), int(s1_begin), X0.data_ptr(), lnp0.data_ptr(),
                X1.data_ptr(), lnp1.data_ptr() if lnp1 is not None else 0, n_half, c0_aos.data_ptr(), c1_aos.data_ptr(),
                float(a), int(seed), int(iteration),
                float(hill_factor), lnp_spec.data_ptr(), status_spec.data_ptr(), dec.data_ptr(),
                accepted0.data_ptr() if accepted0 is not None else 0, _lib.stream_handle(stream))
        _lib.check(rc, "rvm_stretch_iteration_begin")

    def close(self):
        if getattr(self, "_h", None) is not None and self._h.value:
            self.lib.rvm_plan_destroy(self._h)
            self._h = C.c_void_p()

    def __del__(self):
        try:
            self.close()
        except Exception:
            pass


def stretch_iteration_end(X0, X0_aos, dec, dec_all, X1, X1_aos, lnp1, c0_aos, c1_aos, lnp_spec, status_spec,
                          s0_begin, s1_begin, a, seed, iteration, accepted1=None, lnp_new=None, status_new=None,
                          stream=None):
    torch = _torch()
# ... 136 lines not shown
```

Baseline: 3.127 million.

## Let refine teams wait briefly for in-flight hedge results before refining

Adds a bounded hedge-wait path: when a refine team finds its walkers' hedge slots still running, it polls the hedge group state and takes the hedged result if it finishes, giving way when the partner team reaches its barrier or a quarter-spin timeout expires. Cancelled hedge blocks now publish a stop state so waiters can exit early, and the hedge-mark variant kernel is launched whenever hedging is on rather than only when marking is enabled. The hedge key computation is also restructured to batch several walkers per thread with all loads issued before the math. The aim is to avoid redundant refine work that a hedge block is about to finish, at the cost of extra spinning, new atomics and more register pressure.

```diff
diff --git a/include/rvmcmc.h b/include/rvmcmc.h
--- a/include/rvmcmc.h
+++ b/include/rvmcmc.h
@@ -55,6 +55,8 @@
 int rvm_plan_hedge_stats(rvm_plan* plan, int32_t reset, int64_t* hedged, int64_t* replayed, int64_t* missed,
                          void* stream);
 int rvm_plan_hedge_marks(rvm_plan* plan, int32_t reset, int64_t* marked, int64_t* gave_up, void* stream);
+int rvm_plan_hedge_waits(rvm_plan* plan, int32_t reset, int64_t* waited, int64_t* late_hits, int64_t* gave_way,
+                         void* stream);
 int rvm_plan_time_kernels(rvm_plan* plan, int32_t max_launches);
 int rvm_plan_kernel_times(rvm_plan* plan, float* logl_ms, float* refine_ms, int32_t max, int32_t* n_out);
 int rvm_plan_set_handoff_timeout(rvm_plan* plan, double seconds);
diff --git a/rvel-mcmc_amd/csrc/host_sanitize.cpp b/rvel-mcmc_amd/csrc/host_sanitize.cpp
--- a/rvel-mcmc_amd/csrc/host_sanitize.cpp
+++ b/rvel-mcmc_amd/csrc/host_sanitize.cpp
@@ -46,7 +46,8 @@
 static const char* const kKnobNames[] = {
     "RVM_SKIP_VARIANTS", "RVM_LATE_SPO",   "RVM_NO_LEVEL_SPLIT", "RVM_REFINE_TEAMS", "RVM_EAGER_SPLIT",
     "RVM_NO_EXTENSION",  "RVM_REFINE_SPLIT", "RVM_TEAMS_HINT",   "RVM_EAGER",        "RVM_EAGER_PASSES",
-    "RVM_HEDGE",         "RVM_HEDGE_GROUPS", "RVM_HEDGE_MARK",   "RVM_LS_F0"};
+    "RVM_HEDGE",         "RVM_HEDGE_GROUPS", "RVM_HEDGE_MARK",   "RVM_HEDGE_WAIT",
+    "RVM_LS_F0"};
 
 static rvm::PlanKnobs knobs_with(const char* name, const char* value) {
     setenv(name, value, 1);
@@ -63,13 +64,17 @@
     const PlanKnobs K = read_plan_knobs();
     expect(K.skip_variants == 1 && K.late_spo == 96.0 && !K.no_level_split && K.n_teams == RVM_TEAMS_DEFAULT &&
                K.eager_split == 1 && !K.no_extension && K.refine_split && K.teams_hint && K.eager &&
-               K.eager_passes == 1 && K.hedge_groups == RVM_HEDGE_GROUPS_MAX && K.hedge_mark == 1,
+               K.eager_passes == 1 && K.hedge_groups == RVM_HEDGE_GROUPS_MAX && K.hedge_mark == 1 &&
+               K.hedge_wait == 1,
            "knob defaults");
     expect(knobs_with("RVM_REFINE_TEAMS", "9").n_teams == RVM_TEAMS_MAX, "RVM_REFINE_TEAMS=9 clamps");
     expect(knobs_with("RVM_HEDGE", "0").hedge_groups == 0, "RVM_HEDGE=0");
     expect(knobs_with("RVM_HEDGE_GROUPS", "3").hedge_groups == 3, "RVM_HEDGE_GROUPS=3");
     expect(knobs_with("RVM_EAGER_PASSES", "2").eager_passes == 2, "RVM_EAGER_PASSES=2");
     expect(knobs_with("RVM_SKIP_VARIANTS", "0").skip_variants == 0, "RVM_SKIP_VARIANTS=0");
+    expect(knobs_with("RVM_HEDGE_WAIT", "0").hedge_wait == 0 && knobs_with("RVM_HEDGE_WAIT", "1").hedge_wait == 1 &&
+               knobs_with("RVM_HEDGE_WAIT", "2").hedge_wait == 2 && knobs_with("RVM_HEDGE_WAIT", "x").hedge_wait == 1,
+           "RVM_HEDGE_WAIT");
 
     int mult[RVM_MAX_LEVELS] = {}, max_mult = 0;
     expect(check_plan_config(&cfg, t.data(), rv.data(), sg.data(), n_obs, 4096, mult, &max_mult) == nullptr,
@@ -138,6 +143,10 @@
     expect(P.fin_level == 3, "fin_level");
     expect(P.ext_mult == 8 && P.mult[4] == 8 && P.inv_ext == 0.125 && P.inv_mult[4] == 0.125, "ext_mult");
     expect(P.rmax == 6 && P.rtol_dir == 2.5e-7 && P.cut == 1 && P.n_teams == RVM_TEAMS_DEFAULT, "adaptive scalars");
+    expect(P.hedge_wait_ticks == hedge_wait_bound(P.spin_ticks) && P.hedge_wait_ticks < (P.spin_ticks << 1),
+           "hedge_wait_ticks");
+    for (unsigned long long sp : {1ull, 2ull, 3ull, 4ull, 1000ull, 200000000ull, 1ull << 40, 1ull << 62})
+        expect(hedge_wait_bound(sp) < sp && hedge_wait_bound(sp) < (sp << 1), "hedge_wait_bound");
     for (int k = 0; k < 4; k++) {
         const double nh = 2.0 * M_PI * cfg.dt / (mult[k] * cfg.period_hint), zn = 2.0 * nh * nh;
         expect(P.nt[k] == (zn <= 0.1 ? 6 : (zn <= 0.3 ? 7 : 8)) && P.spec[k] == (zn <= 0.04 ? 1 : 0), "nt / spec");
@@ -180,10 +189,12 @@
             const RqLayout R = rq_layout(mw, teams);
             expect(R.xgroups == (int32_t)xg, "rq xgroups");
             check_block({{R.x, xg * nt * 256 * 8, true}, {R.xf, xg * nt * 2 * 8, true},
-                         {R.t, xg * (nt - 1) * 1024 * 8, true}, {R.tf, xg * nt * 8, true}, {R.c, 16 * w, true},
+                         {R.t, xg * (nt - 1) * 1024 * 8, true}, {R.tf, xg * nt * 8, true}, {R.tb, xg * 8, true},
+                         {R.c, 16 * w, true},
                          {R.w, 12 * w, false}, {R.n, 16, false}, {R.gen, 8, true}, {R.mark, 4 * w, false},
                          {R.depth, 8 * (RVM_DEPTH_WINDOW + 1), true}},
                         R.bytes, "rqmem layout");
+            expect(R.tb == R.tf + xg * nt * 8, "rq_tb right behind rq_tf");
             expect(R.gen == R.n + 32 && R.mark == R.n + 64 && R.mark % 64 == R.n % 64, "rq_n | gen_dev | rq_mark");
         }
         const HLayout H = h_layout((int32_t)em, mw);
@@ -191,6 +202,9 @@
         check_block({{H.hrv, 16 * em * hs, true}, {H.hsum, 48 * hs, true}, {H.hslot, 16 * hs, true},
                      {H.htab, 8 * w, true}, {H.hw, 8 * RVM_HW_WORDS, true}},
                     H.bytes, "hmem layout");
+        expect(RVM_HW_STATS + 5 <= RVM_HW_MARK && RVM_HW_MARK + 2 * RVM_HEDGE_GROUPS_MAX <= RVM_HW_WAIT &&
+                   RVM_HW_WAIT + 3 <= RVM_HW_WORDS,
+               "hw words");
         const ELayout E = e_layout((int32_t)em, mw);
         check_block({{E.rve, 32 * em * w, true}, {E.esum, 96 * w, true},
                      {E.eflag, 8 * (RVM_EFLAG_WORDS * (size_t)((RVM_EAGER_MAX + 15) / 16) + 8), true}},
@@ -236,6 +250,9 @@
     expect(rvm_logl_batch(nullptr, 1, nullptr, 1.0, nullptr, nullptr, nullptr, nullptr) < 0, "logl null plan");
     int64_t mk = -1, gu = -1;
     expect(rvm_plan_hedge_marks(nullptr, 0, &mk, &gu, nullptr) < 0 && mk == -1 && gu == -1, "hedge_marks null plan");
+    int64_t lh = -1;
+    expect(rvm_plan_hedge_waits(nullptr, 0, &mk, &lh, &gu, nullptr) < 0 && mk == -1 && lh == -1 && gu == -1,
+           "hedge_waits null plan");
     rvm_param_map pm{};
     expect(rvm_stretch_half_step(nullptr, &pm, 10, 1, 0, nullptr, nullptr, nullptr, 1, nullptr, 2.0, 0, 0, 0, 1.0,
                                  nullptr, nullptr, nullptr, nullptr) < 0,
diff --git a/rvel-mcmc_amd/csrc/rvm_internal.h b/rvel-mcmc_amd/csrc/rvm_internal.h
--- a/rvel-mcmc_amd/csrc/rvm_internal.h
+++ b/rvel-mcmc_amd/csrc/rvm_internal.h
@@ -28,7 +28,8 @@
 constexpr int RVM_HEDGE_MAX_W = 12288;
 constexpr int RVM_HW_STATS = 2 + 2 * RVM_HEDGE_GROUPS_MAX;
 constexpr int RVM_HW_MARK = RVM_HW_STATS + 3 + 3;
-constexpr int RVM_HW_WORDS = RVM_HW_MARK + 2 * RVM_HEDGE_GROUPS_MAX;
+constexpr int RVM_HW_WAIT = RVM_HW_MARK + 2 * RVM_HEDGE_GROUPS_MAX;
+constexpr int RVM_HW_WORDS = RVM_HW_WAIT + 3;
 
 struct DirSched {
     int32_t n_epochs;
@@ -69,6 +70,7 @@
     int32_t* rq_w;
     double* rq_c;
     int32_t rq_cap;
+    uint32_t hedge_wait_ticks;
     int32_t* rq_mark;
     int32_t skip_variants;
     unsigned long long* rq_x;
@@ -87,6 +89,7 @@
     int32_t eager_split;
     int32_t hedge_groups;
     int32_t hedge_mark;
+    int32_t hedge_wait;
     double* hrv;
     double* hsum;
     unsigned long long* hslot;
diff --git a/rvel-mcmc_amd/csrc/rvm_plan.hip b/rvel-mcmc_amd/csrc/rvm_plan.hip
--- a/rvel-mcmc_amd/csrc/rvm_plan.hip
+++ b/rvel-mcmc_amd/csrc/rvm_plan.hip
@@ -163,6 +163,7 @@
             P.hw = at<unsigned long long>(plan->hmem, L.hw);
             P.hedge_groups = K.hedge_groups;
             P.hedge_mark = K.hedge_mark;
+            P.hedge_wait = K.hedge_wait;
         }
     }
     if (!(refines && K.eager)) {
@@ -324,6 +325,17 @@
     return 0;
 }
 
+int rvm_plan_hedge_waits(rvm_plan* plan, int32_t reset, int64_t* waited, int64_t* late_hits, int64_t* gave_way,
+                         void* stream) {
+    unsigned long long h[3];
+    const int rc = read_hw_words(plan, "rvm_plan_hedge_waits", rvm::RVM_HW_WAIT, 3, reset, stream, h);
+    if (rc != 0) return rc;
+    if (waited) *waited = (int64_t)h[0];
+    if (late_hits) *late_hits = (int64_t)h[1];
+    if (gave_way) *gave_way = (int64_t)h[2];
+    return 0;
+}
+
 int rvm_plan_faults(rvm_plan* plan, int32_t reset, int64_t* handoff_timeouts, int64_t* nonfinite,
                     int64_t* unresolved, int64_t* refined, int64_t* truncated, void* stream) {
     if (!plan) return fail(-1, "rvm_plan_faults: null plan");
@@ -375,6 +387,7 @@
     if (!(seconds > 0.0) || !(seconds < 1e9)) return fail(-1, "rvm_plan_set_handoff_timeout: seconds out of range");
     const double ticks = seconds * 1e8;
     plan->dev.spin_ticks = ticks < 1.0 ? 1ull : (unsigned long long)ticks;
+    plan->dev.hedge_wait_ticks = rvm::hedge_wait_bound(plan->dev.spin_ticks);
     return 0;
 }
 
diff --git a/rvel-mcmc_amd/csrc/rvm_plan_host.cpp b/rvel-mcmc_amd/csrc/rvm_plan_host.cpp
--- a/rvel-mcmc_amd/csrc/rvm_plan_host.cpp
+++ b/rvel-mcmc_amd/csrc/rvm_plan_host.cpp
@@ -38,6 +38,8 @@
     if (const char* hn = getenv("RVM_HEDGE_GROUPS"))
         K.hedge_groups = std::min(K.hedge_groups, std::max(0, std::min(atoi(hn), (int)RVM_HEDGE_GROUPS_MAX)));
     K.hedge_mark = starts(getenv("RVM_HEDGE_MARK"), '0') ? 0 : 1;
+    const char* hwt = getenv("RVM_HEDGE_WAIT");
+    K.hedge_wait = starts(hwt, '0') ? 0 : (starts(hwt, '2') ? 2 : 1);
     return K;
 }
 
@@ -169,6 +171,7 @@
     P.rmax = P.rtol_dir < INFINITY ? cfg->resolve_max : 0;
     P.cut = 1;
     P.spin_ticks = 200000000ull;
+    P.hedge_wait_ticks = hedge_wait_bound(P.spin_ticks);
     const int emax = (int)std::max<size_t>(std::max(nf, nb), 1);
     const int fit = (int)(RVM_LC_RING_BYTES / ((size_t)(nl + 1) * walkers_per_group(cfg->n_planets) * sizeof(double)));
     P.lc_ring = std::max(2, std::min(std::min(RVM_LC_RING, emax), fit));
@@ -187,6 +190,11 @@
     for (int k = 0; k <= RVM_MAX_LEVELS; k++) P.lw5[k] = 0.0;
 }
 
+uint32_t hedge_wait_bound(unsigned long long spin_ticks) {
+    const unsigned long long q = spin_ticks >> 2;
+    return q < 0xFFFFFFFFull ? (uint32_t)q : 0xFFFFFFFFu;
+}
+
 bool plan_wants_extension(const DevPlan& P, const PlanKnobs& K) {
     return P.rmax > 0 && P.n_levels >= 2 && P.n_levels < RVM_MAX_LEVELS && !K.no_extension;
 }
@@ -267,6 +275,7 @@
     L.xf = take(L.bytes, xg * nt * 2 * u64);
     L.t = take(L.bytes, xg * (nt - 1) * 16 * 64 * u64);
     L.tf = take(L.bytes, xg * nt * u64);
+    L.tb = take(L.bytes, xg * u64);
     L.c = take(L.bytes, 2 * (size_t)max_walkers * sizeof(double));
     L.w = take(L.bytes, (3 * (size_t)max_walkers * sizeof(int32_t) + 7) & ~(size_t)7);
     L.n = take(L.bytes, 64);
diff --git a/rvel-mcmc_amd/csrc/rvm_plan_host.h b/rvel-mcmc_amd/csrc/rvm_plan_host.h
--- a/rvel-mcmc_amd/csrc/rvm_plan_host.h
+++ b/rvel-mcmc_amd/csrc/rvm_plan_host.h
@@ -19,6 +19,7 @@
     int32_t eager_passes;
     int32_t hedge_groups;
     int32_t hedge_mark;
+    int32_t hedge_wait;
 };
 PlanKnobs read_plan_knobs();
 
@@ -40,6 +41,7 @@
 
 void fill_plan_scalars(const rvm_config* cfg, const int* mult, int32_t n_obs, size_t nf, size_t nb, int n_cu,
                        const PlanKnobs& K, DevPlan* P);
+uint32_t hedge_wait_bound(unsigned long long spin_ticks);
 bool plan_wants_extension(const DevPlan& P, const PlanKnobs& K);
 void fill_plan_extension(DevPlan* P);
 bool plan_wants_level_split(const DevPlan& P, int32_t max_walkers, const PlanKnobs& K);
@@ -59,7 +61,7 @@
 };
 XLayout x_layout(size_t nf, size_t nb, int32_t max_walkers, int n_teams);
 struct RqLayout {
-    size_t x, xf, t, tf, c, w, n, gen, mark, depth, bytes;
+    size_t x, xf, t, tf, tb, c, w, n, gen, mark, depth, bytes;
     int32_t xgroups;
 };
 RqLayout rq_layout(int32_t max_walkers, int n_teams);
diff --git a/rvel-mcmc_amd/csrc/rvm_refine_impl.h b/rvel-mcmc_amd/csrc/rvm_refine_impl.h
--- a/rvel-mcmc_amd/csrc/rvm_refine_impl.h
+++ b/rvel-mcmc_amd/csrc/rvm_refine_impl.h
@@ -16,7 +16,7 @@
 namespace rvm {
 
 #ifdef RVM_PROFILE
-#define RVM_RPROF_SLOTS 20
+#define RVM_RPROF_SLOTS 24
 #define RVM_RPROF_MAX_WAVES 4096
 static __device__ unsigned long long rvm_rprof[RVM_RPROF_MAX_WAVES * RVM_RPROF_SLOTS];
 #define RPROF_T(v) const unsigned long long v = __builtin_readcyclecounter()
@@ -64,6 +64,36 @@
     const unsigned long long nm = __builtin_popcountll(ballot(mark));
     if (lane == 0 && nm)
         __hip_atomic_fetch_add(hw + RVM_HW_STATS + 3, nm, __ATOMIC_RELAXED, __HIP_MEMORY_SCOPE_AGENT);
+}
+
+__device__ __forceinline__ int hedge_wait_poll(const DevPlan& P, const unsigned long long gen, const int wme,
+                                               const bool o0, const bool o1, const int wpb, const gu64* tbw,
+                                               const gu64* tdone) {
+    const unsigned long long done = (gen << 8) | 2ull, stop = (gen << 8) | 3ull;
+    auto state = [&](const int dd, const bool want) -> int {
+        if (!want) return 0;
+        const unsigned long long tb = __hip_atomic_load((gu64*)P.htab + wme, __ATOMIC_RELAXED, __HIP_MEMORY_SCOPE_AGENT);
+        const int ix = (int)(tb & 0xFFFF);
+        if ((tb >> 16) != gen || ix >= RVM_HEDGE_STRIDE || ix / wpb >= RVM_HEDGE_GROUPS_MAX) return 2;
+        if (__hip_atomic_load((gu64*)P.hslot + (size_t)dd * RVM_HEDGE_STRIDE + ix, __ATOMIC_RELAXED,
+                              __HIP_MEMORY_SCOPE_AGENT) != ((gen << 16) | (unsigned long long)wme))
+            return 2;
+        const unsigned long long w =
+            __hip_atomic_load((gu64*)P.hw + 2 + 2 * (ix / wpb) + dd, __ATOMIC_RELAXED, __HIP_MEMORY_SCOPE_AGENT);
+        return w == done ? 0 : (w == stop ? 2 : 1);
+    };
+    SpinClock clk;
+    clk.restart();
+    for (bool first = true;; first = false) {
+        const int s0 = state(0, o0), s1 = state(1, o1);
+        if (ballot(s0 == 2 || s1 == 2) != 0) return first ? -1 : 0;
+        if (ballot(s0 == 1 || s1 == 1) == 0) return 1;
+        const bool give = __hip_atomic_load(tbw, __ATOMIC_RELAXED, __HIP_MEMORY_SCOPE_AGENT) == ((gen << 8) | 1ull) ||
+                          __hip_atomic_load(tdone, __ATOMIC_RELAXED, __HIP_MEMORY_SCOPE_AGENT) == done ||
+                          clk.expired(P.hedge_wait_ticks);
+        if (__builtin_amdgcn_readfirstlane((int)give)) return 0;
+        __builtin_amdgcn_s_sleep(2);
+    }
 }
 
 __device__ __forceinline__ unsigned long long pass_ticks(const DevPlan& P, int rf) {
@@ -97,6 +127,7 @@
     RPROF_RT(prt_entry);
 #ifdef RVM_PROFILE
     unsigned long long p_seg = 0, p_epo = 0, p_steps = 0, p_wait = 0, p_pass = 0;
+    unsigned long long p_look = 0, p_info = 0, p_need = 0, p_barr = 0;
     int p_lvl = -1;
 #endif
 
@@ -166,7 +197,7 @@
     const int ntask = eager ? (esplit ? 2 * ngw : ngw) : (team ? ntask_team : (split ? ntask_split : ng));
     if ((int)blockIdx.x >= ntask) {
         if constexpr (HM) {
-            if (hedge && blockIdx.x == gridDim.x - 1 && wv == 0)
+            if (hedge && P.hedge_mark && blockIdx.x == gridDim.x - 1 && wv == 0)
                 hedge_mark_unneeded(P.rq_w, P.rq_cap, P.htab, P.hw, nq[0], nq[1], nq[2], gen, hedge, WPB);
         }
         leave();
@@ -716,6 +747,15 @@
             }
             if (bfirst) {
                 if (wv == 0) {
+#ifdef RVM_PROFILE
+                    p_barr = __builtin_amdgcn_s_memrealtime();
+                    p_info |= (unsigned long long)g << 32;
+#endif
+                    if constexpr (HM) {
+                        if (hedge && P.hedge_wait != 0 && tm == 1 && lane == 0)
+                            __hip_atomic_store((gu64*)(P.rq_tf + (size_t)P.rq_xgroups * P.n_teams + g), (gen << 8) | 1ull, __ATOMIC_RELAXED,
+                                               __HIP_MEMORY_SCOPE_AGENT);
+                    }
                     SpinClock clk;
                     clk.restart();
                     unsigned long long f = 0;
@@ -878,9 +918,44 @@
                 uint64_t m1 = ballot(live && s_open[1][lane] == 1);
                 if (hedge && team && tm == 0 && rf == 1 && own <= 0 && P.rmax >= 2 && (m0 | m1) != 0) {
                     const bool o0 = live && s_open[0][lane] == 1, o1 = live && s_open[1][lane] == 1;
-                    const int hi[2] = {hedge_index(0, o0), hedge_index(1, o1)};
+                    int hi[2] = {hedge_index(0, o0), hedge_index(1, o1)};
                     bool took = false;
-                    if (ballot((o0 && hi[0] < 0) || (o1 && hi[1] < 0)) == 0) {
+                    bool allin = ballot((o0 && hi[0] < 0) || (o1 && hi[1] < 0)) == 0;
+#ifdef RVM_PROFILE
+                    p_look = __builtin_amdgcn_s_memrealtime();
+                    p_info = (unsigned long long)g << 32;
+                    if (ballot((o0 && hi[0] < 0) || (o1 && hi[1] < 0)) == 0) p_info |= 1ull << 25;
+                    for (int d3 = 0; d3 < 2; d3++) {
+                        const bool want = d3 ? o1 : o0;
+                        const unsigned long long tb =
+                            __hip_atomic_load((gu64*)P.htab + wme, __ATOMIC_RELAXED, __HIP_MEMORY_SCOPE_AGENT);
+                        const int ix = (int)(tb & 0xFFFF);
+                        const bool tagged = (tb >> 16) == gen && ix < RVM_HEDGE_STRIDE && ix / WPB < RVM_HEDGE_GROUPS_MAX;
+                        const int blk = want && tagged ? 2 * (ix / WPB) + d3 : -1;
+                        for (int b = 0; b < 2 * RVM_HEDGE_GROUPS_MAX; b++) {
+                            const unsigned long long nb = __builtin_popcountll(ballot(blk == b));
+                            if (nb) {
+                                p_info |= 1ull << b;
+                                p_need += (nb < 15 ? nb : 15ull) << (4 * b);
+                            }
+                        }
+                        p_info += (unsigned long long)__builtin_popcountll(ballot(want && !tagged)) << 16;
+                    }
+#endif
+                    int polled = -1;
+                    if constexpr (HM) {
+                        if (P.hedge_wait != 0 && (P.hedge_wait == 2 || !allin)) {
+                            polled = hedge_wait_poll(P, gen, wme, o0, o1, WPB, (const gu64*)(P.rq_tf + (size_t)P.rq_xgroups * P.n_teams + g), tdone);
+                            if (polled >= 0) {
+                                if (polled == 1) {
+                                    hi[0] = hedge_index(0, o0);
+                                    hi[1] = hedge_index(1, o1);
+                                }
+                                allin = polled == 1 && ballot((o0 && hi[0] < 0) || (o1 && hi[1] < 0)) == 0;
+                            }
+                        }
+                    }
+                    if (allin) {
                         DirState q[2] = {dir_load(0), dir_load(1)};
                         bool fl[2] = {false, false};
                         for (int d3 = 0; d3 < 2; d3++) {
@@ -944,7 +1019,18 @@
                         if (took) __hip_atomic_fetch_add(P.counters + 3, nd, __ATOMIC_RELAXED, __HIP_MEMORY_SCOPE_AGENT);
                         __hip_atomic_fetch_add((gu64*)P.hw + RVM_HW_STATS + (took ? 1 : 2), nd, __ATOMIC_RELAXED,
                                                __HIP_MEMORY_SCOPE_AGENT);
-                    }
+                        if constexpr (HM) {
+                            if (polled >= 0) {
+                                __hip_atomic_fetch_add((gu64*)P.hw + RVM_HW_WAIT, 1ull, __ATOMIC_RELAXED,
+                                                       __HIP_MEMORY_SCOPE_AGENT);
+                                __hip_atomic_fetch_add((gu64*)P.hw + RVM_HW_WAIT + (took ? 1 : 2), 1ull, __ATOMIC_RELAXED,
+                                                       __HIP_MEMORY_SCOPE_AGENT);
+                            }
+                        }
+                    }
+#ifdef RVM_PROFILE
+                    if (took) p_info |= 1ull << 24;
+#endif
                     if (took) m0 = m1 = 0;
                 }
                 if (lane == 0) {
@@ -1031,6 +1117,10 @@
             o[15] = pt_setup - pt_entry;
             o[16] = pt_slot - pt_entry;
             o[17] = pt_rows - pt_entry;
+            o[18] = p_look;
+            o[19] = p_info;
+            o[20] = p_need;
+            o[21] = p_barr;
         }
 #endif
     }
@@ -1192,8 +1282,10 @@
     }
     __syncthreads();
     auto count_marked = [&]() {
-        if (tid == 0 && s_marked)
-            __hip_atomic_fetch_add(hw + RVM_HW_STATS + 4, 1ull, __ATOMIC_RELAXED, __HIP_MEMORY_SCOPE_AGENT);
+        if (tid == 0) {
+            if (s_marked) __hip_atomic_fetch_add(hw + RVM_HW_STATS + 4, 1ull, __ATOMIC_RELAXED, __HIP_MEMORY_SCOPE_AGENT);
+            __hip_atomic_store(hw + 2 + 2 * g + dd, (gen << 8) | 3ull, __ATOMIC_RELAXED, __HIP_MEMORY_SCOPE_AGENT);
+        }
     };
     if (s_cancel[0]) {
         count_marked();
@@ -1204,24 +1296,53 @@
         s_ck[i] = kbad;
         s_ci[i] = 0;
     }
-    for (int i = tid; i < W; i += 256) {
-        int kind = 0, wk = i, jst = 0, jp = 0;
-        double zst = 0.0, zp = 0.0;
-        stretch_slot(sa, i, kind, wk, zst, jst, zp, jp);
-        double sc = INFINITY;
-        bool ok = true;
-#pragma unroll
-        for (int p = 0; p < NP; p++) {
-            const double m = walker_param(true, nullptr, W, wk, sa, PR * p + 0, zst, jst, kind, zp, jp);
-            const double a = walker_param(true, nullptr, W, wk, sa, PR * p + 1, zst, jst, kind, zp, jp);
-            const double h = walker_param(true, nullptr, W, wk, sa, PR * p + 2, zst, jst, kind, zp, jp);
-            const double k = walker_param(true, nullptr, W, wk, sa, PR * p + 3, zst, jst, kind, zp, jp);
-            const double e = sqrt(h * h + k * k);
-            ok = ok && a > 0.02 && m > 5e-6 && e < 1.0;
-            sc = fmin(sc, a * (1.0 - e) / cbrt(1.0 + m));
-        }
-        ok = ok && isfinite(sc) && sc > 0.0;
-        s_key[i] = ok ? (unsigned long long)__double_as_longlong(sc) : kbad;
+    constexpr int KCH = NP <= 2 ? 4 : 2;
+    for (int i0 = tid; i0 < W; i0 += 256 * KCH) {
+        int kind[KCH], wk[KCH], jst[KCH], jp[KCH];
+        double zst[KCH], zp[KCH];
+#pragma unroll
+        for (int c = 0; c < KCH; c++) {
+            const int i = i0 + 256 * c < W ? i0 + 256 * c : i0;
+            kind[c] = 0, wk[c] = i, jst[c] = 0, jp[c] = 0;
+            zst[c] = 0.0, zp[c] = 0.0;
+            stretch_slot(sa, i, kind[c], wk[c], zst[c], jst[c], zp[c], jp[c]);
+        }
+        double va[KCH][4 * NP], vb[KCH][4 * NP], vx[KCH][4 * NP];
+#pragma unroll
+        for (int c = 0; c < KCH; c++) {
+#pragma unroll
+            for (int q = 0; q < 4 * NP; q++) {
+                const int k = sa.src[PR * (q >> 2) + (q & 3)];
+                const int ku = k < 0 ? 0 : k;
+                const double* ba = kind[c] == 0 ? sa.c : sa.c0;
+                const double* bx = kind[c] == 0 ? sa.x : sa.x1;
+                const size_t sx = (size_t)(kind[c] == 0 ? sa.xstride : sa.n_spec);
+                va[c][q] = ba[(size_t)jst[c] * sa.dim + ku];
+                vb[c][q] = sa.c[(size_t)(kind[c] == 2 ? jp[c] : 0) * sa.dim + ku];
+                vx[c][q] = bx[(size_t)ku * sx + wk[c]];
+            }
+        }
+#pragma unroll
+        for (int c = 0; c < KCH; c++) {
+            double row[4 * NP];
+#pragma unroll
+            for (int q = 0; q < 4 * NP; q++) {
+                const int r = PR * (q >> 2) + (q & 3);
+                const double cj = kind[c] == 2 ? stretch_q(vb[c][q], zp[c], va[c][q]) : va[c][q];
+                row[q] = sa.src[r] < 0 ? sa.base[r] : stretch_q(cj, zst[c], vx[c][q]);
+            }
+            double sc = INFINITY;
+            bool ok = true;
+#pragma unroll
+            for (int p = 0; p < NP; p++) {
+                const double m = row[4 * p + 0], a = row[4 * p + 1], h = row[4 * p + 2], k = row[4 * p + 3];
+                const double e = sqrt(h * h + k * k);
+                ok = ok && a > 0.02 && m > 5e-6 && e < 1.0;
+                sc = fmin(sc, a * (1.0 - e) / cbrt(1.0 + m));
+            }
+            ok = ok && isfinite(sc) && sc > 0.0;
+            if (i0 + 256 * c < W) s_key[i0 + 256 * c] = ok ? (unsigned long long)__double_as_longlong(sc) : kbad;
+        }
     }
     auto scan256 = [&](int* c) {
         const int c0 = c[4 * lane], c1 = c[4 * lane + 1], c2 = c[4 * lane + 2], c3 = c[4 * lane + 3];
@@ -1408,6 +1529,7 @@
         o[9] = (unsigned long long)blockIdx.x | (1ull << 29) | ((unsigned long long)(cancelled ? 1 : 0) << 30);
         o[10] = cancelled ? 0 : 1;
         o[11] = (unsigned long long)(unsigned)__builtin_amdgcn_s_getreg((31 << 11) | 4);
+        o[4] = (unsigned long long)s_marked;
     }
 #endif
     if (cancelled) {
@@ -1433,6 +1555,11 @@
         asm volatile("s_waitcnt vmcnt(0)" ::: "memory");
         if (lane == 0)
             __hip_atomic_store(hw + 2 + 2 * g + dd, (gen << 8) | 2ull, __ATOMIC_RELAXED, __HIP_MEMORY_SCOPE_AGENT);
+#ifdef RVM_PROFILE
+        if (lane == 0 && RVM_RPROF_MAX_WAVES / 2 + (size_t)blockIdx.x * 8 < RVM_RPROF_MAX_WAVES)
+            rvm_rprof[(RVM_RPROF_MAX_WAVES / 2 + (size_t)blockIdx.x * 8) * RVM_RPROF_SLOTS + 5] =
+                __builtin_amdgcn_s_memrealtime();
+#endif
     }
 }
 
@@ -1519,7 +1646,7 @@
     const int groups = (W + wpb - 1) / wpb + 2;
     int nb = std::max(2, std::min(P.n_cu > 0 ? P.n_cu : 256, 2 * groups));
     nb &= ~1;
-    if (w4 && hedge && P.hedge_mark && smem <= refine_budget<NPV, D3V, RVM_REFINE_HM>())
+    if (w4 && hedge && smem <= refine_budget<NPV, D3V, RVM_REFINE_HM>())
         refine_kernel<NPV, D3V, RVM_REFINE_HM><<<dim3(nb), dim3(256), smem, stream>>>(P, W, params, hill_factor, rv_out,
                                                                                       logl, status, sa, eager, hedge);
     else if (w4)
@@ -1537,7 +1664,7 @@
     const size_t smem = (size_t)emax * 8 * sizeof(double);
     const size_t b = std::min(refine_budget<NPV, D3V, 4>(), refine_budget<NPV, D3V, 8>());
     if (P.hedge_groups > 0) (void)hedge_budget<NPV, D3V>();
-    if (P.hedge_groups > 0 && P.hedge_mark) (void)refine_budget<NPV, D3V, RVM_REFINE_HM>();
+    if (P.hedge_groups > 0) (void)refine_budget<NPV, D3V, RVM_REFINE_HM>();
     return smem <= b ? hipSuccess : hipErrorInvalidConfiguration;
 }
 
diff --git a/rvel-mcmc_amd/rvmcmc/_lib.py b/rvel-mcmc_amd/rvmcmc/_lib.py
--- a/rvel-mcmc_amd/rvmcmc/_lib.py
+++ b/rvel-mcmc_amd/rvmcmc/_lib.py
@@ -93,6 +93,8 @@
     "rvm_plan_hedge_stats": (C.c_int, [C.c_void_p, C.c_int32, C.POINTER(C.c_int64), C.POINTER(C.c_int64),
                                        C.POINTER(C.c_int64), C.c_void_p]),
     "rvm_plan_hedge_marks": (C.c_int, [C.c_void_p, C.c_int32, C.POINTER(C.c_int64), C.POINTER(C.c_int64), C.c_void_p]),
+    "rvm_plan_hedge_waits": (C.c_int, [C.c_void_p, C.c_int32, C.POINTER(C.c_int64), C.POINTER(C.c_int64),
+                                       C.POINTER(C.c_int64), C.c_void_p]),
     "rvm_plan_info": (C.c_int, [C.c_void_p, C.POINTER(C.c_int32), C.POINTER(C.c_int32), C.POINTER(C.c_int32),
                                 C.POINTER(C.c_int32)]),
     "rvm_logl_batch": (C.c_int, [C.c_void_p, C.c_int32, _dp, C.c_double, _dp, _dp, _dp, _dp]),
diff --git a/rvel-mcmc_amd/rvmcmc/engine.py b/rvel-mcmc_amd/rvmcmc/engine.py
--- a/rvel-mcmc_amd/rvmcmc/engine.py
+++ b/rvel-mcmc_amd/rvmcmc/engine.py
@@ -173,6 +173,12 @@
                                                  _lib.stream_handle(stream)), "rvm_plan_hedge_marks")
         return dict(marked=m.value, gave_up=g.value)
 
+    def hedge_waits(self, reset=False, stream=None) -> dict:
+        w, h, g = C.c_int64(), C.c_int64(), C.c_int64()
+        _lib.check(self.lib.rvm_plan_hedge_waits(self._h, int(bool(reset)), C.byref(w), C.byref(h), C.byref(g),
+                                                 _lib.stream_handle(stream)), "rvm_plan_hedge_waits")
+        return dict(waited=w.value, late_hits=h.value, gave_way=g.value)
+
     def check_faults(self, what="plan", stream=None, group=None) -> dict:
         f = self.faults(reset=True, stream=stream)
         bad = [f["handoff_timeouts"], f["nonfinite"], f["unresolved"] if self.resolve_max > 0 else 0]
```

Result: faster. 3.226 million, median of 6 (+3.1%).
